# JJKK1313/DiTreeOnlinePlanner

Measured on AMD Instinct MI355X. Metric: candidate tree-expansions/sec (carmaze, H=32), higher is better.
Workload: dtype f16x3; 1 GPU; cfgs/carmaze.yaml + fm_policy flow sampler (K=1), batch=1024 candidates per GPU, H=32 (4 chunks x 8 steps), boxes.csv 20x20, 1024-node tree snapshot, seeded random weights; batch_per_gpu=1024, global_batch=1024, edge_length=32, action_horizon=8, pred_horizon=64, flow_steps=1, tree_nodes=1024, parallelism=candidates sharded x1

## Files before the change

### ditreeonlineplanner_amd/csrc/denoise.h

```cpp
#pragma once
#include <hip/hip_runtime.h>
#include <stdint.h>

enum { MODE_BIAS = 0, MODE_GN_MISH = 1, MODE_GN_MISH_FILM = 2, MODE_GN_MISH_RES = 3 };

enum { ST_BF16 = 0, ST_F32 = 1, ST_F16 = 2 };
static inline int fmt_make(int st, bool split) { return st | (split ? 4 : 0); }
static inline __host__ __device__ int fmt_st(int f) { return f & 3; }
static inline __host__ __device__ bool fmt_split(int f) { return (f & 4) != 0; }
static inline int fmt_es(int f) { return fmt_st(f) == ST_F32 ? 4 : 2; }

struct ConvGemmParams {
  const void* A;
  int lda;
  int in_Lp;
  int in_stride;
  int in_off;
  int taps, Cin;
  const void* W;
  void* Out;
  int ldc;
  int out_Lp, out_stride, out_off;
  int out_coff;
  int L;
  int M, N;
  const float* bias;
  int mode;
  const float* gamma;
  const float* beta;
  int group_ch;
  float eps;
  const float* film;
  int film_ld, film_off;
  const void* Res;
  int ldres, res_Lp, res_off;
  int out_f32;
  int dbg;
  int c2d, c2_H, c2_W, c2_OW, c2_OHW, c2_stride, c2_pad;
  signed char c2_kh[12], c2_kw[12];
  const void* zero;
  long long a_plane, w_plane, out_plane, res_plane;
  float w_scale;
  int splitk;
  long long slab_stride;
  float* sk_ws;
  int* sk_cnt;
  int* sat;
};

void denoise_set_dry_run(bool on);
bool denoise_dry_run();
void launch_conv_gemm(const ConvGemmParams& p, int fmt, hipStream_t s);
bool conv2d_small_eligible(int fmt);
int conv_gemm_kind(const ConvGemmParams& p, int fmt);
bool conv_gemm_supported(const ConvGemmParams& p, int fmt);
void launch_prep_sample(const float* x, void* A0, int B, int P, int D, int fmt, long long plane, hipStream_t s, int* sat = nullptr);
void launch_time_embed(float t, const float* W1, const float* b1, const float* W2, const float* b2, float* out,
                       hipStream_t s);
void launch_prep_cond(const float* temb, const float* map_emb, int E, int E_ld, const float* cond, int G, void* out, int B,
                      int Kpad, int fmt, long long plane, hipStream_t s, int* sat = nullptr);
struct FlowStep {
  int mode;
  float dt;
  float sb, sa, c0, c1, sigma;
  const float* z;
  long long z_row;
  const int* z_idx;
  int z_row0;
};
void launch_final_proj_flow(const void* Y, int C, int Lp, long long plane, const float* W, const float* bias, int D, float* x,
                            FlowStep fs, const double* act_norm , double* actions, int B, int P, int fmt,
                            hipStream_t s);
struct TapList {
  int n;
  signed char kh[49], kw[49];
};
void launch_gn1d(void* x, int ld, int Lp, int row_off, int coff, int L, int C, const float* gamma, const float* beta, float eps,
                 int mode, const float* film, int film_ld, int film_off, const void* res, int ldres, int res_Lp, int res_off,
                 int B, int fmt, long long x_plane, long long res_plane, hipStream_t s, int* sat = nullptr);
void launch_encoder_stem(const float* lm, int n, const float* W, const float* gamma, const float* beta, void* out, int B, float eps,
                         int fmt, long long plane, hipStream_t s, int* sat = nullptr);
void launch_im2col2d(const void* in, bool src_f32, void* out, int B, int H, int W, int C, const TapList& taps, int stride,
                     int pad, int OH, int OW, int Kpad, int fmt, hipStream_t s);
void launch_gn2d(const float* in, int nslab, long long slab_stride, const float* gamma, const float* beta, const void* res,
                 int relu, void* out, int B, int HW, int C, float eps, int fmt, long long res_plane, long long out_plane,
                 hipStream_t s, int* sat = nullptr);
void launch_maxpool2d(const void* in, void* out, int B, int H, int W, int C, int OH, int OW, int fmt, hipStream_t s);
void launch_avgpool2d(const void* in, void* out, int B, int HW, int C, int fmt, long long in_plane, long long out_plane,
                      hipStream_t s);
void launch_unpack_act(const void* in, int ld, int coff, int Lp, int roff, float* out, int B, int L, int C, int fmt,
                       long long plane, hipStream_t s);

enum { ENC_RESNET = 0, ENC_IDENTITY = 1, ENC_MLP = 2, ENC_MAX = 3, ENC_GRID = 4, ENC_CNN = 5 };
struct SmallEncoderParams {
  int kind;
  const float* lm;
  float* out;
  int B, n, E, k;
  const float* w[4];
  const float* b[4];
};
const char* small_encoder_name(int kind);
int small_encoder_width(int kind, int n, int k);
void launch_small_encoder(const SmallEncoderParams& p, hipStream_t s);
```

### ditreeonlineplanner_amd/csrc/denoise_host.hip

```cpp
#include <algorithm>
#include <cmath>
#include <cstring>
#include <functional>
#include <map>
#include <sstream>
#include <thread>

#include "denoise.h"
#include "ditree_internal.h"

namespace {

struct HostParam {
  std::vector<int64_t> dims;
  const float* data = nullptr;
  int64_t n = 0;
};

struct Act {
  void* p = nullptr;
  int L = 0, C = 0;
  int ld = 0, coff = 0;
  bool padded = true;
  long long plane = 0;
  int fmt = 0;
  int Lp() const { return padded ? L + 2 : L; }
};

struct Packed {
  void* p = nullptr;
  long long plane = 0;
  float scale = 1.0f;
};

inline uint16_t f2bf_host(float f) {
  uint32_t u;
  std::memcpy(&u, &f, 4);
  if ((u & 0x7fffffffu) > 0x7f800000u) return (uint16_t)((u >> 16) | 0x40);
  u += 0x7fffu + ((u >> 16) & 1u);
  return (uint16_t)(u >> 16);
}
inline float bf2f_host(uint16_t h) {
  uint32_t u = (uint32_t)h << 16;
  float f;
  std::memcpy(&f, &u, 4);
  return f;
}
inline uint16_t f2h_host(float f) { _Float16 h = (_Float16)f; uint16_t u; std::memcpy(&u, &h, 2); return u; }
inline float h2f_host(uint16_t u) { _Float16 h; std::memcpy(&h, &u, 2); return (float)h; }

}

struct DenoiserState {
  ditree_ctx* ctx = nullptr;
  std::vector<float> blob;
  std::map<std::string, HostParam> params;
  int D = 2, P = 64, E = 400, G = 7, cond_dim = 663, lm = 20;
  int enc_kind = ENC_RESNET;
  int enc_E = -1;
  int enc_k = 0;
  int dims[3] = {512, 1024, 2048};
  bool loaded = false;
  const float* ddpm_coef = nullptr;
  const float* ddpm_z = nullptr;
  long long ddpm_z_row = 0, ddpm_z_step = 0;
  int ddpm_row0 = 0;
  int prec = -1, Bmax = 0;
  int Buser = 0;
  int bgran = 16;
  int ufmt = 0, efmt = 0;
  std::vector<void*> allocs;
  std::map<std::string, Act> named;
  std::map<std::string, Packed> dev_w;
  std::map<std::string, float*> dev_f;
  std::vector<std::function<void(int, int, hipStream_t)>> unet_ops;
  std::vector<std::function<void(int, int, int, hipStream_t)>> enc_ops;
  static constexpr int ENC_SUBS = 4;
  int sub_cap = 0;
  size_t col_region = 0, gout_region = 0;
  hipStream_t aux[ENC_SUBS] = {nullptr, nullptr, nullptr, nullptr};
  hipEvent_t ev_fork = nullptr, ev_join[ENC_SUBS] = {nullptr, nullptr, nullptr, nullptr};
  std::function<void(int, int, hipStream_t)> film_op;
  float* x_cur = nullptr;
  float* temb = nullptr;
  float temb_t = -1.0f;
  float* map_emb = nullptr;
  int E_ld = 400;
  float* film = nullptr;
  void* condA = nullptr;
  long long cond_plane = 0;
  int condK = 0, film_cols = 0;
  Act final_h;
  const float* lm_ptr = nullptr;
  void* zero_row = nullptr;
  static constexpr int SAT_SLOTS = 256;
  int* sat_flags = nullptr;
  int *sat_cond = nullptr, *sat_sample = nullptr;
  std::vector<std::string> sat_names;
  int* sat_slot(const std::string& layer, int fmt) {
    if (fmt_st(fmt) != ST_F16 || sat_flags == nullptr) return nullptr;
    for (size_t i = 0; i < sat_names.size(); ++i)
      if (sat_names[i] == layer) return sat_flags + i;
    if ((int)sat_names.size() >= SAT_SLOTS) return sat_flags + SAT_SLOTS - 1;
    sat_names.push_back(layer);
    return sat_flags + sat_names.size() - 1;
  }
  int last_splitk[4] = {1, 1, 1, 1};
  long long last_slab[4] = {0, 0, 0, 0};
  bool prof_on = false;
  int prof_mode = 0;
  std::vector<hipEvent_t> prof_ev;
  size_t prof_used = 0;
  double prof_ms_done[3] = {0, 0, 0};
  int64_t prof_launches_done[3] = {0, 0, 0};
  double prof_flops_done[3] = {0, 0, 0};
  struct ProfRec { size_t a, b; int kind; double flops; int launches; };
  bool run_open = false;
  size_t run_end = 0;
  void close_run() {
    if (run_open) { hipEventRecord(prof_ev[run_end], prof_last_stream); run_open = false; }
  }
  hipStream_t prof_last_stream = nullptr;
  bool prof_chain = false;
  std::vector<ProfRec> prof_pairs;
  void note_other() { close_run(); prof_chain = false; }
  float* sk_ws = nullptr;
  int* sk_cnt = nullptr;
  static constexpr int SK_MAX_SLABS = 512;
  int pick_splitk(const ConvGemmParams& p, int fmt) {
    const char* e = getenv("DITREE_DENOISE_SPLITK");
    if (!e || atoi(e) == 0 || !fmt_split(fmt) || p.L == 4 || conv_gemm_kind(p, fmt) != 0) return 1;
    const int tiles = (p.M >> 8) * (p.N >> 8), nvc = p.Cin >> 5;
    int sk = 1;
    static const int cap = [] { const char* c = getenv("DITREE_DENOISE_SPLITK_WGS"); return c ? atoi(c) : 64; }();
    while (sk < 16 && tiles * (sk * 2) <= cap && tiles * (sk * 2) <= SK_MAX_SLABS && nvc % (sk * 2) == 0 && nvc / (sk * 2) >= 2) sk *= 2;
    return sk;
  }
  void run_gemm(const ConvGemmParams& p_in, int fmt, hipStream_t s) {
    ConvGemmParams p = p_in;
    static const int strips = [] { const char* e = getenv("DITREE_XCD_STRIPS"); return e ? atoi(e) : 1; }();
    p.dbg = strips;
    if (const int sk = pick_splitk(p, fmt); sk > 1) {
      if (sk_ws == nullptr) {
        sk_ws = (float*)dalloc((size_t)SK_MAX_SLABS * 65536 * sizeof(float), false);
        sk_cnt = (int*)dalloc(SK_MAX_SLABS * sizeof(int));
      }
      p.splitk = sk; p.sk_ws = sk_ws; p.sk_cnt = sk_cnt;
    }
    if (!conv_gemm_supported(p, fmt))
      throw std::runtime_error("denoiser layer of shape M " + std::to_string(p.M) + " x N " + std::to_string(p.N) + " x K " +
                               std::to_string(p.taps) + "*" + std::to_string(p.Cin) + " (L " + std::to_string(p.L) +
                               ") fits no tile of this precision");
    if (!prof_on) { launch_conv_gemm(p, fmt, s); return; }
    if (prof_used + 2 > prof_ev.size()) {
      const size_t old = prof_ev.size();
      prof_ev.resize(old + 4096);
      for (size_t i = old; i < prof_ev.size(); ++i) hipEventCreate(&prof_ev[i]);
    }
    const double fl = 2.0 * (double)p.M * (double)p.N * (double)p.taps * (double)p.Cin;
    if (prof_mode == 2) {
      const int dom = fmt_st(ufmt) == ST_F32 ? 1 : 0;
      if (conv_gemm_kind(p, fmt) != dom || fmt != ufmt) { close_run(); launch_conv_gemm(p, fmt, s); return; }
      if (run_open && prof_last_stream == s) {
        launch_conv_gemm(p, fmt, s);
        prof_pairs.back().flops += fl;
        prof_pairs.back().launches += 1;
        return;
      }
      close_run();
      const size_t st = prof_used++;
      run_end = prof_used++;
      hipEventRecord(prof_ev[st], s);
      launch_conv_gemm(p, fmt, s);
      prof_pairs.push_back(ProfRec{st, run_end, dom, fl, 1});
      run_open = true;
      prof_last_stream = s;
      return;
    }
    size_t start;
    if (prof_chain && prof_last_stream == s && prof_used > 0) {
      start = prof_used - 1;
    } else {
      start = prof_used++;
      hipEventRecord(prof_ev[start], s);
    }
    launch_conv_gemm(p, fmt, s);
    const size_t end = prof_used++;
    hipEventRecord(prof_ev[end], s);
    prof_pairs.push_back(ProfRec{start, end, conv_gemm_kind(p, fmt), fl, 1});
    prof_chain = true;
    prof_last_stream = s;
  }
  void prof_collect() {
    close_run();
    if (prof_used == 0) return;
    hipDeviceSynchronize();
    for (auto& pr : prof_pairs) {
      float ms = 0.f;
      if (hipEventElapsedTime(&ms, prof_ev[pr.a], prof_ev[pr.b]) == hipSuccess) prof_ms_done[pr.kind] += ms;
      prof_launches_done[pr.kind] += pr.launches;
      prof_flops_done[pr.kind] += pr.flops;
    }
    prof_pairs.clear();
    prof_used = 0;
    prof_chain = false;
  }
  int es() const { return fmt_es(ufmt); }
  int ees() const { return fmt_es(efmt); }
  int planes() const { return fmt_split(ufmt) ? 2 : 1; }

  const HostParam& P_(const std::string& name) const {
    auto it = params.find(name);
    if (it == params.end()) throw std::runtime_error("missing parameter " + name);
    return it->second;
  }
  bool has(const std::string& name) const { return params.count(name) != 0; }

  void* dalloc(size_t bytes, bool zero = true) {
    void* p = nullptr;
    if (hipMalloc(&p, bytes ? bytes : 16) != hipSuccess) throw std::runtime_error("hipMalloc failed");
    if (zero && hipMemset(p, 0, bytes ? bytes : 16) != hipSuccess) throw std::runtime_error("hipMemset failed");
    allocs.push_back(p);
    return p;
  }
  void free_workspace() {
    for (void* p : allocs) hipFree(p);
    allocs.clear();
    sk_ws = nullptr;
    sk_cnt = nullptr;
    named.clear();
    dev_w.clear();
    dev_f.clear();
    enc_ops.clear();
    unet_ops.clear();
    film_op = nullptr;
    sat_flags = sat_cond = sat_sample = nullptr;
    sat_names.clear();
    prec = -1;
    Bmax = 0;
    Buser = 0;
    temb_t = -1.0f;
  }

  float* upload_f32(const std::string& key, const float* src, int64_t n) {
    auto it = dev_f.find(key);
    if (it != dev_f.end()) return it->second;
    float* d = (float*)dalloc((size_t)n * 4, false);
    if (hipMemcpy(d, src, (size_t)n * 4, hipMemcpyHostToDevice) != hipSuccess) throw std::runtime_error("memcpy");
    dev_f[key] = d;
    return d;
  }
  float* vec(const std::string& name) {
    const HostParam& hp = P_(name);
    return upload_f32(name, hp.data, hp.n);
  }

  template <class F>
  Packed pack(const std::string& key, int fmt, int N, int T, int Cin_pad, F get) {
    auto it = dev_w.find(key);
    if (it != dev_w.end()) return it->second;
    const int Npad = (N + 255) / 256 * 256;
    const size_t K = (size_t)T * Cin_pad, total = (size_t)Npad * K;
    const int st = fmt_st(fmt), e = fmt_es(fmt), npl = fmt_split(fmt) ? 2 : 1;
    std::vector<uint8_t> host(total * e * npl, 0);
    const int nthreads = std::max(1u, std::min(16u, std::thread::hardware_concurrency()));
    float mul = 1.0f;
    if (st == ST_F16) {
      std::vector<float> mx(nthreads, 0.0f);
      std::vector<std::thread> th;
      for (int ti = 0; ti < nthreads; ++ti)
        th.emplace_back([&, ti]() {
          float m = 0.f;
          for (int n = ti; n < N; n += nthreads)
            for (int t = 0; t < T; ++t)
              for (int ci = 0; ci < Cin_pad; ++ci) m = std::max(m, std::fabs(get(n, t, ci)));
          mx[ti] = m;
        });
      for (auto& t : th) t.join();
      const float m = *std::max_element(mx.begin(), mx.end());
      if (m > 0.f && std::isfinite(m)) {
        int ex;
        std::frexp(m, &ex);
        mul = std::ldexp(1.0f, 14 - ex);
      }
    }
    std::vector<std::thread> th;
    for (int ti = 0; ti < nthreads; ++ti) {
      th.emplace_back([&, ti]() {
        for (int n = ti; n < N; n += nthreads) {
          for (int t = 0; t < T; ++t)
            for (int ci = 0; ci < Cin_pad; ++ci) {
              const float v = get(n, t, ci) * mul;
              const size_t idx = (size_t)n * K + (size_t)t * Cin_pad + ci;
              if (st == ST_F32) { ((float*)host.data())[idx] = v; continue; }
              uint16_t* hi = (uint16_t*)host.data();
              uint16_t* lo = hi + total;
              if (st == ST_BF16) {
                hi[idx] = f2bf_host(v);
                if (npl == 2) lo[idx] = f2bf_host(v - bf2f_host(hi[idx]));
              } else {
                hi[idx] = f2h_host(v);
                if (npl == 2) lo[idx] = f2h_host(v - h2f_host(hi[idx]));
              }
            }
        }
      });
    }
    for (auto& t : th) t.join();
    Packed pk;
    pk.p = dalloc(total * e * npl, false);
    pk.plane = npl == 2 ? (long long)(total * e) : 0;
    pk.scale = 1.0f / mul;
    if (hipMemcpy(pk.p, host.data(), total * e * npl, hipMemcpyHostToDevice) != hipSuccess) throw std::runtime_error("memcpy");
    dev_w[key] = pk;
    return pk;
  }
  static void set_w(ConvGemmParams& p, const Packed& pk) { p.W = pk.p; p.w_plane = pk.plane; p.w_scale = pk.scale; }

  Act make_act(const std::string& name, int L, int C, bool padded = true) {
    Act a;
    a.L = L; a.C = C; a.ld = C; a.coff = 0; a.padded = padded; a.fmt = ufmt;
    const size_t bytes = (size_t)Bmax * a.Lp() * C * es();
    a.plane = planes() == 2 ? (long long)bytes : 0;
    if (planes() == 2 && bytes >= 0x7f000000ull) throw std::runtime_error("activation plane of 2 GiB or more: lower the reserved batch");
    a.p = dalloc(bytes * planes());
    named[name] = a;
    return a;
  }
  static void set_in(ConvGemmParams& p, const Act& in) { p.a_plane = in.plane; }
  static void set_out(ConvGemmParams& p, const Act& out) { p.out_plane = out.plane; }
  static Act view(const Act& base, int coff, int C, const char* = nullptr) {
    Act v = base;
    v.coff = coff;
    v.C = C;
    return v;
  }
  const char* aptr(const Act& a) const { return (const char*)a.p + (size_t)a.coff * es(); }

  void add_conv3(std::vector<std::function<void(int, int, hipStream_t)>>& ops, const std::string& wname, const Act& in,
                 const Act& out, int mode, const std::string& gn, int film_off, const Act* res) {
    const HostParam& w = P_(wname + ".weight");
    const int Cout = (int)w.dims[0], Cin = (int)w.dims[1];
    const float* wd = w.data;
    const Packed wp = pack(wname, ufmt, Cout, 3, Cin, [=](int n, int t, int ci) { return wd[((size_t)n * Cin + ci) * 3 + t]; });
    ConvGemmParams p{};
    p.A = aptr(in); p.lda = in.ld; p.in_Lp = in.Lp(); p.in_stride = 1; p.in_off = 0; p.taps = 3; p.Cin = Cin;
    set_w(p, wp); set_in(p, in); set_out(p, out);
    p.sat = sat_slot(wname, ufmt);
    p.Out = (void*)aptr(out); p.ldc = out.ld; p.out_Lp = out.Lp(); p.out_stride = 1; p.out_off = 1; p.out_coff = 0;
    p.L = in.L; p.N = Cout; p.bias = vec(wname + ".bias"); p.mode = mode; p.eps = 1e-5f;
    if (mode >= MODE_GN_MISH) {
      p.gamma = vec(gn + ".weight"); p.beta = vec(gn + ".bias"); p.group_ch = Cout / 8;
    }
    if (mode == MODE_GN_MISH_FILM) { p.film = film; p.film_ld = film_cols; p.film_off = film_off; }
    if (mode == MODE_GN_MISH_RES) {
      p.Res = aptr(*res); p.ldres = res->ld; p.res_Lp = res->Lp(); p.res_off = res->padded ? 1 : 0; p.res_plane = res->plane;
    }
    emit_block(ops, p, out, in.L);
  }
  void emit_block(std::vector<std::function<void(int, int, hipStream_t)>>& ops, const ConvGemmParams& p, const Act& out, int L) {
    const int Cout = p.N, mode = p.mode, uf = ufmt;
    const int gch = Cout / 8;
    static const bool short_unfused = [] { const char* e = getenv("DITREE_GN_SHORT_UNFUSED"); return e && atoi(e) != 0; }();
    const bool short_fusable = (L == 8 || L == 4) && fmt_st(uf) != ST_F32 && !short_unfused;
    const bool fused = mode < MODE_GN_MISH ||
                       ((Cout & 255) == 0 && (gch == 64 || gch == 128 || gch == 256) && ((L & 15) == 0 || short_fusable));
    const bool fused_needs_tiles = fused && mode >= MODE_GN_MISH && (L & 15) != 0;
    ConvGemmParams qf = p, q = p;
    q.mode = MODE_BIAS;
    const float* film_p = p.film;
    const int film_ld_ = p.film_ld, film_off_ = p.film_off, ldres = p.ldres, res_Lp = p.res_Lp, res_off = p.res_off;
    const void* resp = p.Res;
    const float *ga = p.gamma, *be = p.beta;
    void* xo = (void*)out.p;
    const int ld = out.ld, oLp = out.Lp(), ocoff = out.coff;
    const long long xpl = out.plane, rpl = p.res_plane;
    int* gsat = p.sat;
    ops.push_back([=, this](int, int Bp, hipStream_t s) mutable {
      if (fused && (!fused_needs_tiles || ((Bp * L) & 255) == 0)) {
        qf.M = Bp * L;
        run_gemm(qf, uf, s);
        return;
      }
      q.M = Bp * L;
      run_gemm(q, uf, s);
      note_other();
      launch_gn1d(xo, ld, oLp, 1, ocoff, L, Cout, ga, be, 1e-5f, mode, film_p, film_ld_, film_off_, resp, ldres, res_Lp,
                  res_off, Bp, uf, xpl, rpl, s, gsat);
    });
  }
  void add_conv1(std::vector<std::function<void(int, int, hipStream_t)>>& ops, const std::string& wname, const Act& in,
                 const Act& out) {
    const HostParam& w = P_(wname + ".weight");
    const int Cout = (int)w.dims[0], Cin = (int)w.dims[1];
    const float* wd = w.data;
    const Packed wp = pack(wname, ufmt, Cout, 1, Cin, [=](int n, int, int ci) { return wd[(size_t)n * Cin + ci]; });
    ConvGemmParams p{};
    p.A = aptr(in); p.lda = in.ld; p.in_Lp = in.Lp(); p.in_stride = 1; p.in_off = 1; p.taps = 1; p.Cin = Cin;
    set_w(p, wp); set_in(p, in); set_out(p, out);
    p.sat = sat_slot(wname, ufmt);
    p.Out = (void*)aptr(out); p.ldc = out.ld; p.out_Lp = out.Lp(); p.out_stride = 1; p.out_off = 1;
    p.L = in.L; p.N = Cout; p.bias = vec(wname + ".bias"); p.mode = MODE_BIAS;
    const int L = in.L, uf = ufmt;
    ops.push_back([this, p, L, uf](int, int Bp, hipStream_t s) mutable {
      p.M = Bp * L;
      run_gemm(p, uf, s);
    });
  }
  void add_down(std::vector<std::function<void(int, int, hipStream_t)>>& ops, const std::string& wname, const Act& in,
                const Act& out) {
    const HostParam& w = P_(wname + ".weight");
    const int Cout = (int)w.dims[0], Cin = (int)w.dims[1];
    const float* wd = w.data;
    const Packed wp = pack(wname, ufmt, Cout, 3, Cin, [=](int n, int t, int ci) { return wd[((size_t)n * Cin + ci) * 3 + t]; });
    ConvGemmParams p{};
    p.A = aptr(in); p.lda = in.ld; p.in_Lp = in.Lp(); p.in_stride = 2; p.in_off = 0; p.taps = 3; p.Cin = Cin;
    set_w(p, wp); set_in(p, in); set_out(p, out);
    p.sat = sat_slot(wname, ufmt);
    p.Out = (void*)aptr(out); p.ldc = out.ld; p.out_Lp = out.Lp(); p.out_stride = 1; p.out_off = 1;
    p.L = out.L; p.N = Cout; p.bias = vec(wname + ".bias"); p.mode = MODE_BIAS;
    const int L = out.L, uf = ufmt;
    ops.push_back([this, p, L, uf](int, int Bp, hipStream_t s) mutable {
      p.M = Bp * L;
      run_gemm(p, uf, s);
    });
  }
  void add_up(std::vector<std::function<void(int, int, hipStream_t)>>& ops, const std::string& wname, const Act& in,
              const Act& out) {
    const HostParam& w = P_(wname + ".weight");
    const int Cin = (int)w.dims[0], Cout = (int)w.dims[1];
    const float* wd = w.data;
    for (int par = 0; par < 2; ++par) {
      const int k0 = par == 0 ? 3 : 2, k1 = par == 0 ? 1 : 0;
      const Packed wp = pack(wname + (par ? ".odd" : ".even"), ufmt, Cout, 2, Cin, [=](int n, int t, int ci) {
        return wd[((size_t)ci * Cout + n) * 4 + (t == 0 ? k0 : k1)];
      });
      ConvGemmParams p{};
      p.A = aptr(in); p.lda = in.ld; p.in_Lp = in.Lp(); p.in_stride = 1; p.in_off = par; p.taps = 2; p.Cin = Cin;
      set_w(p, wp); set_in(p, in); set_out(p, out);
      p.sat = sat_slot(wname, ufmt);
      p.Out = (void*)aptr(out); p.ldc = out.ld; p.out_Lp = out.Lp(); p.out_stride = 2; p.out_off = 1 + par;
      p.L = in.L; p.N = Cout; p.bias = vec(wname + ".bias"); p.mode = MODE_BIAS;
      const int L = in.L, uf = ufmt;
      ops.push_back([this, p, L, uf](int, int Bp, hipStream_t s) mutable {
        p.M = Bp * L;
        run_gemm(p, uf, s);
      });
    }
  }

  void add_crb(const std::string& pre, const Act& in, const Act& out, int& film_cursor, const std::string& tag) {
    const int Cout = (int)P_(pre + ".blocks.0.block.0.weight").dims[0];
    Act h = make_act(tag + ".h", in.L, Cout);
    const int film_off = film_cursor;
    film_cursor += 2 * Cout;
    add_conv3(unet_ops, pre + ".blocks.0.block.0", in, h, MODE_GN_MISH_FILM, pre + ".blocks.0.block.1", film_off, nullptr);
    Act res = in;
    if (has(pre + ".residual_conv.weight")) {
      res = make_act(tag + ".res", in.L, Cout);
      add_conv1(unet_ops, pre + ".residual_conv", in, res);
    }
    add_conv3(unet_ops, pre + ".blocks.1.block.0", h, out, MODE_GN_MISH_RES, pre + ".blocks.1.block.1", 0, &res);
  }

  void build(int prec_, int Bmax_);
};

void DenoiserState::build(int prec_, int Bmax_) {
  free_workspace();
  prec = prec_;
  switch (prec) {
    case DITREE_PREC_BF16: ufmt = fmt_make(ST_BF16, false); efmt = ST_BF16; break;
    case DITREE_PREC_F32: ufmt = fmt_make(ST_F32, false); efmt = ST_F32; break;
    case DITREE_PREC_F16X3: ufmt = fmt_make(ST_F16, true); efmt = ufmt; break;
    case DITREE_PREC_BF16X3: ufmt = fmt_make(ST_BF16, true); efmt = ufmt; break;
    case DITREE_PREC_F16: ufmt = fmt_make(ST_F16, false); efmt = ST_F16; break;
    default: throw std::runtime_error("unknown precision");
  }
  sat_flags = (int*)dalloc(SAT_SLOTS * sizeof(int));
  sat_cond = sat_slot("cond_encoder input: Mish(time | map embedding | observation)", ufmt);
  sat_sample = sat_slot("sample (the noisy action sequence)", ufmt);
  const int C0 = dims[0], C1 = dims[1], C2 = dims[2];
  const int L0 = P, L1 = P / 2, L2 = P / 4;
  if (P % 16 != 0 || P < 16 || P > 256 || (256 % P) != 0) throw std::runtime_error("pred_horizon must be 16, 32, 64, 128 or 256");
  bgran = fmt_st(ufmt) != ST_F32 ? std::max(16, 1024 / P) : 16;
  Buser = Bmax_;
  Bmax = (Bmax_ + bgran - 1) / bgran * bgran;
  {
    const long long per_sample = std::max({(long long)(L2 + 2) * 2 * C2, (long long)(L1 + 2) * 2 * C1, (long long)(L0 + 2) * C0,
                                           (long long)L0 * 64}) * fmt_es(ufmt);
    long long cap = std::min<long long>(8192, 0x7f000000LL / per_sample);
    cap = cap / 256 * 256;
    if (cap < 256) throw std::runtime_error("denoiser too large for one 256-sample work unit");
    if (Bmax > cap) Bmax = (int)cap;
  }
  if (fmt_split(ufmt) && ((C0 | C1 | C2) & 255) != 0)
    throw std::runtime_error("the split precisions need down_dims that are multiples of 256 (halo / gemm16 tiles)");
  x_cur = (float*)dalloc((size_t)Bmax * P * D * 4);
  temb = (float*)dalloc(256 * 4);
  condK = (cond_dim + 63) / 64 * 64;
  const int Brows = (Bmax + 255) / 256 * 256;
  E_ld = (enc_kind == ENC_RESNET && fmt_split(efmt)) ? (E + 255) / 256 * 256 : E;
  map_emb = (float*)dalloc((size_t)Brows * E_ld * 4);
  cond_plane = planes() == 2 ? (long long)Brows * condK * es() : 0;
  condA = dalloc((size_t)Brows * condK * es() * planes());

  std::vector<std::string> crbs = {"unet.down_modules.0.0", "unet.down_modules.0.1", "unet.down_modules.1.0",
                                   "unet.down_modules.1.1", "unet.down_modules.2.0", "unet.down_modules.2.1",
                                   "unet.mid_modules.0",    "unet.mid_modules.1",    "unet.up_modules.0.0",
                                   "unet.up_modules.0.1",   "unet.up_modules.1.0",   "unet.up_modules.1.1"};
  film_cols = 0;
  std::vector<int> film_offs;
  for (auto& c : crbs) {
    film_offs.push_back(film_cols);
    film_cols += (int)P_(c + ".cond_encoder.1.weight").dims[0];
  }
  film = (float*)dalloc((size_t)Brows * film_cols * 4);
  {
    std::vector<const float*> wsrc, bsrc;
    std::vector<int> rows;
    for (auto& c : crbs) {
      wsrc.push_back(P_(c + ".cond_encoder.1.weight").data);
      bsrc.push_back(P_(c + ".cond_encoder.1.bias").data);
      rows.push_back((int)P_(c + ".cond_encoder.1.weight").dims[0]);
    }
    std::vector<int> start(rows.size());
    for (size_t i = 0, a = 0; i < rows.size(); ++i) { start[i] = (int)a; a += rows[i]; }
    const int cd = cond_dim;
    const Packed wp = pack("film.all", ufmt, film_cols, 1, condK, [=](int n, int, int ci) {
      size_t i = std::upper_bound(start.begin(), start.end(), n) - start.begin() - 1;
      return ci < cd ? wsrc[i][(size_t)(n - start[i]) * cd + ci] : 0.0f;
    });
    std::vector<float> ball(film_cols);
    for (size_t i = 0; i < rows.size(); ++i) std::memcpy(ball.data() + start[i], bsrc[i], (size_t)rows[i] * 4);
    float* bd = upload_f32("film.bias", ball.data(), film_cols);
    ConvGemmParams p{};
    p.A = condA; p.lda = condK; p.in_Lp = 0; p.in_stride = 1; p.in_off = 0; p.taps = 1; p.Cin = condK;
    set_w(p, wp); p.a_plane = cond_plane;
    p.Out = film; p.ldc = film_cols; p.out_Lp = 0; p.out_stride = 1; p.out_off = 0;
    p.N = film_cols; p.bias = bd; p.mode = MODE_BIAS; p.out_f32 = 1;
    const int uf = ufmt;
    film_op = [this, p, uf](int, int Bp, hipStream_t s) mutable {
      const int Mr = fmt_st(uf) == ST_F32 ? Bp : (Bp + 255) / 256 * 256;
      p.M = Mr; p.L = Mr; p.in_Lp = Mr; p.out_Lp = Mr;
      run_gemm(p, uf, s);
    };
  }

  int fc = 0;
  Act a0;
  a0.L = L0; a0.C = 64; a0.ld = 64; a0.coff = 0; a0.padded = false; a0.fmt = ufmt;
  a0.plane = planes() == 2 ? (long long)Bmax * L0 * 64 * es() : 0;
  a0.p = dalloc((size_t)Bmax * L0 * 64 * es() * planes());
  named["a0"] = a0;
  {
    const std::string pre = "unet.down_modules.0.0";
    const HostParam& w = P_(pre + ".blocks.0.block.0.weight");
    const float* wd = w.data;
    const int Dd = D;
    const Packed wp = pack(pre + ".blocks.0.block.0", ufmt, C0, 1, 64, [=](int n, int, int ci) {
      if (ci >= 3 * Dd) return 0.0f;
      const int t = ci / Dd, d = ci - t * Dd;
      return wd[((size_t)n * Dd + d) * 3 + t];
    });
    Act h = make_act("d0b1.h", L0, C0);
    ConvGemmParams p{};
    p.A = a0.p; p.lda = 64; p.in_Lp = L0; p.in_stride = 1; p.in_off = 0; p.taps = 1; p.Cin = 64;
    set_w(p, wp); set_in(p, a0); set_out(p, h);
    p.sat = sat_slot(pre + ".blocks.0.block.0", ufmt);
    p.Out = h.p; p.ldc = h.ld; p.out_Lp = h.Lp(); p.out_stride = 1; p.out_off = 1;
    p.L = L0; p.N = C0; p.bias = vec(pre + ".blocks.0.block.0.bias"); p.mode = MODE_GN_MISH_FILM; p.eps = 1e-5f;
    p.gamma = vec(pre + ".blocks.0.block.1.weight"); p.beta = vec(pre + ".blocks.0.block.1.bias"); p.group_ch = C0 / 8;
    p.film = film; p.film_ld = film_cols; p.film_off = film_offs[0];
    const int L = L0;
    emit_block(unet_ops, p, h, L0);
    const HostParam& wr = P_(pre + ".residual_conv.weight");
    const float* wrd = wr.data;
    const Packed wrp = pack(pre + ".residual_conv", ufmt, C0, 1, 64, [=](int n, int, int ci) {
      return (ci >= Dd && ci < 2 * Dd) ? wrd[(size_t)n * Dd + (ci - Dd)] : 0.0f;
    });
    Act res = make_act("d0b1.res", L0, C0);
    ConvGemmParams q{};
    q.A = a0.p; q.lda = 64; q.in_Lp = L0; q.in_stride = 1; q.in_off = 0; q.taps = 1; q.Cin = 64;
    set_w(q, wrp); set_in(q, a0); set_out(q, res);
    q.sat = sat_slot(pre + ".residual_conv", ufmt);
    q.Out = res.p; q.ldc = res.ld; q.out_Lp = res.Lp(); q.out_stride = 1; q.out_off = 1;
    q.L = L0; q.N = C0; q.bias = vec(pre + ".residual_conv.bias"); q.mode = MODE_BIAS;
    const int uf = ufmt;
    unet_ops.push_back([this, q, L, uf](int, int Bp, hipStream_t s) mutable { q.M = Bp * L; run_gemm(q, uf, s); });
    Act o = make_act("d0b1.out", L0, C0);
    add_conv3(unet_ops, pre + ".blocks.1.block.0", h, o, MODE_GN_MISH_RES, pre + ".blocks.1.block.1", 0, &res);
    fc = film_offs[1];
  }
  Act cat1 = make_act("cat1", L1, 2 * C1);
  Act cat0 = make_act("cat0", L2, 2 * C2);
  Act d0o = named["d0b1.out"];
  Act skip0 = make_act("skip0", L0, C0);
  add_crb("unet.down_modules.0.1", d0o, skip0, fc, "d0b2");
  Act d1in = make_act("d1.in", L1, C0);
  add_down(unet_ops, "unet.down_modules.0.2.conv", skip0, d1in);
  Act d1o = make_act("d1b1.out", L1, C1);
  add_crb("unet.down_modules.1.0", d1in, d1o, fc, "d1b1");
  Act skip1 = view(cat1, C1, C1);
  named["skip1"] = skip1;
  add_crb("unet.down_modules.1.1", d1o, skip1, fc, "d1b2");
  Act d2in = make_act("d2.in", L2, C1);
  add_down(unet_ops, "unet.down_modules.1.2.conv", skip1, d2in);
  Act d2o = make_act("d2b1.out", L2, C2);
  add_crb("unet.down_modules.2.0", d2in, d2o, fc, "d2b1");
  Act skip2 = view(cat0, C2, C2);
  named["skip2"] = skip2;
  add_crb("unet.down_modules.2.1", d2o, skip2, fc, "d2b2");
  Act m1 = make_act("mid1.out", L2, C2);
  add_crb("unet.mid_modules.0", skip2, m1, fc, "mid1");
  Act m2 = view(cat0, 0, C2);
  named["mid2.out"] = m2;
  add_crb("unet.mid_modules.1", m1, m2, fc, "mid2");
  Act u0a = make_act("u0b1.out", L2, C1);
  add_crb("unet.up_modules.0.0", cat0, u0a, fc, "u0b1");
  Act u0b = make_act("u0b2.out", L2, C1);
  add_crb("unet.up_modules.0.1", u0a, u0b, fc, "u0b2");
  Act up0 = view(cat1, 0, C1);
  named["up0.out"] = up0;
  add_up(unet_ops, "unet.up_modules.0.2.conv", u0b, up0);
  Act u1a = make_act("u1b1.out", L1, C0);
  add_crb("unet.up_modules.1.0", cat1, u1a, fc, "u1b1");
  Act u1b = make_act("u1b2.out", L1, C0);
  add_crb("unet.up_modules.1.1", u1a, u1b, fc, "u1b2");
  Act fin = make_act("final.in", L0, C0);
  add_up(unet_ops, "unet.up_modules.1.2.conv", u1b, fin);
  final_h = make_act("final.h", L0, C0);
  add_conv3(unet_ops, "unet.final_conv.0.block.0", fin, final_h, MODE_GN_MISH, "unet.final_conv.0.block.1", 0, nullptr);
  vec("unet.final_conv.1.weight");
  vec("unet.final_conv.1.bias");
  vec("unet.diffusion_step_encoder.1.weight");
  vec("unet.diffusion_step_encoder.1.bias");
  vec("unet.diffusion_step_encoder.3.weight");
  vec("unet.diffusion_step_encoder.3.bias");

  sub_cap = ((Bmax + ENC_SUBS - 1) / ENC_SUBS + 15) / 16 * 16;
  if (enc_kind != ENC_RESNET) {
    SmallEncoderParams q{};
    q.kind = enc_kind; q.n = lm; q.E = E; q.k = enc_k;
    auto transposed = [&](const std::string& name, int out_f, int in_f) {
      const HostParam& w = P_(name);
      if (w.dims.size() != 2 || w.dims[0] != out_f || w.dims[1] != in_f)
        throw std::runtime_error(name + " must be (" + std::to_string(out_f) + ", " + std::to_string(in_f) + ")");
      std::vector<float> t((size_t)out_f * in_f);
      for (int o = 0; o < out_f; ++o)
        for (int i = 0; i < in_f; ++i) t[(size_t)i * out_f + o] = w.data[(size_t)o * in_f + i];
      return upload_f32(name + "#t", t.data(), (int64_t)t.size());
    };
    auto conv_w = [&](const std::string& name, int co, int ci) {
      const HostParam& w = P_(name + ".weight");
      const HostParam& b = P_(name + ".bias");
      if (w.dims.size() != 4 || w.dims[0] != co || w.dims[1] != ci || w.dims[2] != 3 || w.dims[3] != 3 || b.n != co)
        throw std::runtime_error(name + " must be a Conv2d(" + std::to_string(ci) + ", " + std::to_string(co) + ", 3)");
    };
    if (enc_kind == ENC_MLP) {
      const int in_f = lm * lm;
      q.w[0] = transposed("encoder.fc1.weight", 128, in_f);
      q.w[1] = transposed("encoder.fc2.weight", 256, 128);
      q.w[2] = transposed("encoder.fc3.weight", E, 256);
      const int outs[3] = {128, 256, E};
      for (int l = 0; l < 3; ++l) {
        const std::string bn = "encoder.fc" + std::to_string(l + 1) + ".bias";
        if (P_(bn).n != outs[l]) throw std::runtime_error(bn + " must have " + std::to_string(outs[l]) + " elements");
        q.b[l] = vec(bn);
      }
    } else if (enc_kind == ENC_GRID || enc_kind == ENC_CNN) {
      const bool g = enc_kind == ENC_GRID;
      const int nl = g ? 3 : 4;
      const int ci[4] = {1, g ? 3 : 2, g ? 6 : 4, 4}, co[4] = {g ? 3 : 2, g ? 6 : 4, 4, 4};
      for (int l = 0; l < nl; ++l) {
        const std::string nm = "encoder.conv" + std::to_string(l + 1);
        conv_w(nm, co[l], ci[l]);
        q.w[l] = vec(nm + ".weight");
        q.b[l] = vec(nm + ".bias");
      }
    }
    const float** lm_slot = &lm_ptr;
    float* op = map_emb;
    const int LM = lm * lm, Ew = E;
    enc_ops.push_back([=, this](int b0, int Bn, int, hipStream_t s) {
      note_other();
      SmallEncoderParams r = q;
      r.lm = *lm_slot + (size_t)b0 * LM; r.out = op + (size_t)b0 * Ew; r.B = Bn;
      launch_small_encoder(r, s);
    });
  } else {
    const std::string R = "encoder.resnet18.";
    const int pr = efmt;
    const size_t E_ = ees();
    zero_row = dalloc(256);
    const size_t col_per_sample = 25 * 576;
    const size_t gout_per_sample = 9216;
    col_region = (size_t)sub_cap * col_per_sample;
    gout_region = (size_t)sub_cap * gout_per_sample;
    char* col = (char*)dalloc(col_region * ENC_SUBS * E_);
    float* gout = (float*)dalloc(gout_region * ENC_SUBS * 4);
    const size_t colreg = col_region, goutreg = gout_region;
    auto ebuf = [&](const std::string& name, int HW, int C) {
      Act a;
      a.L = HW; a.C = C; a.ld = C; a.coff = 0; a.padded = false; a.fmt = efmt;
      const size_t rows = HW == 1 ? (size_t)Brows : (size_t)Bmax;
      const size_t bytes = rows * HW * C * ees();
      a.plane = fmt_split(efmt) ? (long long)bytes : 0;
      a.p = dalloc(bytes * (fmt_split(efmt) ? 2 : 1));
      named[name] = a;
      return a;
    };
    auto live_taps = [](int k, int stride, int pad, int H, int OH) {
      TapList tl{};
      for (int kh = 0; kh < k; ++kh)
        for (int kw = 0; kw < k; ++kw) {
          bool lh = false, lw = false;
          for (int o = 0; o < OH; ++o) {
            const int ih = o * stride + kh - pad, iw = o * stride + kw - pad;
            lh |= (ih >= 0 && ih < H);
            lw |= (iw >= 0 && iw < H);
          }
          if (lh && lw) { tl.kh[tl.n] = (signed char)kh; tl.kw[tl.n] = (signed char)kw; ++tl.n; }
        }
      return tl;
    };
    auto conv2d = [&](const std::string& wname, const void* in, long long in_plane, int H, int Cin, int Cout, int k, int stride,
                      int pad, int OH, bool fold_in) {
      const HostParam& w = P_(wname + ".weight");
      const float* wd = w.data;
      const int Cw = (int)w.dims[1];
      const TapList tl = live_taps(k, stride, pad, H, OH);
      const int K = tl.n * Cin, Kpad = (K + 63) / 64 * 64;
      if ((size_t)OH * OH * Kpad > col_per_sample || (size_t)OH * OH * Cout > gout_per_sample)
        throw std::runtime_error("encoder scratch region too small for " + wname);
      const Packed wp = pack(wname, efmt, Cout, 1, Kpad, [=](int n, int, int kk) {
        if (kk >= K) return 0.0f;
        const int c = kk % Cin, t = kk / Cin, kw = tl.kw[t], kh = tl.kh[t];
        if (!fold_in) return wd[(((size_t)n * Cw + c) * k + kh) * k + kw];
        float s = 0.f;
        for (int cc = 0; cc < Cw; ++cc) s += wd[(((size_t)n * Cw + cc) * k + kh) * k + kw];
        return s;
      });
      const float** lm_slot = &lm_ptr;
      const bool implicit = (in != nullptr) && (Cin % 64 == 0) && tl.n <= 12;
      if (!implicit && fmt_split(efmt)) throw std::runtime_error("split encoder: " + wname + " needs the im2col path");
      const void* zr = zero_row;
      enc_ops.push_back([=, this](int b0, int Bn, int reg, hipStream_t s) {
        char* colr = col + (size_t)reg * colreg * E_;
        float* goutr = gout + (size_t)reg * goutreg;
        ConvGemmParams p{};
        const int M = Bn * OH * OH;
        if (implicit) {
          p.A = (const char*)in + (size_t)b0 * H * H * Cin * E_; p.lda = Cin; p.taps = tl.n; p.Cin = Cin; p.a_plane = in_plane;
          p.c2d = 1; p.c2_H = H; p.c2_W = H; p.c2_OW = OH; p.c2_OHW = OH * OH; p.c2_stride = stride; p.c2_pad = pad;
          for (int t = 0; t < tl.n; ++t) { p.c2_kh[t] = tl.kh[t]; p.c2_kw[t] = tl.kw[t]; }
          p.zero = zr;
          const int nk_total = tl.n * (Cin / 64);
          const int tiles = ((1024 * OH * OH + 255) / 256) * ((Cout + 255) / 256);
          static int sk_target = -1, sk_cap = 8;
          if (sk_target < 0) {
            const char* e = getenv("DITREE_SPLITK_TARGET");
            sk_target = (e && atoi(e) > 0) ? atoi(e) : 256;
            const char* c = getenv("DITREE_SPLITK_CAP");
            if (c && atoi(c) > 0) sk_cap = atoi(c);
          }
          int sk = std::max(1, std::min(std::min(sk_cap, nk_total / 2), std::max(1, sk_target / tiles)));
          while (sk > 1 && (size_t)sk * OH * OH * Cout > gout_per_sample) --sk;
          if (sk > 1) {
            const int per = (nk_total + sk - 1) / sk;
            sk = (nk_total + per - 1) / per;
          }
          static int use_split = -1;
          if (use_split < 0) { const char* e = getenv("DITREE_SPLITK"); use_split = (e && !atoi(e)) ? 0 : 1; }
          if (conv2d_small_eligible(pr)) {
            static int small_target = -1;
            if (small_target < 0) { const char* e = getenv("DITREE_C2D_TARGET"); small_target = (e && atoi(e) > 0) ? atoi(e) : 768; }
            const int tiles64 = ((1024 * OH * OH + 63) / 64) * (Cout / 64);
            sk = std::max(1, std::min(std::min(8, nk_total / 2), small_target / tiles64));
            while (sk > 1 && (size_t)sk * OH * OH * Cout > gout_per_sample) --sk;
            if (sk > 1) {
              const int per = (nk_total + sk - 1) / sk;
              sk = (nk_total + per - 1) / per;
            }
          }
          if (!use_split) sk = 1;
// ... 6 lines not shown
          last_slab[reg] = 0;
        }
        if (!implicit) {
          note_other();
          if (in == nullptr)
            launch_im2col2d(*lm_slot + (size_t)b0 * H * H, true, colr, Bn, H, H, 1, tl, stride, pad, OH, OH, Kpad, pr, s);
          else
            launch_im2col2d((const char*)in + (size_t)b0 * H * H * Cin * E_, false, colr, Bn, H, H, Cin, tl, stride, pad,
                            OH, OH, Kpad, pr, s);
          p.A = colr; p.lda = Kpad; p.taps = 1; p.Cin = Kpad;
        }
        p.in_Lp = M; p.in_stride = 1; p.in_off = 0;
        set_w(p, wp);
        p.Out = goutr; p.ldc = Cout; p.out_Lp = M; p.out_stride = 1; p.out_off = 0;
        p.L = M; p.M = M; p.N = Cout; p.mode = MODE_BIAS; p.out_f32 = 1;
        run_gemm(p, pr, s);
      });
    };
    auto gn = [&](const std::string& gname, const Act& out, const Act* res, bool relu) {
      float* ga = vec(gname + ".weight");
      float* be = vec(gname + ".bias");
      const char* rp = res ? (const char*)res->p : nullptr;
      char* op = (char*)out.p;
      const int HW = out.L, C = out.C;
      const long long rpl = res ? res->plane : 0, opl = out.plane;
      {
        const int pp = (C >= 64 && C <= 1024 && (C & (C - 1)) == 0) ? 256 / (C >> 2) : 0;
        if (pp == 0 || (HW + pp - 1) / pp > 7)
          throw std::runtime_error("encoder GroupNorm: unsupported map (" + std::to_string(HW) + " pixels x " + std::to_string(C) + " channels)");
      }
      int* gsat = sat_slot(gname, efmt);
      enc_ops.push_back([=, this](int b0, int Bn, int reg, hipStream_t s) {
        note_other();
        const size_t off = (size_t)b0 * HW * C * E_;
        launch_gn2d(gout + (size_t)reg * goutreg, last_splitk[reg], last_slab[reg], ga, be, rp ? rp + off : nullptr,
                    relu ? 1 : 0, op + off, Bn, HW, C, 1e-5f, pr, rpl, opl, s, gsat);
      });
    };
    const int H0 = lm;
    auto osz = [](int h, int k, int s, int p) { return (h + 2 * p - k) / s + 1; };
    const int H1 = osz(H0, 7, 2, 3);
    const int H2 = osz(H1, 3, 2, 1);
    Act c1 = ebuf("enc.c1", H1 * H1, 64);
    Act pool = ebuf("enc.pool", H2 * H2, 64);
    if (H0 == 20 || H0 == 16) {
      const HostParam& w = P_(R + "conv1.weight");
      const int Cw = (int)w.dims[1];
      std::vector<float> wf(64 * 49);
      for (int n = 0; n < 64; ++n)
        for (int t = 0; t < 49; ++t) {
          float sacc = 0.f;
          for (int cc = 0; cc < Cw; ++cc) sacc += w.data[((size_t)n * Cw + cc) * 49 + t];
          wf[t * 64 + n] = sacc;
        }
      float* wdev = upload_f32(R + "conv1.weight#folded", wf.data(), 64 * 49);
      float* ga = vec(R + "bn1.weight");
      float* be = vec(R + "bn1.bias");
      char* op = (char*)pool.p;
      const float** lm_slot = &lm_ptr;
      const long long ppl = pool.plane;
      int* ssat = sat_slot(R + "conv1", efmt);
      enc_ops.push_back([=, this](int b0, int Bn, int, hipStream_t s) {
        note_other();
        launch_encoder_stem(*lm_slot + (size_t)b0 * H0 * H0, H0, wdev, ga, be, op + (size_t)b0 * H2 * H2 * 64 * E_, Bn, 1e-5f, pr, ppl, s, ssat);
      });
    } else {
    conv2d(R + "conv1", nullptr, 0, H0, 1, 64, 7, 2, 3, H1, true);
    gn(R + "bn1", c1, nullptr, true);
    {
      const char* ip = (const char*)c1.p; char* op = (char*)pool.p;
      const int a = H1, b2 = H2;
      enc_ops.push_back([=, this](int b0, int Bn, int, hipStream_t s) {
        note_other();
        launch_maxpool2d(ip + (size_t)b0 * a * a * 64 * E_, op + (size_t)b0 * b2 * b2 * 64 * E_, Bn, a, a, 64, b2, b2, pr, s);
      });
    }
    }
    Act cur = pool;
    int Hc = H2, Cc = 64;
    const int chans[4] = {64, 128, 256, 512};
    for (int li = 0; li < 4; ++li) {
      for (int bi = 0; bi < 2; ++bi) {
        const std::string pre = R + "layer" + std::to_string(li + 1) + "." + std::to_string(bi);
        const int Cout = chans[li];
        const int stride = (bi == 0 && li > 0) ? 2 : 1;
        const int Ho = osz(Hc, 3, stride, 1);
        const std::string tag = "enc.l" + std::to_string(li + 1) + "." + std::to_string(bi);
        Act t1 = ebuf(tag + ".t", Ho * Ho, Cout);
        conv2d(pre + ".conv1", cur.p, cur.plane, Hc, Cc, Cout, 3, stride, 1, Ho, false);
        gn(pre + ".bn1", t1, nullptr, true);
        Act idt = cur;
        if (has(pre + ".downsample.0.weight")) {
          Act ds = ebuf(tag + ".ds", Ho * Ho, Cout);
          conv2d(pre + ".downsample.0", cur.p, cur.plane, Hc, Cc, Cout, 1, stride, 0, Ho, false);
          gn(pre + ".downsample.1", ds, nullptr, false);
          idt = ds;
        }
        Act o = ebuf(tag + ".out", Ho * Ho, Cout);
        conv2d(pre + ".conv2", t1.p, t1.plane, Ho, Cout, Cout, 3, 1, 1, Ho, false);
        gn(pre + ".bn2", o, &idt, true);
        cur = o;
        Hc = Ho;
        Cc = Cout;
      }
    }
    Act pooled = ebuf("enc.avg", 1, Cc);
    {
      const char* ip = (const char*)cur.p; char* op = (char*)pooled.p;
      const int HW = Hc * Hc, C = Cc;
      const long long ipl = cur.plane, opl = pooled.plane;
      enc_ops.push_back([=, this](int b0, int Bn, int, hipStream_t s) {
        note_other();
        launch_avgpool2d(ip + (size_t)b0 * HW * C * E_, op + (size_t)b0 * C * E_, Bn, HW, C, pr, ipl, opl, s);
      });
    }
    {
      const HostParam& w = P_(R + "fc.weight");
      const float* wd = w.data;
      const int Kf = (int)w.dims[1], Nf = (int)w.dims[0];
      const Packed wp = pack(R + "fc", efmt, Nf, 1, Kf, [=](int n, int, int ci) { return wd[(size_t)n * Kf + ci]; });
      const bool esplit = fmt_split(efmt);
      const int eld = E_ld;
      float* bd;
      if (esplit) {
        std::vector<float> bpad(eld, 0.0f);
        std::memcpy(bpad.data(), P_(R + "fc.bias").data, (size_t)Nf * 4);
        bd = upload_f32(R + "fc.bias#padded", bpad.data(), eld);
      } else {
        bd = vec(R + "fc.bias");
      }
      const char* ip = (const char*)pooled.p;
      float* op = map_emb;
      const long long ppl = pooled.plane;
      enc_ops.push_back([=, this](int b0, int Bn, int, hipStream_t s) {
        ConvGemmParams p{};
        const int Mr = esplit ? (Bn + 255) / 256 * 256 : Bn;
        p.A = ip + (size_t)b0 * Kf * E_; p.lda = Kf; p.in_Lp = Mr; p.in_stride = 1; p.in_off = 0; p.taps = 1; p.Cin = Kf;
        set_w(p, wp); p.a_plane = ppl;
        p.Out = op + (size_t)b0 * eld; p.ldc = eld; p.out_Lp = Mr; p.out_stride = 1; p.out_off = 0;
        p.L = Mr; p.M = Mr; p.N = esplit ? eld : Nf; p.bias = bd; p.mode = MODE_BIAS; p.out_f32 = 1;
        run_gemm(p, pr, s);
      });
    }
  }
  if (hipDeviceSynchronize() != hipSuccess) throw std::runtime_error("sync after build failed");
  {
    float* lm_dev = (float*)dalloc((size_t)bgran * lm * lm * 4);
    lm_ptr = lm_dev;
    denoise_set_dry_run(true);
    try {
      for (auto& op : enc_ops) op(0, bgran, 0, nullptr);
      film_op(bgran, bgran, nullptr);
      for (auto& op : unet_ops) op(bgran, bgran, nullptr);
    } catch (...) {
      denoise_set_dry_run(false);
      lm_ptr = nullptr;
      throw;
    }
    denoise_set_dry_run(false);
    lm_ptr = nullptr;
  }
}

static int parse_manifest(DenoiserState* st, const char* manifest, int64_t n_floats) {
  std::istringstream in(manifest);
  std::string line;
  while (std::getline(in, line)) {
    if (line.empty()) continue;
    if (line.rfind("#config", 0) == 0) {
      std::istringstream cs(line.substr(7));
      std::string key;
      int val;
      while (cs >> key >> val) {
        if (key == "pred_horizon") st->P = val;
        else if (key == "local_map_size") st->lm = val;
      }
      continue;
    }
    if (line.rfind("#encoder", 0) == 0) {
      std::istringstream cs(line.substr(8));
      std::string kind;
      if (!(cs >> kind)) return -1;
      st->enc_kind = -1;
      for (int k = ENC_RESNET; k <= ENC_CNN; ++k)
        if (kind == small_encoder_name(k)) st->enc_kind = k;
      if (st->enc_kind < 0) return -3;
      int e;
      if (cs >> e) st->enc_E = e;
      continue;
    }
    if (line.rfind("#checksum", 0) == 0) {
      std::istringstream cs(line.substr(9));
      std::string a, b;
      if (!(cs >> a >> b)) return -1;
      const uint32_t* w = (const uint32_t*)st->blob.data();
      uint64_t s1 = 0, s2 = 0;
      for (int64_t i = 0; i < n_floats; ++i) { s1 += w[i]; s2 += s1; }
      if (s1 != std::stoull(a, nullptr, 16) || s2 != std::stoull(b, nullptr, 16)) return -2;
      continue;
    }
    if (line[0] == '#') continue;
    std::istringstream ls(line);
    std::string name;
    int64_t off, n;
    int nd;
    if (!(ls >> name >> off >> n >> nd)) return -1;
    HostParam hp;
    int64_t prod = 1;
    for (int i = 0; i < nd; ++i) {
      int64_t d;
      if (!(ls >> d)) return -1;
      hp.dims.push_back(d);
      prod *= d;
    }
    if (prod != n || off < 0 || off + n > n_floats) return -1;
    hp.data = st->blob.data() + off;
    hp.n = n;
    st->params[name] = hp;
  }
  return 0;
}

static int denoise_core(ditree_ctx* ctx, const float* noise, int64_t noise_stride, const int32_t* noise_idx,
                        const float* local_map, const float* cond, int B, int K, const float* t0, const float* dt,
                        const double* act_norm, double* actions, float* x_out, hipStream_t s, float t_scale, int raw,
                        int reuse_encoder);

static int denoise_core_one(ditree_ctx* ctx, const float* noise, int64_t noise_stride, const int32_t* noise_idx,
                            const float* local_map, const float* cond, int B, int K, const float* t0, const float* dt,
                            const double* act_norm, double* actions, float* x_out, hipStream_t s, float t_scale, int raw,
                            int reuse_encoder);

int denoise_run_ddpm(ditree_ctx* ctx, const float* noise, int64_t noise_stride, const int32_t* noise_idx, const float* local_map,
                     const float* cond, int B, int K, const float* timesteps, const float* coef, const float* z, int64_t z_row,
                     int64_t z_step, const double* act_norm, double* actions, float* x_out, hipStream_t s) {
  DenoiserState* st = ctx->dn;
  if (!st || !st->loaded) return set_err(ctx, DITREE_E_STATE, "denoise: weights not loaded");
  if (!coef || !timesteps || K < 1) return set_err(ctx, DITREE_E_ARG, "denoise_ddpm: schedule missing");
  std::vector<float> ones((size_t)K, 1.0f);
  st->ddpm_coef = coef; st->ddpm_z = z; st->ddpm_z_row = z_row; st->ddpm_z_step = z_step; st->ddpm_row0 = 0;
  const int rc = denoise_core(ctx, noise, noise_stride, noise_idx, local_map, cond, B, K, timesteps, ones.data(), act_norm, actions,
                              x_out, s, 1.0f, 0, 0);
  st->ddpm_coef = nullptr; st->ddpm_z = nullptr;
  return rc;
}

int denoise_wave_quantum(ditree_ctx* ctx) {
  DenoiserState* st = ctx->dn;
  if (!st || !st->loaded) return 512;
  const long long q = 256ll * 65536ll / ((long long)st->P * st->dims[0]);
  return (int)std::max(64ll, std::min(q, 65536ll));
}

int denoise_run(ditree_ctx* ctx, const float* noise, int64_t noise_stride, const int32_t* noise_idx, const float* local_map,
                const float* cond, int B, int K, const float* t0, const float* dt, const double* act_norm, double* actions,
                float* x_out, hipStream_t s) {
  return denoise_core(ctx, noise, noise_stride, noise_idx, local_map, cond, B, K, t0, dt, act_norm, actions, x_out, s,
                      20.0f , 0, 0);
}

static int denoise_core(ditree_ctx* ctx, const float* noise, int64_t noise_stride, const int32_t* noise_idx,
                        const float* local_map, const float* cond, int B, int K, const float* t0, const float* dt,
                        const double* act_norm, double* actions, float* x_out, hipStream_t s, float t_scale, int raw,
                        int reuse_encoder) {
  DenoiserState* st = ctx->dn;
  if (!st || !st->loaded) return set_err(ctx, DITREE_E_STATE, "denoise: weights not loaded");
  if (st->prec < 0) return set_err(ctx, DITREE_E_STATE, "denoise: call ditree_denoise_reserve first");
  if (B <= 0 || B > st->Buser) return set_err(ctx, DITREE_E_ARG, "denoise: batch exceeds the reserved workspace");
  if (B <= st->Bmax)
    return denoise_core_one(ctx, noise, noise_stride, noise_idx, local_map, cond, B, K, t0, dt, act_norm, actions, x_out, s,
                            t_scale, raw, reuse_encoder);
  if (!noise || !local_map || !cond) return set_err(ctx, DITREE_E_ARG, "denoise: bad argument");
  const size_t PD = (size_t)st->P * st->D, LM = (size_t)st->lm * st->lm;
  const int row0 = st->ddpm_row0;
  for (int b0 = 0; b0 < B; b0 += st->Bmax) {
    const int bn = std::min(st->Bmax, B - b0);
    st->ddpm_row0 = row0 + (noise_idx ? 0 : b0);
    const int rc = denoise_core_one(ctx, noise_idx ? noise : noise + (size_t)b0 * noise_stride, noise_stride,
                                    noise_idx ? noise_idx + b0 : nullptr, local_map + (size_t)b0 * LM, cond + (size_t)b0 * st->G, bn,
                                    K, t0, dt, act_norm, actions ? actions + (size_t)b0 * PD : nullptr,
                                    x_out ? x_out + (size_t)b0 * PD : nullptr, s, t_scale, raw, 0);
    if (rc) { st->ddpm_row0 = row0; return rc; }
  }
  st->ddpm_row0 = row0;
  return DITREE_OK;
}

static int denoise_core_one(ditree_ctx* ctx, const float* noise, int64_t noise_stride, const int32_t* noise_idx,
                            const float* local_map, const float* cond, int B, int K, const float* t0, const float* dt,
                            const double* act_norm, double* actions, float* x_out, hipStream_t s, float t_scale, int raw,
                            int reuse_encoder) {
  DenoiserState* st = ctx->dn;
  if (B <= 0 || B > st->Bmax) return set_err(ctx, DITREE_E_ARG, "denoise: batch exceeds the workspace");
  if (!noise || !local_map || !cond || !t0 || !dt || !act_norm || K <= 0 || (!actions && !x_out))
    return set_err(ctx, DITREE_E_ARG, "denoise: bad argument");
  const int Bp = (B + st->bgran - 1) / st->bgran * st->bgran;
  const int uf = st->ufmt;
  {
    const size_t row = (size_t)st->P * st->D * 4;
    if (noise_stride < (int64_t)st->P * st->D) return set_err(ctx, DITREE_E_ARG, "denoise: noise stride");
    if (noise_idx)
      launch_gather_rows_f32(noise, noise_stride, noise_idx, st->x_cur, st->P * st->D, B, s);
    else
      HIP_TRY(ctx, hipMemcpy2DAsync(st->x_cur, row, noise, (size_t)noise_stride * 4, row, (size_t)B,
                                    hipMemcpyDeviceToDevice, s));
  }
  st->lm_ptr = local_map;
  try {
  if (!reuse_encoder) {
    static int subs_env = -1;
    if (subs_env < 0) { const char* e = getenv("DITREE_ENC_SUBS"); subs_env = e ? std::max(1, std::min(atoi(e), (int)DenoiserState::ENC_SUBS)) : 1; }
    const int nsub = (B >= 64 && !fmt_split(st->efmt)) ? subs_env : 1;
    const int per = nsub == 1 ? B : std::min(st->sub_cap, (((B + nsub - 1) / nsub) + 15) / 16 * 16);
    if (nsub > 1 && !st->aux[1]) {
      for (int i = 1; i < DenoiserState::ENC_SUBS; ++i) {
        HIP_TRY(ctx, hipStreamCreateWithFlags(&st->aux[i], hipStreamNonBlocking));
        HIP_TRY(ctx, hipEventCreateWithFlags(&st->ev_join[i], hipEventDisableTiming));
      }
      HIP_TRY(ctx, hipEventCreateWithFlags(&st->ev_fork, hipEventDisableTiming));
    }
    if (nsub > 1) HIP_TRY(ctx, hipEventRecord(st->ev_fork, s));
    for (int i = 0; i < nsub; ++i) {
      const int b0 = i * per, bn = std::min(per, B - b0);
      if (bn <= 0) break;
      hipStream_t si = (i == 0) ? s : st->aux[i];
      if (i > 0) HIP_TRY(ctx, hipStreamWaitEvent(si, st->ev_fork, 0));
      for (auto& op : st->enc_ops) op(b0, bn, i, si);
      if (i > 0) {
        HIP_TRY(ctx, hipEventRecord(st->ev_join[i], si));
        HIP_TRY(ctx, hipStreamWaitEvent(s, st->ev_join[i], 0));
      }
    }
  }
  for (int k = 0; k < K; ++k) {
    const float t = t0[k] * t_scale;
    if (t != st->temb_t) {
      launch_time_embed(t, st->dev_f["unet.diffusion_step_encoder.1.weight"], st->dev_f["unet.diffusion_step_encoder.1.bias"],
                        st->dev_f["unet.diffusion_step_encoder.3.weight"], st->dev_f["unet.diffusion_step_encoder.3.bias"],
                        st->temb, s);
      st->temb_t = K == 1 ? t : -1.0f;
    }
    st->note_other();
    launch_prep_cond(st->temb, st->map_emb, st->E, st->E_ld, cond, st->G, st->condA, B, st->condK, uf, st->cond_plane, s,
                     st->sat_cond);
    st->film_op(B, Bp, s);
    st->note_other();
    launch_prep_sample(st->x_cur, st->named["a0"].p, Bp, st->P, st->D, uf, st->named["a0"].plane, s,
                       st->sat_sample);
    for (auto& op : st->unet_ops) op(B, Bp, s);
    const bool last = (k == K - 1);
    st->note_other();
    FlowStep fs{};
    fs.mode = raw ? 1 : 0;
    fs.dt = dt[k];
    if (st->ddpm_coef) {
      const float* c = st->ddpm_coef + 5 * k;
      fs.mode = 2; fs.sb = c[0]; fs.sa = c[1]; fs.c0 = c[2]; fs.c1 = c[3]; fs.sigma = c[4];
      fs.z = st->ddpm_z ? st->ddpm_z + (long long)k * st->ddpm_z_step : nullptr;
      fs.z_row = st->ddpm_z_row; fs.z_idx = noise_idx; fs.z_row0 = st->ddpm_row0;
      if (fs.sigma != 0.0f && !fs.z) return set_err(ctx, DITREE_E_ARG, "denoise: a DDPM step with sigma > 0 needs step noise");
    }
    launch_final_proj_flow(st->final_h.p, st->final_h.C, st->final_h.Lp(), st->final_h.plane, st->dev_f["unet.final_conv.1.weight"],
                           st->dev_f["unet.final_conv.1.bias"], st->D, st->x_cur, fs, act_norm,
                           (last && actions) ? actions : nullptr, B, st->P, uf, s);
  }
  } catch (const std::exception& e) {
    return set_err(ctx, DITREE_E_ARG, std::string("denoise: ") + e.what());
  }
  if (x_out) HIP_TRY(ctx, hipMemcpyAsync(x_out, st->x_cur, (size_t)B * st->P * st->D * 4, hipMemcpyDeviceToDevice, s));
  HIP_TRY(ctx, hipGetLastError());
  return DITREE_OK;
}

void denoise_destroy(ditree_ctx* ctx) {
  if (ctx->dn) {
    for (auto e : ctx->dn->prof_ev) hipEventDestroy(e);
    ctx->dn->prof_ev.clear();
    for (int i = 1; i < DenoiserState::ENC_SUBS; ++i) {
      if (ctx->dn->aux[i]) hipStreamDestroy(ctx->dn->aux[i]);
      if (ctx->dn->ev_join[i]) hipEventDestroy(ctx->dn->ev_join[i]);
    }
    if (ctx->dn->ev_fork) hipEventDestroy(ctx->dn->ev_fork);
    ctx->dn->free_workspace();
    delete ctx->dn;
    ctx->dn = nullptr;
  }
}

extern "C" {

int32_t ditree_load_weights(ditree_ctx* ctx, const float* blob, int64_t n_floats, const char* manifest, void* stream) {
  if (!ctx) return DITREE_E_ARG;
  if (!blob || !manifest || n_floats <= 0) return set_err(ctx, DITREE_E_ARG, "load_weights: bad argument");
  HIP_TRY(ctx, hipSetDevice(ctx->device));
  denoise_destroy(ctx);
  DenoiserState* st = new (std::nothrow) DenoiserState();
  if (!st) return set_err(ctx, DITREE_E_NOMEM, "load_weights: out of memory");
  st->ctx = ctx;
  try {
    st->blob.assign(blob, blob + n_floats);
    const int prc = parse_manifest(st, manifest, n_floats);
    if (prc == -2) throw std::runtime_error("weight blob does not match the manifest checksum");
    if (prc == -3) throw std::runtime_error("unknown encoder in the manifest (identity, mlp, max, grid, cnn or resnet)");
    if (prc != 0) throw std::runtime_error("malformed manifest");
    const HostParam& w0 = st->P_("unet.down_modules.0.0.blocks.0.block.0.weight");
    st->D = (int)w0.dims[1];
    for (int i = 0; i < 3; ++i)
      st->dims[i] = (int)st->P_("unet.down_modules." + std::to_string(i) + ".0.blocks.0.block.0.weight").dims[0];
    if (st->has("unet.down_modules.3.0.blocks.0.block.0.weight")) throw std::runtime_error("only 3 U-Net levels supported");
    st->cond_dim = (int)st->P_("unet.down_modules.0.0.cond_encoder.1.weight").dims[1];
    if (st->lm != 20 && st->lm != 16) throw std::runtime_error("local_map_size must be 20 (car) or 16 (ant)");
    if (st->enc_kind == ENC_RESNET) {
      st->E = (int)st->P_("encoder.resnet18.fc.weight").dims[0];
      if (st->enc_E >= 0 && st->enc_E != st->E) throw std::runtime_error("the manifest's encoder width differs from encoder.resnet18.fc");
    } else {
      const std::string kn = small_encoder_name(st->enc_kind);
      if (st->enc_E < 1) throw std::runtime_error("the manifest's #encoder line must carry the embedding width");
      st->enc_k = 0;
      if (st->enc_kind == ENC_MAX) {
        int k = 1;
        while ((k + 1) * (k + 1) <= st->enc_E) ++k;
        if (k * k != st->enc_E) throw std::runtime_error("encoder 'max': the embedding width must be a perfect square, got " + std::to_string(st->enc_E));
        st->enc_k = k;
      }
      st->E = small_encoder_width(st->enc_kind, st->lm, st->enc_k);
      if (st->E != st->enc_E)
        throw std::runtime_error("encoder '" + kn + "' produces " + std::to_string(st->E) + " columns at local_map_size " +
                                 std::to_string(st->lm) + ", the manifest declares " + std::to_string(st->enc_E));
    }
    st->G = st->cond_dim - 256 - st->E;
    if (st->G < 0 && st->enc_kind != ENC_RESNET)
      throw std::runtime_error("the U-Net's cond_dim " + std::to_string(st->cond_dim) + " is narrower than 256 + the encoder's " +
                               std::to_string(st->E) + " columns");
    if (st->G < 0 || (st->D != 2 && st->D != 8)) throw std::runtime_error("unsupported dimensions (action_dim 2 or 8)");
    if (st->P_("unet.diffusion_step_encoder.1.weight").dims[1] != 256) throw std::runtime_error("diffusion_step_embed_dim must be 256");
    for (int i = 0; i < 3; ++i)
      if (st->dims[i] % 64 != 0 || st->dims[i] > 4096) throw std::runtime_error("down_dims must be multiples of 64, <= 4096");
  } catch (const std::exception& e) {
    delete st;
    return set_err(ctx, DITREE_E_ARG, std::string("load_weights: ") + e.what());
  }
  st->loaded = true;
  ctx->dn = st;
  (void)stream;
  return DITREE_OK;
}

int32_t ditree_denoise_reserve(ditree_ctx* ctx, int32_t max_batch, int32_t precision) {
  if (!ctx) return DITREE_E_ARG;
  DenoiserState* st = ctx->dn;
  if (!st || !st->loaded) return set_err(ctx, DITREE_E_STATE, "denoise_reserve: weights not loaded");
  if (max_batch <= 0 || precision < DITREE_PREC_BF16 || precision > DITREE_PREC_F16)
    return set_err(ctx, DITREE_E_ARG, "denoise_reserve: bad argument");
  HIP_TRY(ctx, hipSetDevice(ctx->device));
  if (st->prec == precision && st->Buser >= max_batch) return DITREE_OK;
  try {
    HIP_TRY(ctx, hipDeviceSynchronize());
    st->build(precision, max_batch);
  } catch (const std::exception& e) {
    st->free_workspace();
    return set_err(ctx, DITREE_E_NOMEM, std::string("denoise_reserve: ") + e.what());
  }
  return DITREE_OK;
}

int32_t ditree_denoise(ditree_ctx* ctx, const float* noise, const float* local_map, const float* cond, int32_t B,
                       int32_t K, const float* t0, const float* dt, const double* act_norm, double* actions,
                       float* x_out, void* stream) {
  if (!ctx) return DITREE_E_ARG;
  if (!ctx->dn) return set_err(ctx, DITREE_E_STATE, "denoise: weights not loaded");
  return denoise_run(ctx, noise, (int64_t)ctx->dn->P * ctx->dn->D, nullptr, local_map, cond, B, K, t0, dt, act_norm, actions, x_out,
                     (hipStream_t)stream);
}

int32_t ditree_denoise_ddpm(ditree_ctx* ctx, const float* noise, const float* step_noise, const float* local_map, const float* cond,
                            int32_t B, int32_t K, const float* timesteps, const float* coef, const double* act_norm,
                            double* actions, float* x_out, void* stream) {
  if (!ctx) return DITREE_E_ARG;
  if (!ctx->dn) return set_err(ctx, DITREE_E_STATE, "denoise_ddpm: weights not loaded");
  if (B == 0) return DITREE_OK;
  const int64_t PD = (int64_t)ctx->dn->P * ctx->dn->D;
  return denoise_run_ddpm(ctx, noise, PD, nullptr, local_map, cond, B, K, timesteps, coef, step_noise, (int64_t)K * PD, PD, act_norm,
                          actions, x_out, (hipStream_t)stream);
}

int32_t ditree_denoise_eval(ditree_ctx* ctx, const float* sample, const float* local_map, const float* cond, int32_t B,
                            float timestep, int32_t reuse_encoder, float* out, void* stream) {
  if (!ctx) return DITREE_E_ARG;
  if (!ctx->dn) return set_err(ctx, DITREE_E_STATE, "denoise_eval: weights not loaded");
  if (!out) return set_err(ctx, DITREE_E_ARG, "denoise_eval: bad argument");
  const float one = 1.0f;
  double unit[16];
  for (int d = 0; d < 8; ++d) { unit[d] = 0.0; unit[8 + d] = 1.0; }
  for (int d = 0; d < ctx->dn->D && d < 8; ++d) { unit[d] = 0.0; unit[ctx->dn->D + d] = 1.0; }
  return denoise_core(ctx, sample, (int64_t)ctx->dn->P * ctx->dn->D, nullptr, local_map, cond, B, 1, &timestep, &one, unit,
                      nullptr, out, (hipStream_t)stream, 1.0f, 1, reuse_encoder);
}

int32_t ditree_denoise_dims(ditree_ctx* ctx, int32_t* dims5) {
  if (!ctx) return DITREE_E_ARG;
  DenoiserState* st = ctx->dn;
  if (!st || !st->loaded || !dims5) return set_err(ctx, DITREE_E_STATE, "denoise_dims: weights not loaded");
  dims5[0] = st->P; dims5[1] = st->D; dims5[2] = st->lm; dims5[3] = st->G; dims5[4] = st->E;
  return DITREE_OK;
}

int32_t ditree_denoise_status(ditree_ctx* ctx, int32_t* n_saturated, char* names, int64_t names_cap, int32_t clear,
                              void* stream) {
  if (!ctx) return DITREE_E_ARG;
  DenoiserState* st = ctx->dn;
  if (!n_saturated || (names_cap > 0 && !names)) return set_err(ctx, DITREE_E_ARG, "denoise_status: bad argument");
  *n_saturated = 0;
  if (names_cap > 0) names[0] = '\0';
  if (!st || st->prec < 0 || st->sat_flags == nullptr || st->sat_names.empty()) return DITREE_OK;
  hipStream_t s = (hipStream_t)stream;
  std::vector<int> host(st->sat_names.size());
  HIP_TRY(ctx, hipMemcpyAsync(host.data(), st->sat_flags, host.size() * sizeof(int), hipMemcpyDeviceToHost, s));
  HIP_TRY(ctx, hipStreamSynchronize(s));
  std::string text;
  for (size_t i = 0; i < host.size(); ++i)
    if (host[i] != 0) {
      ++*n_saturated;
      if (!text.empty()) text += "\n";
      text += st->sat_names[i];
    }
  if (names_cap > 0) {
    const size_t n = std::min((size_t)names_cap - 1, text.size());
    std::memcpy(names, text.data(), n);
    names[n] = '\0';
  }
  if (clear && *n_saturated) HIP_TRY(ctx, hipMemsetAsync(st->sat_flags, 0, host.size() * sizeof(int), s));
  return DITREE_OK;
}

int32_t ditree_profile(ditree_ctx* ctx, int32_t enable) {
  if (!ctx) return DITREE_E_ARG;
  DenoiserState* st = ctx->dn;
  if (!st) return set_err(ctx, DITREE_E_STATE, "profile: weights not loaded");
  st->prof_collect();
  st->prof_on = enable != 0;
  st->prof_mode = enable;
  if (enable) for (int k = 0; k < 3; ++k) { st->prof_ms_done[k] = 0.0; st->prof_launches_done[k] = 0; st->prof_flops_done[k] = 0.0; }
  return DITREE_OK;
}

int32_t ditree_profile_read(ditree_ctx* ctx, double* ms3, int64_t* launches3, double* flops3) {
  if (!ctx) return DITREE_E_ARG;
  DenoiserState* st = ctx->dn;
  if (!st || !ms3 || !launches3 || !flops3) return set_err(ctx, DITREE_E_STATE, "profile_read: bad state");
  st->prof_collect();
  for (int k = 0; k < 3; ++k) {
    ms3[k] = st->prof_ms_done[k];
    launches3[k] = st->prof_launches_done[k];
    flops3[k] = st->prof_flops_done[k];
  }
  return DITREE_OK;
}

int32_t ditree_denoise_debug_read(ditree_ctx* ctx, const char* name, int32_t B, float* out, int64_t capacity,
                                  int32_t* dims3, void* stream) {
  if (!ctx) return DITREE_E_ARG;
  DenoiserState* st = ctx->dn;
  if (!st || st->prec < 0 || !name || !out || !dims3) return set_err(ctx, DITREE_E_STATE, "debug_read: no workspace");
  hipStream_t s = (hipStream_t)stream;
  std::string nm(name);
  if (nm == "film" || nm == "map_emb") {
    const int cols = nm == "film" ? st->film_cols : st->E;
    const int ld = nm == "film" ? st->film_cols : st->E_ld;
    const float* src = nm == "film" ? st->film : st->map_emb;
    if ((int64_t)B * cols > capacity) return set_err(ctx, DITREE_E_ARG, "debug_read: capacity");
    HIP_TRY(ctx, hipMemcpy2DAsync(out, (size_t)cols * 4, src, (size_t)ld * 4, (size_t)cols * 4, (size_t)B, hipMemcpyDeviceToDevice, s));
    dims3[0] = B; dims3[1] = 1; dims3[2] = cols;
    return DITREE_OK;
  }
  auto it = st->named.find(nm);
  if (it == st->named.end()) return set_err(ctx, DITREE_E_ARG, "debug_read: unknown buffer " + nm);
  const Act& a = it->second;
  if ((int64_t)B * a.L * a.C > capacity) return set_err(ctx, DITREE_E_ARG, "debug_read: capacity");
  launch_unpack_act(a.p, a.ld, a.coff, a.Lp(), a.padded ? 1 : 0, out, B, a.L, a.C, a.fmt, a.plane, s);
  dims3[0] = B; dims3[1] = a.L; dims3[2] = a.C;
  HIP_TRY(ctx, hipGetLastError());
  return DITREE_OK;
}

}
```

### ditreeonlineplanner_amd/csrc/denoise_kernels.hip

```cpp
#include <cstdlib>
#include <type_traits>

#include <stdexcept>

#include "denoise.h"

static thread_local bool g_dn_dry_run = false;
void denoise_set_dry_run(bool on) { g_dn_dry_run = on; }
bool denoise_dry_run() { return g_dn_dry_run; }
#define DN_LAUNCH(...) do { if (!g_dn_dry_run) hipLaunchKernelGGL(__VA_ARGS__); } while (0)

typedef __attribute__((ext_vector_type(8))) __bf16 bf16x8_t;
typedef __attribute__((ext_vector_type(8))) _Float16 half8_t;
typedef __attribute__((ext_vector_type(8))) short short8_t;
typedef __attribute__((ext_vector_type(4))) short short4_t;
typedef __attribute__((ext_vector_type(16))) float f32x16_t;
typedef __attribute__((ext_vector_type(4))) float f32x4_t;
typedef __attribute__((ext_vector_type(2))) float f32x2_t;
typedef __attribute__((ext_vector_type(2))) _Float16 half2_t;
typedef __attribute__((ext_vector_type(2))) short short2_t;

#define GLOBAL_AS __attribute__((address_space(1)))
#define LDS_AS __attribute__((address_space(3)))

// ... 381 lines not shown
    const int c = (r & 128) + 4 * (r & 31) + ((r >> 5) & 3);
    boff[q] = (((long long)(tn * 256 + c)) * K + slot * EPS) * ES;
  }
  const char* pa[4];
  const char* pb[4];
#pragma unroll
  for (int q = 0; q < 4; ++q) {
    pa[q] = Abase + aoff[q];
    pb[q] = Wbase + boff[q] + (long long)k_first * 128;
  }
  int kin = C2D ? (k_first % kpt) : 0;
  const long long a_tap_jump = ((long long)p.lda - (long long)p.Cin + EK) * ES;
  const char* c2_base[4];
  int c2_ih0[4], c2_iw0[4], c2_slot[4];
  int c2_tap = C2D ? (k_first / kpt) : 0;
  if constexpr (C2D) {
#pragma unroll
    for (int q = 0; q < 4; ++q) {
      const int r = (w * 4 + q) * 8 + (lane >> 3);
      int m = tm * 256 + r;
      m = m < p.M ? m : p.M - 1;
      const int b = m / p.c2_OHW, rem = m - b * p.c2_OHW;
      const int oh = rem / p.c2_OW, ow = rem - oh * p.c2_OW;
      c2_base[q] = Abase + (long long)b * p.c2_H * p.c2_W * p.Cin * ES;
      c2_ih0[q] = oh * p.c2_stride - p.c2_pad;
      c2_iw0[q] = ow * p.c2_stride - p.c2_pad;
      c2_slot[q] = ((lane & 7) ^ ((r >> 1) & 7)) * 16;
    }
  }
  auto c2_point = [&]() {
    const int kh = p.c2_kh[c2_tap], kw = p.c2_kw[c2_tap];
#pragma unroll
    for (int q = 0; q < 4; ++q) {
      const int ih = c2_ih0[q] + kh, iw = c2_iw0[q] + kw;
      const bool ok = ih >= 0 && ih < p.c2_H && iw >= 0 && iw < p.c2_W;
      const char* src = c2_base[q] + ((long long)(ih * p.c2_W + iw) * p.Cin + kin * EK) * ES;
      pa[q] = (ok ? src : (const char*)p.zero) + c2_slot[q];
    }
  };
  if constexpr (C2D) c2_point();
  auto advance = [&]() {
    ++kin;
    if constexpr (C2D) {
      if (kin == kpt) { kin = 0; ++c2_tap; }
      if (c2_tap < p.taps) c2_point();
#pragma unroll
      for (int q = 0; q < 4; ++q) pb[q] += 128;
    } else {
      long long ainc = 128;
      if (kin == kpt) { kin = 0; ainc = a_tap_jump; }
#pragma unroll
      for (int q = 0; q < 4; ++q) {
        pa[q] += ainc;
        pb[q] += 128;
      }
    }
  };
  auto stage_piece = [&](int q, char* sbase) {
    if (q < 4)
      __builtin_amdgcn_global_load_lds((const GLOBAL_AS void*)pa[q], (LDS_AS void*)(sbase + (w * 4 + q) * 1024), 16, 0, 0);
    else
      __builtin_amdgcn_global_load_lds((const GLOBAL_AS void*)pb[q - 4],
                                       (LDS_AS void*)(sbase + 32768 + (w * 4 + q - 4) * 1024), 16, 0, 0);
  };

  f32x16_t acc[2][4];
#pragma unroll
  for (int mb = 0; mb < 2; ++mb)
#pragma unroll
    for (int j = 0; j < 4; ++j)
#pragma unroll
      for (int i = 0; i < 16; ++i) acc[mb][j][i] = 0.0f;

  const int swl = (r5 >> 1) & 7;
  const int a_row_off = (wm * 64 + r5) * 128;
  const int b_row_off = 32768 + (wn * 128 + r5) * 128;

  auto kstep = [&](const char* sb, auto stage_tag, char* snext) {
    constexpr bool STAGE = decltype(stage_tag)::value;
    if constexpr (PREC != 1) {
      short8_t af[2][2], bfr[2][4];
      auto rd = [&](int ks, int slot) {
        const int ps = (((ks << 1) | h) ^ swl) << 4;
#pragma unroll
        for (int mb = 0; mb < 2; ++mb)
          af[slot][mb] = *(const short8_t*)(sb + a_row_off + mb * 4096 + ps);
#pragma unroll
        for (int j = 0; j < 4; ++j)
          bfr[slot][j] = *(const short8_t*)(sb + b_row_off + j * 4096 + ps);
      };
      if constexpr (STAGE) {
#pragma unroll
        for (int q = 0; q < 8; ++q) stage_piece(q, snext);
      }
      rd(0, 0);
#pragma unroll
      for (int ks = 0; ks < 4; ++ks) {
        if (ks < 3) rd(ks + 1, (ks + 1) & 1);
#pragma unroll
        for (int mb = 0; mb < 2; ++mb)
#pragma unroll
          for (int j = 0; j < 4; ++j)
            acc[mb][j] = mfma32<ET>(af[ks & 1][mb], bfr[ks & 1][j], acc[mb][j]);
      }
      if constexpr (STAGE) __builtin_amdgcn_sched_group_barrier(0x020, 8, 0);
      __builtin_amdgcn_sched_group_barrier(0x100, 6, 0);
#pragma unroll
      for (int ks = 0; ks < 4; ++ks) {
        if (ks < 3) __builtin_amdgcn_sched_group_barrier(0x100, 6, 0);
        __builtin_amdgcn_sched_group_barrier(0x008, 8, 0);
      }
    } else {
#pragma unroll
      for (int sl = 0; sl < 8; ++sl) {
        const int ps = (sl ^ swl) << 4;
        f32x4_t af[2], bfr[4];
#pragma unroll
        for (int mb = 0; mb < 2; ++mb) af[mb] = *(const f32x4_t*)(sb + a_row_off + mb * 4096 + ps);
#pragma unroll
        for (int j = 0; j < 4; ++j) bfr[j] = *(const f32x4_t*)(sb + b_row_off + j * 4096 + ps);
#pragma unroll
        for (int s2 = 0; s2 < 2; ++s2) {
#pragma unroll
          for (int mb = 0; mb < 2; ++mb) {
            const float a = h ? af[mb][2 * s2 + 1] : af[mb][2 * s2];
#pragma unroll
            for (int j = 0; j < 4; ++j) {
              const float bv = h ? bfr[j][2 * s2 + 1] : bfr[j][2 * s2];
              acc[mb][j] = __builtin_amdgcn_mfma_f32_32x32x2f32(a, bv, acc[mb][j], 0, 0, 0);
            }
          }
        }
        if constexpr (STAGE) stage_piece(sl, snext);
      }
    }
  };

#pragma unroll
  for (int q = 0; q < 8; ++q) stage_piece(q, smem);
  advance();
  for (int kt = 0; kt < nk - 1; ++kt) {
    asm volatile("s_waitcnt vmcnt(0)" ::: "memory");
    __syncthreads();
    kstep(smem + (kt & 1) * 65536, std::true_type{}, smem + ((kt + 1) & 1) * 65536);
    advance();
  }
  asm volatile("s_waitcnt vmcnt(0)" ::: "memory");
  __syncthreads();
  kstep(smem + ((nk - 1) & 1) * 65536, std::false_type{}, nullptr);
  __syncthreads();
  gemm_epilogue<PREC>(p, acc, smem, tm, tn, tid, lane, r5, h, wm, wn, out_extra);
}

template <int ET, bool SPLIT, bool SHORT = false>
__device__ __forceinline__ void gemm_epilogue16(const ConvGemmParams& p, f32x4_t (&acc)[4][8], char* smem, int tm, int tn,
                                                int tid, int lane, int r4, int h4, int wm, int wn) {
  const int c_l = wn * 128 + 8 * r4;
  const int n0 = tn * 256 + c_l;
  {
    f32x4_t b0 = {0.f, 0.f, 0.f, 0.f}, b1 = b0;
    if (p.bias != nullptr) { b0 = *(const f32x4_t*)(p.bias + n0); b1 = *(const f32x4_t*)(p.bias + n0 + 4); }
    if constexpr (ET == 1) {
      const float ws = p.w_scale;
#pragma unroll
      for (int mb = 0; mb < 4; ++mb)
#pragma unroll
        for (int j = 0; j < 4; ++j) { acc[mb][j] = acc[mb][j] * ws + b0[j]; acc[mb][4 + j] = acc[mb][4 + j] * ws + b1[j]; }
    } else if (p.bias != nullptr) {
#pragma unroll
      for (int mb = 0; mb < 4; ++mb)
#pragma unroll
        for (int j = 0; j < 4; ++j) { acc[mb][j] += b0[j]; acc[mb][4 + j] += b1[j]; }
    }
  }
  constexpr bool short_l = SHORT;
  const int lane_b = short_l ? (4 * h4) / p.L : 0, lane_l = -lane_b * p.L;
  int blk_b[4], blk_l[4];
#pragma unroll
  for (int mb = 0; mb < 4; ++mb) {
    const int m0 = tm * 256 + wm * 64 + mb * 16;
    const int b = m0 / p.L;
    blk_b[mb] = b;
    blk_l[mb] = m0 - b * p.L;
  }
  auto store_row = [&](char* o, const float (&v)[8]) {
    short8_t hi, lo;
    if constexpr (ET == 1) {
      sat_check_row(p.sat, v);
#pragma unroll
      for (int jj = 0; jj < 4; ++jj) {
        const f32x2_t c = {__builtin_amdgcn_fmed3f(v[2 * jj], -65504.0f, 65504.0f),
                           __builtin_amdgcn_fmed3f(v[2 * jj + 1], -65504.0f, 65504.0f)};
        const half2_t h = __builtin_convertvector(c, half2_t);
        const short2_t hs = __builtin_bit_cast(short2_t, h);
        hi[2 * jj] = hs[0]; hi[2 * jj + 1] = hs[1];
        if constexpr (SPLIT) {
          const half2_t l = __builtin_convertvector(c - __builtin_convertvector(h, f32x2_t), half2_t);
          const short2_t ls = __builtin_bit_cast(short2_t, l);
          lo[2 * jj] = ls[0]; lo[2 * jj + 1] = ls[1];
        }
      }
    } else {
#pragma unroll
      for (int j = 0; j < 8; ++j) {
        hi[j] = (short)f2bf(v[j]);
        if constexpr (SPLIT) lo[j] = (short)f2bf(v[j] - bf2f((unsigned short)hi[j]));
      }
    }
    *(short8_t*)o = hi;
    if constexpr (SPLIT) *(short8_t*)(o + p.out_plane) = lo;
  };
  auto out_ptr = [&](int mb, int esize) {
    const long long orow = (long long)(blk_b[mb] + lane_b) * p.out_Lp + (long long)(blk_l[mb] + 4 * h4 + lane_l) * p.out_stride + p.out_off;
    return (char*)p.Out + (orow * p.ldc + p.out_coff + n0) * esize;
  };
  if (p.mode < MODE_GN_MISH) {
    const int esize = p.out_f32 ? 4 : 2;
    const long long ostep = (long long)p.out_stride * p.ldc * esize;
#pragma unroll
    for (int mb = 0; mb < 4; ++mb) {
      char* ob = out_ptr(mb, esize);
#pragma unroll
      for (int i = 0; i < 4; ++i, ob += ostep) {
        float v[8];
#pragma unroll
        for (int j = 0; j < 8; ++j) v[j] = acc[mb][j][i];
        if (p.out_f32) {
          *(f32x4_t*)ob = f32x4_t{v[0], v[1], v[2], v[3]};
          *(f32x4_t*)(ob + 16) = f32x4_t{v[4], v[5], v[6], v[7]};
        } else {
          store_row(ob, v);
        }
      }
    }
    return;
  }
  const bool has_film = p.mode == MODE_GN_MISH_FILM, has_res = p.mode == MODE_GN_MISH_RES;
  const int spt = 256 / p.L;
  const int ns = spt > 16 ? spt * 4 : 64;
  float* s_sum = (float*)smem;
  float* s_sq = s_sum + ns;
  float* s_gb = s_sq + ns;
  float* s_film = s_gb + 512;
  const bool film_direct = has_film && short_l;
  const int b_last = p.M / p.L - 1;
  for (int i = tid; i < 2 * ns; i += 512) s_sum[i] = 0.0f;
  s_gb[tid] = tid < 256 ? p.gamma[tn * 256 + tid] : p.beta[tn * 256 + tid - 256];
  if (has_film && !film_direct) {
    for (int idx = tid; idx < spt * 128; idx += 512) {
      const int sm = idx >> 7, c4 = idx & 127;
      const int b = min(tm * spt + sm, b_last);
      const float* src = p.film + (long long)b * p.film_ld + p.film_off + tn * 256 + (c4 & 63) * 4 + (c4 >> 6) * p.N;
      *(f32x4_t*)(s_film + sm * 512 + c4 * 4) = *(const f32x4_t*)src;
    }
  }
  f32x4_t rh[2], rl[2];
  const long long rstep = (long long)p.ldres * 2;
  auto fetch_film = [&](int mb) {
    const float* fr = p.film + (long long)min(blk_b[mb] + lane_b, b_last) * p.film_ld + p.film_off + n0;
    rh[0] = *(const f32x4_t*)fr; rh[1] = *(const f32x4_t*)(fr + 4);
    rl[0] = *(const f32x4_t*)(fr + p.N); rl[1] = *(const f32x4_t*)(fr + p.N + 4);
  };
  if (film_direct) fetch_film(0);
  auto fetch_res = [&](int r) {
    const long long rrow = (long long)(blk_b[r >> 2] + lane_b) * p.res_Lp + blk_l[r >> 2] + 4 * h4 + lane_l + p.res_off;
    const char* rp = (const char*)p.Res + (rrow * p.ldres + n0) * 2 + (r & 3) * rstep;
    rh[r & 1] = *(const f32x4_t*)rp;
    if constexpr (SPLIT) rl[r & 1] = *(const f32x4_t*)(rp + p.res_plane);
  };
  if (has_res) { fetch_res(0); fetch_res(1); }
  __syncthreads();
  const int gi = c_l / p.group_ch;
  const bool wide = p.group_ch >= 128;
  const float inv_cnt = 1.0f / (float)(p.group_ch * p.L);
  int slot[4];
#pragma unroll
  for (int mb = 0; mb < 4; ++mb) slot[mb] = (blk_b[mb] + lane_b - tm * spt) * 4 + gi;
  const int hsame = short_l ? (p.L == 8 ? 2 : 1) : 4;
  const bool adder = (r4 == 0 || (!wide && r4 == 8)) && (h4 & (hsame - 1)) == 0;
  auto block_sums = [&](float (&s)[4], float* cell) {
#pragma unroll
    for (int mb = 0; mb < 4; ++mb) s[mb] = dpp_add<0xB1>(s[mb]);
#pragma unroll
    for (int mb = 0; mb < 4; ++mb) s[mb] = dpp_add<0x4E>(s[mb]);
#pragma unroll
    for (int mb = 0; mb < 4; ++mb) s[mb] = dpp_add<0x141>(s[mb]);
    if (wide) {
#pragma unroll
      for (int mb = 0; mb < 4; ++mb) s[mb] = dpp_add<0x140>(s[mb]);
    }
    if (hsame >= 2) {
#pragma unroll
      for (int mb = 0; mb < 4; ++mb) s[mb] += __shfl_xor(s[mb], 16);
    }
    if (hsame == 4) {
#pragma unroll
      for (int mb = 0; mb < 4; ++mb) s[mb] += __shfl_xor(s[mb], 32);
    }
    if (adder) {
#pragma unroll
      for (int mb = 0; mb < 4; ++mb) atomicAdd(&cell[slot[mb]], s[mb]);
    }
  };
  float mean_[4], rstd_[4];
  auto pair = [&](int mb, int j, int ip) { return f32x2_t{acc[mb][j][2 * ip], acc[mb][j][2 * ip + 1]}; };
  if constexpr (!SPLIT) {
    float s[4], q[4];
#pragma unroll
    for (int mb = 0; mb < 4; ++mb) {
      f32x2_t s2 = {0.f, 0.f}, q2 = {0.f, 0.f};
#pragma unroll
      for (int j = 0; j < 8; ++j)
#pragma unroll
        for (int ip = 0; ip < 2; ++ip) {
          const f32x2_t v = pair(mb, j, ip);
          s2 += v;
          q2 = __builtin_elementwise_fma(v, v, q2);
        }
      s[mb] = s2[0] + s2[1];
      q[mb] = q2[0] + q2[1];
    }
    block_sums(s, s_sum);
    block_sums(q, s_sq);
    __syncthreads();
#pragma unroll
    for (int mb = 0; mb < 4; ++mb) {
      mean_[mb] = s_sum[slot[mb]] * inv_cnt;
      const float var = fmaxf(s_sq[slot[mb]] * inv_cnt - mean_[mb] * mean_[mb], 0.0f);
      rstd_[mb] = rsqrtf(var + p.eps);
    }
  } else {
    float s[4];
#pragma unroll
    for (int mb = 0; mb < 4; ++mb) {
      f32x2_t s2 = {0.f, 0.f};
#pragma unroll
      for (int j = 0; j < 8; ++j)
#pragma unroll
        for (int ip = 0; ip < 2; ++ip) s2 += pair(mb, j, ip);
      s[mb] = s2[0] + s2[1];
    }
    block_sums(s, s_sum);
    __syncthreads();
#pragma unroll
    for (int mb = 0; mb < 4; ++mb) {
      mean_[mb] = s_sum[slot[mb]] * inv_cnt;
      f32x2_t q2 = {0.f, 0.f};
#pragma unroll
      for (int j = 0; j < 8; ++j) {
#pragma unroll
        for (int ip = 0; ip < 2; ++ip) {
          const f32x2_t d = pair(mb, j, ip) - mean_[mb];
          q2 = __builtin_elementwise_fma(d, d, q2);
        }
        if (j & 1) __builtin_amdgcn_sched_barrier(0);
      }
      s[mb] = q2[0] + q2[1];
    }
    block_sums(s, s_sq);
    __syncthreads();
#pragma unroll
    for (int mb = 0; mb < 4; ++mb) rstd_[mb] = rsqrtf(s_sq[slot[mb]] * inv_cnt + p.eps);
  }
  const long long ostep = (long long)p.out_stride * p.ldc * 2;
#pragma unroll
  for (int mb = 0; mb < 4; ++mb) {
    float mean = mean_[mb];
    const float rstd = rstd_[mb];
    if constexpr (SPLIT) asm volatile("" : "+v"(mean));
    float ga[8], be[8], fs[8], fb[8];
    {
      const f32x4_t gam0 = *(const f32x4_t*)(s_gb + c_l), gam1 = *(const f32x4_t*)(s_gb + c_l + 4);
      const f32x4_t bet0 = *(const f32x4_t*)(s_gb + 256 + c_l), bet1 = *(const f32x4_t*)(s_gb + 256 + c_l + 4);
#pragma unroll
      for (int j = 0; j < 4; ++j) {
        ga[j] = gam0[j] * rstd; ga[4 + j] = gam1[j] * rstd;
        if constexpr (SPLIT) { be[j] = bet0[j]; be[4 + j] = bet1[j]; }
        else { be[j] = bet0[j] - mean * ga[j]; be[4 + j] = bet1[j] - mean * ga[4 + j]; }
      }
    }
    if (film_direct) {
#pragma unroll
      for (int j = 0; j < 4; ++j) { fs[j] = rh[0][j]; fs[4 + j] = rh[1][j]; fb[j] = rl[0][j]; fb[4 + j] = rl[1][j]; }
      if (mb + 1 < 4) fetch_film(mb + 1);
    } else if (has_film) {
      const float* fr = s_film + (blk_b[mb] - tm * spt) * 512 + c_l;
      const f32x4_t f0 = *(const f32x4_t*)fr, f1 = *(const f32x4_t*)(fr + 4);
      const f32x4_t f2 = *(const f32x4_t*)(fr + 256), f3 = *(const f32x4_t*)(fr + 260);
#pragma unroll
      for (int j = 0; j < 4; ++j) { fs[j] = f0[j]; fs[4 + j] = f1[j]; fb[j] = f2[j]; fb[4 + j] = f3[j]; }
    }
    char* ob = out_ptr(mb, 2);
#pragma unroll
    for (int ip = 0; ip < 2; ++ip, ob += 2 * ostep) {
      const int r = mb * 4 + 2 * ip;
      f32x2_t v[8];
      if (has_res) {
        const short8_t h0 = __builtin_bit_cast(short8_t, rh[0]), h1 = __builtin_bit_cast(short8_t, rh[1]);
#pragma unroll
        for (int j = 0; j < 8; ++j) v[j] = f32x2_t{e2f<ET>((unsigned short)h0[j]), e2f<ET>((unsigned short)h1[j])};
        if constexpr (SPLIT) {
          const short8_t l0 = __builtin_bit_cast(short8_t, rl[0]), l1 = __builtin_bit_cast(short8_t, rl[1]);
#pragma unroll
          for (int j = 0; j < 8; ++j) v[j] += f32x2_t{e2f<ET>((unsigned short)l0[j]), e2f<ET>((unsigned short)l1[j])};
        }
        if (r + 2 < 16) { fetch_res(r + 2); fetch_res(r + 3); }
      } else {
#pragma unroll
        for (int j = 0; j < 8; ++j) v[j] = f32x2_t{0.f, 0.f};
      }
#pragma unroll
      for (int j = 0; j < 8; ++j) {
        f32x2_t x = pair(mb, j, ip);
        if constexpr (SPLIT) x = (x - mean) * ga[j] + be[j];
        else x = x * ga[j] + be[j];
        x = mish2<SPLIT ? 2 : 0>(x);
        v[j] += x;
      }
      if (has_film) {
#pragma unroll
        for (int j = 0; j < 8; ++j) v[j] = v[j] * fs[j] + fb[j];
      }
      float row[8];
#pragma unroll
      for (int j = 0; j < 8; ++j) row[j] = v[j][0];
      store_row(ob, row);
#pragma unroll
      for (int j = 0; j < 8; ++j) row[j] = v[j][1];
      store_row(ob + ostep, row);
      __builtin_amdgcn_sched_barrier(0);
    }
  }
}

#ifdef HALO16_STAMP
__device__ unsigned long long g_halo_stamp[8];
extern "C" int ditree_debug_halo_stamp(unsigned long long* out) {
  return (int)hipMemcpyFromSymbol(out, HIP_SYMBOL(g_halo_stamp), sizeof(g_halo_stamp));
}
__device__ unsigned int g_x3_phase[8][32];
extern "C" int ditree_debug_x3_phase(unsigned int* out) {
  return (int)hipMemcpyFromSymbol(out, HIP_SYMBOL(g_x3_phase), sizeof(g_x3_phase));
}
#define X3_STAMP_MAX 65536
__device__ unsigned long long g_x3_stamp[X3_STAMP_MAX][6];
__device__ unsigned int g_x3_count;
extern "C" int ditree_debug_x3_stamp(unsigned long long* out, unsigned int* count, int reset) {
  int rc = (int)hipMemcpyFromSymbol(count, HIP_SYMBOL(g_x3_count), 4);
  if (rc == 0 && out != nullptr) rc = (int)hipMemcpyFromSymbol(out, HIP_SYMBOL(g_x3_stamp), sizeof(unsigned long long) * 6 * X3_STAMP_MAX);
  if (rc == 0 && reset) { unsigned int z = 0; rc = (int)hipMemcpyToSymbol(HIP_SYMBOL(g_x3_count), &z, 4); }
  return rc;
}
#endif
template <int ET, bool SPLIT>
__global__ void __launch_bounds__(512, 2) conv3_halo16_kernel(ConvGemmParams p) {
  extern __shared__ __attribute__((aligned(16))) char smem[];
  constexpr int A_BUF = 40960, W_BUF = 32768, W_BASE = 2 * A_BUF;
  const int tid = threadIdx.x, lane = tid & 63;
  const int w = __builtin_amdgcn_readfirstlane(tid >> 6);
  const int r4 = lane & 15, h4 = lane >> 4;
  const int wm = w >> 1, wn = w & 1;
  const int ntn = (p.N + 255) >> 8;
  const int ntm = (p.M + 255) >> 8;
  const int tile = xcd_remap_strips(blockIdx.x, ntm, ntn, p.dbg);
  const int tm = tile / ntn, tn = tile - tm * ntn;
  const int L = p.L, Lp = p.in_Lp, S = 256 / L;
  const int a_rows = S * Lp;
  const int nc = p.Cin >> 6;
  const int nv = SPLIT ? 3 * nc : nc;
  const int a_plane = (int)p.a_plane, w_plane = (int)p.w_plane;
  const long long K = 3LL * p.Cin;
  constexpr bool SNAKE = true;

  unsigned pa0, pa4, pbe, pbo;
  const char* const a_base = (const char*)p.A + ((long long)tm * S * Lp + p.in_off) * p.lda * 2;
  const char* const w_base = (const char*)p.W + ((long long)tn * 256) * K * 2;
  const __amdgpu_buffer_rsrc_t a_rsrc = __builtin_amdgcn_make_buffer_rsrc((void*)a_base, 0, 0x7fffffff, 0x00020000);
  const __amdgpu_buffer_rsrc_t w_rsrc = __builtin_amdgcn_make_buffer_rsrc((void*)w_base, 0, 0x7fffffff, 0x00020000);
  {
    const int r = w * 8 + (lane >> 3);
    const int slot = (lane & 7) ^ (r & 7);
    pa0 = (unsigned)((r * p.lda + slot * 8) * 2);
    const int r4r = r + 256;
    const int rs = r4r < a_rows ? r4r : a_rows - 1;
    pa4 = (unsigned)((rs * p.lda + slot * 8) * 2);
  }
  const int a_piece = 64 * p.lda * 2;
  long long wq[4];
  {
    const int lr = lane >> 3;
    const int slot0 = (lane & 7) ^ lr;
    const int slot1 = slot0;
    pbe = (unsigned)(((long long)(8 * lr) * K + slot0 * 8) * 2);
    pbo = (unsigned)(((long long)(8 * lr) * K + slot1 * 8) * 2);
#pragma unroll
    for (int q = 0; q < 4; ++q) {
      const int r0 = (w * 4 + q) * 8;
      const int cu = (r0 & 128) + 8 * (r0 & 8) + ((r0 >> 4) & 7);
      wq[q] = (long long)cu * K * 2;
    }
  }
  const int w_tap = p.Cin * 2;
  auto issue_a = [&](int v, int i) {
    int c = v, po = 0;
    if constexpr (SPLIT) { c = v / 3; po = (v - 3 * c == 2) ? a_plane : 0; }
    __builtin_amdgcn_raw_ptr_buffer_load_lds(a_rsrc, (LDS_AS void*)(smem + (v & 1) * A_BUF + (w + 8 * i) * 1024), 16,
                                             i < 4 ? pa0 : pa4, c * 128 + (i < 4 ? i * a_piece : 0) + po, 0, 0);
  };
  auto issue_w = [&](int v, int t, int q) {
    int c = v, po = 0;
    if constexpr (SPLIT) { c = v / 3; po = (v - 3 * c == 1) ? w_plane : 0; }
    __builtin_amdgcn_raw_ptr_buffer_load_lds(w_rsrc, (LDS_AS void*)(smem + W_BASE + ((v + t) & 1) * W_BUF + (w * 4 + q) * 1024),
                                             16, (q & 1) ? pbo : pbe, (int)wq[q] + c * 128 + t * w_tap + po, 0, 0);
  };

  int lrow0;
  {
    const int ml = wm * 64 + r4;
    const int sb = ml / L;
    lrow0 = sb * Lp + (ml - sb * L);
  }
  int lstep[4];
#pragma unroll
  for (int mb = 0; mb < 4; ++mb) lstep[mb] = 16 * mb + 2 * (((wm * 64 + 16 * mb) / L) - ((wm * 64) / L));
  const int swl = r4 & 7;
  const int b_row_off = (wn * 128 + r4) * 128;

  f32x4_t acc[4][8];
#pragma unroll
  for (int mb = 0; mb < 4; ++mb)
#pragma unroll
    for (int j = 0; j < 8; ++j) acc[mb][j] = f32x4_t{0.f, 0.f, 0.f, 0.f};

  short8_t af[2][4], bq[2][4];
  auto rdA = [&](int set, int c, int t, int ks) {
    const char* ab = smem + (c & 1) * A_BUF;
#pragma unroll
    for (int mb = 0; mb < 4; ++mb) {
      const int row = lrow0 + lstep[mb] + t;
      const int ps = (((ks << 2) | h4) ^ (row & 7)) << 4;
      af[set][mb] = *(const short8_t*)(ab + row * 128 + ps);
    }
  };
  auto rdB = [&](int set, int c, int t, int ks, int half) {
    const char* wb = smem + W_BASE + ((c + t) & 1) * W_BUF + b_row_off + half * 8192;
    const int psb = (((ks << 2) | h4) ^ swl) << 4;
#pragma unroll
    for (int jj = 0; jj < 4; ++jj) bq[set][jj] = *(const short8_t*)(wb + jj * 2048 + psb);
  };
  auto mm = [&](int aset, int bset, int half, int mb, int jj) {
    acc[mb][half * 4 + jj] = mfma16<ET>(af[aset][mb], bq[bset][jj], acc[mb][half * 4 + jj]);
  };
  auto mm16 = [&](int aset, int bset, int half) {
#pragma unroll
    for (int mb = 0; mb < 4; ++mb)
#pragma unroll
      for (int jj = 0; jj < 4; ++jj) mm(aset, bset, half, mb, SNAKE ? ((mb & 1) ? 3 - jj : jj) : jj);
  };

  auto step = [&](auto tT, auto tNext, auto tIW, auto tIA, auto tVM, int c) {
    constexpr int T = decltype(tT)::value;
    constexpr bool HAS_NEXT = decltype(tNext)::value, ISSUE_W = decltype(tIW)::value, ISSUE_A = decltype(tIA)::value;
    constexpr int VM = decltype(tVM)::value;
    constexpr int NV = ISSUE_W ? 4 : 0;
    asm volatile("" : "+v"(lrow0));
    __builtin_amdgcn_s_setprio(2);
    rdB(1, c, T, 0, 1);
    mm16(0, 0, 0);
    __builtin_amdgcn_sched_group_barrier(0x100, 4, 0);
    __builtin_amdgcn_sched_group_barrier(0x008, 16, 0);
    __builtin_amdgcn_sched_barrier(0);
    __builtin_amdgcn_s_setprio(1);
    rdA(1, c, T, 1);
    rdB(0, c, T, 1, 0);
    mm16(0, 1, 1);
    __builtin_amdgcn_sched_group_barrier(0x100, 8, 0);
    __builtin_amdgcn_sched_group_barrier(0x008, 16, 0);
    __builtin_amdgcn_sched_barrier(0);
    __builtin_amdgcn_s_setprio(0);
    rdB(1, c, T, 1, 1);
    mm16(1, 0, 0);
    if constexpr (ISSUE_A && T != 2) {
      if constexpr (T == 0) { issue_a(c + 1, 0); issue_a(c + 1, 1); issue_a(c + 1, 2); }
      else { issue_a(c + 1, 3); issue_a(c + 1, 4); }
      __builtin_amdgcn_sched_group_barrier(0x100, 4, 0);
      __builtin_amdgcn_sched_group_barrier(0x008, 4, 0);
      __builtin_amdgcn_sched_group_barrier(0x020, 1, 0);
      __builtin_amdgcn_sched_group_barrier(0x008, 4, 0);
      __builtin_amdgcn_sched_group_barrier(0x020, 1, 0);
      __builtin_amdgcn_sched_group_barrier(0x008, 4, 0);
      if constexpr (T == 0) __builtin_amdgcn_sched_group_barrier(0x020, 1, 0);
      __builtin_amdgcn_sched_group_barrier(0x008, 4, 0);
    } else {
      __builtin_amdgcn_sched_group_barrier(0x100, 4, 0);
      __builtin_amdgcn_sched_group_barrier(0x008, 16, 0);
    }
    __builtin_amdgcn_sched_barrier(0);
    if constexpr (HAS_NEXT) {
      if constexpr (VM == 0) asm volatile("s_waitcnt vmcnt(0) lgkmcnt(0)" ::: "memory");
      else if constexpr (VM == 3) asm volatile("s_waitcnt vmcnt(3) lgkmcnt(0)" ::: "memory");
      else asm volatile("s_waitcnt vmcnt(2) lgkmcnt(0)" ::: "memory");
      __builtin_amdgcn_s_barrier();
      __builtin_amdgcn_s_setprio(3);
      constexpr int T1 = (T + 1) % 3;
      rdA(0, c + (T + 1) / 3, T1, 0);
      rdB(0, c + (T + 1) / 3, T1, 0, 0);
    }
    constexpr int T2 = (T + 2) % 3;
    const int c2 = c + (T + 2) / 3;
#pragma unroll
    for (int mb = 0; mb < 4; ++mb)
#pragma unroll
      for (int jj = 0; jj < 4; ++jj) {
        mm(1, 1, 1, mb, SNAKE ? ((mb & 1) ? 3 - jj : jj) : jj);
        const int i = mb * 4 + jj;
        const int d = (i & 1) ? -1 : (i >> 1);
        if constexpr (ISSUE_W) { if (d >= 0 && d < 4) issue_w(c2, T2, d); }
      }
    if constexpr (HAS_NEXT) __builtin_amdgcn_sched_group_barrier(0x100, 8, 1);
#pragma unroll
    for (int i = 0; i < 16; ++i) {
      __builtin_amdgcn_sched_group_barrier(0x008, 1, 1);
      if (!(i & 1) && (i >> 1) < NV) __builtin_amdgcn_sched_group_barrier(0x020, 1, 1);
    }
    __builtin_amdgcn_sched_barrier(0);
  };
  using I0 = std::integral_constant<int, 0>;
  using I1 = std::integral_constant<int, 1>;
  using I2 = std::integral_constant<int, 2>;
  using I3 = std::integral_constant<int, 3>;
  using Tt = std::true_type;
  using Ff = std::false_type;

#pragma unroll
  for (int i = 0; i < 5; ++i) issue_a(0, i);
#pragma unroll
  for (int q = 0; q < 4; ++q) issue_w(0, 0, q);
  asm volatile("s_waitcnt vmcnt(0)" ::: "memory");
  __builtin_amdgcn_s_barrier();
#pragma unroll
  for (int q = 0; q < 4; ++q) issue_w(0, 1, q);
  rdA(0, 0, 0, 0);
  rdB(0, 0, 0, 0, 0);

#ifdef HALO16_STAMP
  const unsigned long long st0 = __builtin_amdgcn_s_memtime(), rt0 = __builtin_amdgcn_s_memrealtime();
#endif
  for (int c = 0; c < nv - 2; ++c) {
    step(I0{}, Tt{}, Tt{}, Tt{}, I3{}, c);
    step(I1{}, Tt{}, Tt{}, Tt{}, I2{}, c);
    step(I2{}, Tt{}, Tt{}, Tt{}, I0{}, c);
  }
#ifdef HALO16_STAMP
  if (blockIdx.x == 100 && tid == 0 && nv >= 32) {
    g_halo_stamp[0] = __builtin_amdgcn_s_memtime() - st0;
    g_halo_stamp[1] = __builtin_amdgcn_s_memrealtime() - rt0;
    g_halo_stamp[2] = (unsigned long long)(nv - 2) * 3;
  }
#endif
  {
    const int c = nv - 2;
    step(I0{}, Tt{}, Tt{}, Tt{}, I0{}, c);
    step(I1{}, Tt{}, Tt{}, Tt{}, I0{}, c);
    step(I2{}, Tt{}, Tt{}, Ff{}, I0{}, c);
  }
  {
    const int c = nv - 1;
    step(I0{}, Tt{}, Tt{}, Ff{}, I0{}, c);
    step(I1{}, Tt{}, Ff{}, Ff{}, I0{}, c);
    step(I2{}, Ff{}, Ff{}, Ff{}, I0{}, c);
  }
  __builtin_amdgcn_s_setprio(0);
  __syncthreads();
  gemm_epilogue16<ET, SPLIT>(p, acc, smem, tm, tn, tid, lane, r4, h4, wm, wn);
}

template <int ET, bool SHORT = false, bool SPLITK = false, int NP = 5>
__global__ void __launch_bounds__(512, 2) conv3_halo16x3_kernel(ConvGemmParams p) {
  extern __shared__ __attribute__((aligned(16))) char smem[];
  static_assert(NP == 5 || NP == 6, "five or six activation pieces");
  constexpr int A_BUF = NP * 8192, W_BUF = 32768, W_BASE = 2 * A_BUF;
  const int tid = threadIdx.x, lane = tid & 63;
  const int w = __builtin_amdgcn_readfirstlane(tid >> 6);
  const int r4 = lane & 15, h4 = lane >> 4;
  const int wm = w >> 1, wn = w & 1;
  const int ntn = (p.N + 255) >> 8;
  const int ntm = (p.M + 255) >> 8;
  const int tile = xcd_remap_strips(blockIdx.x, ntm, ntn, p.dbg);
  const int tm = tile / ntn, tn = tile - tm * ntn;
  const int L = p.L, Lp = p.in_Lp, S = 256 / L;
  const int a_rows = S * Lp;
  const int nv_all = p.Cin >> 5;
  const int v_lo = SPLITK ? (int)blockIdx.y * (nv_all / p.splitk) : 0;
  const int nv = SPLITK ? v_lo + nv_all / p.splitk : nv_all;
  const long long K = 3LL * p.Cin;
  const unsigned a_plane = (unsigned)p.a_plane, w_plane = (unsigned)p.w_plane;

  unsigned pa0, pa4, pa5 = 0, pbe, pbo;
  const char* const a_base = (const char*)p.A + ((long long)tm * S * Lp + p.in_off) * p.lda * 2;
  const char* const w_base = (const char*)p.W + ((long long)tn * 256) * K * 2;
  const __amdgpu_buffer_rsrc_t a_rsrc = __builtin_amdgcn_make_buffer_rsrc((void*)a_base, 0, 0x7fffffff, 0x00020000);
  const __amdgpu_buffer_rsrc_t w_rsrc = __builtin_amdgcn_make_buffer_rsrc((void*)w_base, 0, 0x7fffffff, 0x00020000);
  {
    const int r = w * 8 + (lane >> 3);
    const int slot = (lane & 7) ^ (r & 7);
    const unsigned po = (slot & 4) ? a_plane : 0u;
    pa0 = (unsigned)((r * p.lda + (slot & 3) * 8) * 2) + po;
    const int r4r = r + 256;
    const int rs = r4r < a_rows ? r4r : a_rows - 1;
    pa4 = (unsigned)((rs * p.lda + (slot & 3) * 8) * 2) + po;
    if constexpr (NP == 6) {
      const int r5r = r + 320;
      const int rs5 = r5r < a_rows ? r5r : a_rows - 1;
      pa5 = (unsigned)((rs5 * p.lda + (slot & 3) * 8) * 2) + po;
    }
  }
  const int a_piece = 64 * p.lda * 2;
  long long wq[4];
  {
    const int lr = lane >> 3;
    const int slot0 = (lane & 7) ^ lr;
    const int slot1 = slot0;
    pbe = (unsigned)(((long long)(8 * lr) * K + (slot0 & 3) * 8) * 2) + ((slot0 & 4) ? w_plane : 0u);
    pbo = (unsigned)(((long long)(8 * lr) * K + (slot1 & 3) * 8) * 2) + ((slot1 & 4) ? w_plane : 0u);
#pragma unroll
    for (int q = 0; q < 4; ++q) {
      const int r0 = (w * 4 + q) * 8;
      const int cu = (r0 & 128) + 8 * (r0 & 8) + ((r0 >> 4) & 7);
      wq[q] = (long long)cu * K * 2;
    }
  }
  const int w_tap = p.Cin * 2;
  auto issue_a = [&](int v, int i) {
    __builtin_amdgcn_raw_ptr_buffer_load_lds(a_rsrc, (LDS_AS void*)(smem + (v & 1) * A_BUF + (w + 8 * i) * 1024), 16,
                                             i < 4 ? pa0 : (i == 4 ? pa4 : pa5), v * 64 + (i < 4 ? i * a_piece : 0), 0, 0);
  };
  auto issue_w = [&](int v, int t, int q) {
    __builtin_amdgcn_raw_ptr_buffer_load_lds(w_rsrc, (LDS_AS void*)(smem + W_BASE + ((v + t) & 1) * W_BUF + (w * 4 + q) * 1024),
                                             16, (q & 1) ? pbo : pbe, (int)wq[q] + v * 64 + t * w_tap, 0, 0);
  };

  int lrow0;
  {
    const int ml = wm * 64 + r4;
    const int sb = ml / L;
    lrow0 = sb * Lp + (ml - sb * L);
  }
  int lstep[4];
#pragma unroll
  for (int mb = 0; mb < 4; ++mb) lstep[mb] = 16 * mb + 2 * (((wm * 64 + 16 * mb) / L) - ((wm * 64) / L));
  const int swl = r4 & 7;
  const int b_row_off = (wn * 128 + r4) * 128;

  f32x4_t acc[4][8];
#pragma unroll
  for (int mb = 0; mb < 4; ++mb)
#pragma unroll
    for (int j = 0; j < 8; ++j) acc[mb][j] = f32x4_t{0.f, 0.f, 0.f, 0.f};

  short8_t af[2][4], bq[2][4];
  auto rdA = [&](int set, int v, int t, int pl) {
    const char* ab = smem + (v & 1) * A_BUF;
#pragma unroll
    for (int mb = 0; mb < 4; ++mb) {
      const int row = lrow0 + lstep[mb] + t;
      const int ps = (((pl << 2) | h4) ^ (row & 7)) << 4;
      af[set][mb] = *(const short8_t*)(ab + row * 128 + ps);
    }
  };
  auto rdB = [&](int set, int v, int t, int pl, int half) {
    const char* wb = smem + W_BASE + ((v + t) & 1) * W_BUF + b_row_off + half * 8192;
    const int psb = (((pl << 2) | h4) ^ swl) << 4;
#pragma unroll
    for (int jj = 0; jj < 4; ++jj) bq[set][jj] = *(const short8_t*)(wb + jj * 2048 + psb);
  };
  auto mm = [&](int aset, int bset, int half, int mb, int jj) {
    acc[mb][half * 4 + jj] = mfma16<ET>(af[aset][mb], bq[bset][jj], acc[mb][half * 4 + jj]);
  };
  auto mm16 = [&](int aset, int bset, int half) {
#pragma unroll
    for (int mb = 0; mb < 4; ++mb)
#pragma unroll
      for (int jj = 0; jj < 4; ++jj) mm(aset, bset, half, mb, (mb & 1) ? 3 - jj : jj);
  };

#ifdef X3_PHASE_STAMP
  unsigned pst[24];
#define PSTAMP(k) do { pst[T * 8 + (k)] = (unsigned)__builtin_amdgcn_s_memtime(); __builtin_amdgcn_sched_barrier(0); } while (0)
#else
#define PSTAMP(k) do { } while (0)
#endif
  auto step = [&](auto tT, auto tNext, auto tIW, auto tIA, auto tVM, int v) {
    constexpr int T = decltype(tT)::value;
    constexpr bool HAS_NEXT = decltype(tNext)::value, ISSUE_W = decltype(tIW)::value, ISSUE_A = decltype(tIA)::value;
    constexpr int VM = decltype(tVM)::value;
    asm volatile("" : "+v"(lrow0));
    PSTAMP(0);
    __builtin_amdgcn_s_setprio(2);
    rdB(1, v, T, 1, 1);
    mm16(0, 0, 0);
    __builtin_amdgcn_sched_group_barrier(0x100, 4, 0);
    __builtin_amdgcn_sched_group_barrier(0x008, 16, 0);
    __builtin_amdgcn_sched_barrier(0);
    PSTAMP(1);
    rdB(0, v, T, 0, 0);
    rdA(1, v, T, 1);
    mm16(0, 1, 1);
    __builtin_amdgcn_sched_group_barrier(0x100, 8, 0);
    __builtin_amdgcn_sched_group_barrier(0x008, 16, 0);
    __builtin_amdgcn_sched_barrier(0);
    PSTAMP(2);
    __builtin_amdgcn_s_setprio(1);
    rdB(1, v, T, 0, 1);
    mm16(0, 0, 0);
    __builtin_amdgcn_sched_group_barrier(0x100, 4, 0);
    __builtin_amdgcn_sched_group_barrier(0x008, 16, 0);
    __builtin_amdgcn_sched_barrier(0);
    PSTAMP(3);
    mm16(1, 0, 0);
    if constexpr (ISSUE_A && T != 2) {
      if constexpr (T == 0) { issue_a(v + 1, 0); issue_a(v + 1, 1); issue_a(v + 1, 2); }
      else { issue_a(v + 1, 3); issue_a(v + 1, 4); if constexpr (NP == 6) issue_a(v + 1, 5); }
      __builtin_amdgcn_sched_group_barrier(0x008, 4, 2);
      __builtin_amdgcn_sched_group_barrier(0x020, 1, 2);
      __builtin_amdgcn_sched_group_barrier(0x008, 4, 2);
      __builtin_amdgcn_sched_group_barrier(0x020, 1, 2);
      __builtin_amdgcn_sched_group_barrier(0x008, 4, 2);
      if constexpr (T == 0 || NP == 6) __builtin_amdgcn_sched_group_barrier(0x020, 1, 2);
      __builtin_amdgcn_sched_group_barrier(0x008, 4, 2);
    }
    __builtin_amdgcn_sched_barrier(0);
    PSTAMP(4);
    __builtin_amdgcn_s_setprio(0);
    mm16(0, 1, 1);
    __builtin_amdgcn_sched_barrier(0);
    PSTAMP(5);
    if constexpr (HAS_NEXT) {
      if constexpr (VM == 0) asm volatile("s_waitcnt vmcnt(0) lgkmcnt(0)" ::: "memory");
      else if constexpr (VM == 3) asm volatile("s_waitcnt vmcnt(3) lgkmcnt(0)" ::: "memory");
      else asm volatile("s_waitcnt vmcnt(2) lgkmcnt(0)" ::: "memory");
      __builtin_amdgcn_s_barrier();
      __builtin_amdgcn_s_setprio(3);
      PSTAMP(6);
      constexpr int T1 = (T + 1) % 3;
      rdA(0, v + (T + 1) / 3, T1, 0);
      rdB(0, v + (T + 1) / 3, T1, 1, 0);
    }
    constexpr int T2 = (T + 2) % 3;
    const int v2 = v + (T + 2) / 3;
#pragma unroll
    for (int mb = 0; mb < 4; ++mb)
#pragma unroll
      for (int jj = 0; jj < 4; ++jj) {
        mm(1, 1, 1, mb, (mb & 1) ? 3 - jj : jj);
        const int i = mb * 4 + jj;
        const int d = (i & 1) ? -1 : (i >> 1);
        if constexpr (ISSUE_W) { if (d >= 0 && d < 4) issue_w(v2, T2, d); }
      }
    if constexpr (HAS_NEXT) __builtin_amdgcn_sched_group_barrier(0x100, 8, 1);
    constexpr int NV = ISSUE_W ? 4 : 0;
#pragma unroll
    for (int i = 0; i < 16; ++i) {
      __builtin_amdgcn_sched_group_barrier(0x008, 1, 1);
      if (!(i & 1) && (i >> 1) < NV) __builtin_amdgcn_sched_group_barrier(0x020, 1, 1);
    }
    __builtin_amdgcn_sched_barrier(0);
    PSTAMP(7);
  };
#undef PSTAMP
  using I0 = std::integral_constant<int, 0>;
  using I1 = std::integral_constant<int, 1>;
  using I2 = std::integral_constant<int, 2>;
  using I3 = std::integral_constant<int, 3>;
  using Tt = std::true_type;
  using Ff = std::false_type;

#ifdef HALO16_STAMP
  const unsigned long long xs0 = __builtin_amdgcn_s_memrealtime();
#endif
#pragma unroll
  for (int i = 0; i < NP; ++i) issue_a(v_lo, i);
#pragma unroll
  for (int q = 0; q < 4; ++q) issue_w(v_lo, 0, q);
  asm volatile("s_waitcnt vmcnt(0)" ::: "memory");
  __builtin_amdgcn_s_barrier();
#pragma unroll
  for (int q = 0; q < 4; ++q) issue_w(v_lo, 1, q);
  rdA(0, v_lo, 0, 0);
  rdB(0, v_lo, 0, 1, 0);
#ifdef HALO16_STAMP
  const unsigned long long xs1 = __builtin_amdgcn_s_memrealtime();
#endif

  using IT1 = std::integral_constant<int, NP == 6 ? 3 : 2>;
  for (int v = v_lo; v < nv - 2; ++v) {
    step(I0{}, Tt{}, Tt{}, Tt{}, I3{}, v);
    step(I1{}, Tt{}, Tt{}, Tt{}, IT1{}, v);
    step(I2{}, Tt{}, Tt{}, Tt{}, I0{}, v);
  }
#ifdef X3_PHASE_STAMP
  if (blockIdx.x == 100 && lane == 0 && nv == 64) {
#pragma unroll
    for (int k = 0; k < 24; ++k) g_x3_phase[w][k] = pst[k];
    g_x3_phase[w][24] = (unsigned)nv;
  }
#endif
  {
    const int v = nv - 2;
    step(I0{}, Tt{}, Tt{}, Tt{}, I0{}, v);
    step(I1{}, Tt{}, Tt{}, Tt{}, I0{}, v);
    step(I2{}, Tt{}, Tt{}, Ff{}, I0{}, v);
  }
  {
    const int v = nv - 1;
    step(I0{}, Tt{}, Tt{}, Ff{}, I0{}, v);
    step(I1{}, Tt{}, Ff{}, Ff{}, I0{}, v);
    step(I2{}, Ff{}, Ff{}, Ff{}, I0{}, v);
  }
  __builtin_amdgcn_s_setprio(0);
  __syncthreads();
#ifdef HALO16_STAMP
  const unsigned long long xs2 = __builtin_amdgcn_s_memrealtime();
#endif
  if constexpr (SPLITK) {
    const int ntiles = ntm * ntn;
    float* mine = p.sk_ws + ((size_t)blockIdx.y * ntiles + tile) * 65536;
#pragma unroll
    for (int mb = 0; mb < 4; ++mb)
#pragma unroll
      for (int j = 0; j < 8; ++j) *(f32x4_t*)(mine + ((mb * 8 + j) * 512 + tid) * 4) = acc[mb][j];
    __threadfence();
    __syncthreads();
    int* s_last = (int*)smem;
    if (tid == 0) *s_last = atomicAdd(p.sk_cnt + tile, 1) == p.splitk - 1;
    __syncthreads();
    const bool last = *s_last != 0;
    __syncthreads();
    if (!last) return;
    __threadfence();
#pragma unroll
    for (int mb = 0; mb < 4; ++mb)
#pragma unroll
      for (int j = 0; j < 8; ++j) acc[mb][j] = f32x4_t{0.f, 0.f, 0.f, 0.f};
    for (int sp = 0; sp < p.splitk; ++sp) {
      const float* sl = p.sk_ws + ((size_t)sp * ntiles + tile) * 65536;
#pragma unroll
      for (int mb = 0; mb < 4; ++mb)
#pragma unroll
        for (int j = 0; j < 8; ++j) acc[mb][j] += *(const f32x4_t*)(sl + ((mb * 8 + j) * 512 + tid) * 4);
    }
    if (tid == 0) p.sk_cnt[tile] = 0;
  }
  gemm_epilogue16<ET, true, SHORT>(p, acc, smem, tm, tn, tid, lane, r4, h4, wm, wn);
#ifdef HALO16_STAMP
  __syncthreads();
  if (tid == 0) {
    const unsigned long long xs3 = __builtin_amdgcn_s_memrealtime();
    const unsigned int k = atomicAdd(&g_x3_count, 1u);
    if (k < X3_STAMP_MAX) {
      g_x3_stamp[k][0] = xs0; g_x3_stamp[k][1] = xs1; g_x3_stamp[k][2] = xs2; g_x3_stamp[k][3] = xs3;
      g_x3_stamp[k][4] = ((unsigned long long)nv << 32) | blockIdx.x;
      g_x3_stamp[k][5] = ((unsigned long long)__builtin_amdgcn_s_getreg((31 << 11) | 20) << 32) |
                         (unsigned int)__builtin_amdgcn_s_getreg((31 << 11) | 4);
    }
  }
#endif
}

template <int ET, bool SPLIT>
__global__ void __launch_bounds__(256) conv2d_small_kernel(ConvGemmParams p) {
  extern __shared__ __attribute__((aligned(16))) char smem[];
  constexpr int STAGE = 16384;
  constexpr int CK = SPLIT ? 32 : 64;
  const int tid = threadIdx.x, lane = tid & 63;
  const int w = __builtin_amdgcn_readfirstlane(tid >> 6);
  const int r5 = lane & 31, h = lane >> 5;
  const int wm = w >> 1, wn = w & 1;
  const int ntn = p.N >> 6;
  const int tm = blockIdx.x / ntn, tn = blockIdx.x - tm * ntn;
  const int kpt = p.Cin / CK;
  const long long K = (long long)p.taps * p.Cin;
  int k0 = 0, nk = p.taps * kpt;
  long long out_extra = 0;
  if (p.splitk > 1) {
    const int per = (nk + p.splitk - 1) / p.splitk;
    k0 = blockIdx.y * per;
    nk = min(nk - k0, per);
    out_extra = (long long)blockIdx.y * p.slab_stride;
  }

  const char* a_base[2];
  int ih0[2], iw0[2];
  const char* w_src[2];
  int slot_b[2];
  long long plane_a[2];
#pragma unroll
  for (int q = 0; q < 2; ++q) {
    const int r = (2 * w + q) * 8 + (lane >> 3);
    const int slot = (lane & 7) ^ ((r >> 1) & 7);
    slot_b[q] = SPLIT ? (slot & 3) * 16 : slot * 16;
    plane_a[q] = (SPLIT && (slot & 4)) ? p.a_plane : 0;
    const long long plane_w = (SPLIT && (slot & 4)) ? p.w_plane : 0;
    int m = tm * 64 + r;
    m = m < p.M ? m : p.M - 1;
    const int b = m / p.c2_OHW, rem = m - b * p.c2_OHW;
    const int oh = rem / p.c2_OW, ow = rem - oh * p.c2_OW;
    a_base[q] = (const char*)p.A + (long long)b * p.c2_H * p.c2_W * p.Cin * 2;
    ih0[q] = oh * p.c2_stride - p.c2_pad;
    iw0[q] = ow * p.c2_stride - p.c2_pad;
    w_src[q] = (const char*)p.W + ((long long)(tn * 64 + r) * K) * 2 + slot_b[q] + plane_w;
  }
  auto issue = [&](int kl) {
    const int k = k0 + kl;
    const int tap = k / kpt, kin = k - tap * kpt;
    const int kh = p.c2_kh[tap], kw = p.c2_kw[tap];
    char* st = smem + (kl % 3) * STAGE;
#pragma unroll
    for (int q = 0; q < 2; ++q) {
      const int ih = ih0[q] + kh, iw = iw0[q] + kw;
      const bool ok = ih >= 0 && ih < p.c2_H && iw >= 0 && iw < p.c2_W;
      const char* src = ok ? a_base[q] + ((long long)(ih * p.c2_W + iw) * p.Cin + kin * CK) * 2 + plane_a[q] : (const char*)p.zero;
      __builtin_amdgcn_global_load_lds((const GLOBAL_AS void*)(src + slot_b[q]), (LDS_AS void*)(st + (2 * w + q) * 1024), 16, 0, 0);
    }
#pragma unroll
    for (int q = 0; q < 2; ++q)
      __builtin_amdgcn_global_load_lds((const GLOBAL_AS void*)(w_src[q] + (long long)k * (CK * 2)),
                                       (LDS_AS void*)(st + 8192 + (2 * w + q) * 1024), 16, 0, 0);
  };

  f32x16_t acc;
#pragma unroll
  for (int i = 0; i < 16; ++i) acc[i] = 0.0f;
  const int a_row = wm * 32 + r5, b_row = wn * 32 + r5;
  const int a_off = a_row * 128, b_off = 8192 + b_row * 128;
  const int sa = (a_row >> 1) & 7, sb = (b_row >> 1) & 7;

  issue(0);
  if (nk > 1) issue(1);
  for (int k = 0; k < nk; ++k) {
    if (k + 1 < nk) asm volatile("s_waitcnt vmcnt(4)" ::: "memory");
    else asm volatile("s_waitcnt vmcnt(0)" ::: "memory");
    __builtin_amdgcn_s_barrier();
    if (k + 2 < nk) issue(k + 2);
    const char* st = smem + (k % 3) * STAGE;
    if constexpr (SPLIT) {
      short8_t af[4], bf[4];
#pragma unroll
      for (int ks = 0; ks < 4; ++ks) {
        af[ks] = *(const short8_t*)(st + a_off + ((((ks << 1) | h) ^ sa) << 4));
        bf[ks] = *(const short8_t*)(st + b_off + ((((ks << 1) | h) ^ sb) << 4));
      }
#pragma unroll
      for (int kk = 0; kk < 2; ++kk) acc = mfma32<ET>(af[kk], bf[kk + 2], acc);
#pragma unroll
      for (int kk = 0; kk < 2; ++kk) acc = mfma32<ET>(af[kk], bf[kk], acc);
#pragma unroll
      for (int kk = 0; kk < 2; ++kk) acc = mfma32<ET>(af[kk + 2], bf[kk], acc);
    } else {
#pragma unroll
      for (int ks = 0; ks < 4; ++ks) {
        const short8_t af = *(const short8_t*)(st + a_off + ((((ks << 1) | h) ^ sa) << 4));
        const short8_t bf = *(const short8_t*)(st + b_off + ((((ks << 1) | h) ^ sb) << 4));
        acc = mfma32<ET>(af, bf, acc);
      }
    }
    asm volatile("s_waitcnt lgkmcnt(0)" ::: "memory");
  }

  const int n = tn * 64 + wn * 32 + r5;
  float bias = (p.bias != nullptr && k0 == 0) ? p.bias[n] : 0.0f;
#pragma unroll
  for (int i = 0; i < 16; ++i) {
    const int m = tm * 64 + wm * 32 + (i & 3) + 8 * (i >> 2) + 4 * h;
    if (m < p.M) ((float*)p.Out)[out_extra + (long long)m * p.ldc + p.out_coff + n] = (ET == 1 ? acc[i] * p.w_scale : acc[i]) + bias;
  }
}

template <int ET, bool SPLIT, bool SHORT = false>
__global__ void __launch_bounds__(512, 2) gemm16_kernel(ConvGemmParams p) {
  extern __shared__ __attribute__((aligned(16))) char smem[];
  constexpr int BUF = 32768, W_BASE = 2 * BUF;
  const int tid = threadIdx.x, lane = tid & 63;
  const int w = __builtin_amdgcn_readfirstlane(tid >> 6);
  const int r4 = lane & 15, h4 = lane >> 4;
  const int wm = w >> 1, wn = w & 1;
  const int ntn = p.N >> 8, ntm = p.M >> 8;
  const int tile = xcd_remap_strips(blockIdx.x, ntm, ntn, p.dbg);
  const int tm = tile / ntn, tn = tile - tm * ntn;
  constexpr int KB = SPLIT ? 64 : 128;
  const int nc = SPLIT ? (p.Cin >> 5) : (p.Cin >> 6), nk = p.taps * nc;
  const unsigned a_plane = (unsigned)p.a_plane, w_plane = (unsigned)p.w_plane;
  const long long K = (long long)p.taps * p.Cin;

  long long a_tile0;
  {
    const int m0 = tm * 256;
    const int b0 = m0 / p.L, l0 = m0 - b0 * p.L;
    a_tile0 = (((long long)b0 * p.in_Lp + (long long)l0 * p.in_stride + p.in_off) * p.lda) * 2;
  }
  const __amdgpu_buffer_rsrc_t a_rsrc =
      __builtin_amdgcn_make_buffer_rsrc((void*)((const char*)p.A + a_tile0), 0, 0x7fffffff, 0x00020000);
  const __amdgpu_buffer_rsrc_t w_rsrc =
      __builtin_amdgcn_make_buffer_rsrc((void*)((const char*)p.W + ((long long)tn * 256) * K * 2), 0, 0x7fffffff, 0x00020000);
  unsigned pae, pao, pbe, pbo;
  int aq[4], wq[4];
  {
// ... 93 lines not shown
        __builtin_amdgcn_sched_group_barrier(0x008, 8, 0);
      } else
      {
      __builtin_amdgcn_sched_group_barrier(0x100, 4, 0);
      __builtin_amdgcn_sched_group_barrier(0x008, 16, 0);
      }
      __builtin_amdgcn_sched_barrier(0);
      rdB(0, k, 0, 0);
      rdA(1, k, 1);
      mm16(0, 1, 1);
      if constexpr (HAS_NEXT) {
        issue_wq(k + 1, 2); issue_wq(k + 1, 3);
        __builtin_amdgcn_sched_group_barrier(0x100, 8, 0);
        __builtin_amdgcn_sched_group_barrier(0x008, 4, 0);
        __builtin_amdgcn_sched_group_barrier(0x020, 1, 0);
        __builtin_amdgcn_sched_group_barrier(0x008, 4, 0);
        __builtin_amdgcn_sched_group_barrier(0x020, 1, 0);
        __builtin_amdgcn_sched_group_barrier(0x008, 8, 0);
      } else
      {
      __builtin_amdgcn_sched_group_barrier(0x100, 8, 0);
      __builtin_amdgcn_sched_group_barrier(0x008, 16, 0);
      }
      __builtin_amdgcn_sched_barrier(0);
      rdB(1, k, 0, 1);
      mm16(0, 0, 0);
      __builtin_amdgcn_sched_group_barrier(0x100, 4, 0);
      __builtin_amdgcn_sched_group_barrier(0x008, 16, 0);
      __builtin_amdgcn_sched_barrier(0);
      mm16(1, 0, 0);
      __builtin_amdgcn_sched_barrier(0);
      mm16(0, 1, 1);
      __builtin_amdgcn_sched_barrier(0);
    } else {
      rdB(1, k, 0, 1);
      mm16(0, 0, 0);
      __builtin_amdgcn_sched_group_barrier(0x100, 4, 0);
      __builtin_amdgcn_sched_group_barrier(0x008, 16, 0);
      __builtin_amdgcn_sched_barrier(0);
      rdA(1, k, 1);
      rdB(0, k, 1, 0);
      mm16(0, 1, 1);
      __builtin_amdgcn_sched_group_barrier(0x100, 8, 0);
      __builtin_amdgcn_sched_group_barrier(0x008, 16, 0);
      __builtin_amdgcn_sched_barrier(0);
      rdB(1, k, 1, 1);
      mm16(1, 0, 0);
      __builtin_amdgcn_sched_group_barrier(0x100, 4, 0);
      __builtin_amdgcn_sched_group_barrier(0x008, 16, 0);
      __builtin_amdgcn_sched_barrier(0);
    }
    int ao2 = 0, wo2 = 0;
    if constexpr (ISSUE) src_off(k + 2, ao2, wo2);
    if constexpr (HAS_NEXT) {
      asm volatile("s_waitcnt vmcnt(0) lgkmcnt(0)" ::: "memory");
      __builtin_amdgcn_s_barrier();
      rdA(0, k + 1, 0);
      rdB(0, k + 1, SPLIT ? 1 : 0, 0);
    }
#pragma unroll
    for (int mb = 0; mb < 4; ++mb)
#pragma unroll
      for (int jj = 0; jj < 4; ++jj) {
        mm(1, 1, 1, mb, (mb & 1) ? 3 - jj : jj);
        if constexpr (ISSUE) {
          const int m = mb * 4 + jj, i = (m & 1) ? -1 : (m >> 1);
          if (i >= 0 && i < 4)
            __builtin_amdgcn_raw_ptr_buffer_load_lds(a_rsrc, (LDS_AS void*)(smem + (k & 1) * BUF + (w * 4 + i) * 1024), 16,
                                                     (i & 1) ? pao : pae, aq[i] + ao2, 0, 0);
          else if (!SPLIT && i >= 4 && i < 8)
            __builtin_amdgcn_raw_ptr_buffer_load_lds(w_rsrc, (LDS_AS void*)(smem + W_BASE + (k & 1) * BUF + (w * 4 + i - 4) * 1024),
                                                     16, ((i - 4) & 1) ? pbo : pbe, wq[i - 4] + wo2, 0, 0);
        }
      }
    if constexpr (HAS_NEXT) __builtin_amdgcn_sched_group_barrier(0x100, 8, 1);
#pragma unroll
    for (int i = 0; i < 16; ++i) {
      __builtin_amdgcn_sched_group_barrier(0x008, 1, 1);
      if (ISSUE && !(i & 1) && (!SPLIT || i < 8)) __builtin_amdgcn_sched_group_barrier(0x020, 1, 1);
    }
    __builtin_amdgcn_sched_barrier(0);
  };
  using Tt = std::true_type;
  using Ff = std::false_type;

  issue(0);
  asm volatile("s_waitcnt vmcnt(0)" ::: "memory");
  __builtin_amdgcn_s_barrier();
  if (nk > 1) {
    if constexpr (SPLIT) {
      int ao, wo;
      src_off(1, ao, wo);
#pragma unroll
      for (int q = 0; q < 4; ++q)
        __builtin_amdgcn_raw_ptr_buffer_load_lds(a_rsrc, (LDS_AS void*)(smem + BUF + (w * 4 + q) * 1024), 16, (q & 1) ? pao : pae,
                                                 aq[q] + ao, 0, 0);
    } else {
      issue(1);
    }
  }
  rdA(0, 0, 0);
  rdB(0, 0, SPLIT ? 1 : 0, 0);
  for (int k = 0; k < nk - 2; ++k) step(Tt{}, Tt{}, k);
  if (nk >= 2) step(Tt{}, Ff{}, nk - 2);
  step(Ff{}, Ff{}, nk - 1);
  __syncthreads();
  gemm_epilogue16<ET, SPLIT, SHORT>(p, acc, smem, tm, tn, tid, lane, r4, h4, wm, wn);
}
static bool gemm16_eligible(const ConvGemmParams& p, int fmt) {
  const bool short_ok = p.L == 8 || p.L == 4;
  return fmt_st(fmt) != ST_F32 && !p.c2d && (!p.out_f32 || p.mode == MODE_BIAS) && p.taps >= 1 && p.taps <= 3 && (p.M & 255) == 0 &&
         (p.N & 255) == 0 && (p.Cin & 63) == 0 && ((p.L & 15) == 0 || short_ok) && p.M > 0 &&
         (p.mode == MODE_BIAS || (256 % p.L) == 0);
}
static bool halo_eligible(const ConvGemmParams& p, int fmt) {
  static const bool l8_off = [] { const char* e = getenv("DITREE_HALO_L8"); return e && atoi(e) == 0; }();
  static const bool l4_off = [] { const char* e = getenv("DITREE_HALO_L4"); return e && atoi(e) == 0; }();
  const bool l_ok = p.L >= 16 || (p.L == 8 && fmt_split(fmt) && !l8_off) || (p.L == 4 && fmt_split(fmt) && !l4_off && p.splitk <= 1);
  return fmt_st(fmt) != ST_F32 && !p.c2d && p.taps == 3 && p.in_stride == 1 && p.in_Lp == p.L + 2 && (256 % p.L) == 0 &&
         l_ok && (p.M & 255) == 0 && (p.N & 255) == 0 && (p.Cin & 63) == 0 && p.Cin >= 192;
}
bool conv2d_small_eligible(int fmt) { return fmt_st(fmt) != ST_F32; }
int conv_gemm_kind(const ConvGemmParams& p, int fmt) { return halo_eligible(p, fmt) ? 0 : (p.c2d ? 2 : 1); }
bool conv_gemm_supported(const ConvGemmParams& p, int fmt) {
  return !fmt_split(fmt) || halo_eligible(p, fmt) || gemm16_eligible(p, fmt) ||
         (p.c2d && (p.N & 63) == 0 && (p.Cin & 63) == 0 && p.out_f32 && p.mode == MODE_BIAS);
}

static void ensure_lds_attrs() {
  static bool done[64] = {};
  int dev = 0;
  hipGetDevice(&dev);
  if (dev < 0 || dev >= 64 || done[dev]) return;
  done[dev] = true;
  const hipFuncAttribute at = hipFuncAttributeMaxDynamicSharedMemorySize;
  hipFuncSetAttribute((const void*)conv_gemm_kernel<0, false>, at, 131072);
  hipFuncSetAttribute((const void*)conv_gemm_kernel<1, false>, at, 131072);
  hipFuncSetAttribute((const void*)conv_gemm_kernel<2, false>, at, 131072);
  hipFuncSetAttribute((const void*)conv_gemm_kernel<0, true>, at, 131072);
  hipFuncSetAttribute((const void*)conv_gemm_kernel<1, true>, at, 131072);
  hipFuncSetAttribute((const void*)conv_gemm_kernel<2, true>, at, 131072);
  hipFuncSetAttribute((const void*)conv3_halo16_kernel<0, false>, at, 147456);
  hipFuncSetAttribute((const void*)conv3_halo16_kernel<1, false>, at, 147456);
  hipFuncSetAttribute((const void*)conv3_halo16x3_kernel<0>, at, 147456);
  hipFuncSetAttribute((const void*)conv3_halo16x3_kernel<1>, at, 147456);
  hipFuncSetAttribute((const void*)conv3_halo16x3_kernel<0, true>, at, 147456);
  hipFuncSetAttribute((const void*)conv3_halo16x3_kernel<1, true>, at, 147456);
  hipFuncSetAttribute((const void*)conv3_halo16x3_kernel<0, false, true>, at, 147456);
  hipFuncSetAttribute((const void*)conv3_halo16x3_kernel<1, false, true>, at, 147456);
  hipFuncSetAttribute((const void*)conv3_halo16x3_kernel<0, true, true>, at, 147456);
  hipFuncSetAttribute((const void*)conv3_halo16x3_kernel<1, true, true>, at, 147456);
  hipFuncSetAttribute((const void*)conv3_halo16x3_kernel<0, true, false, 6>, at, 163840);
  hipFuncSetAttribute((const void*)conv3_halo16x3_kernel<1, true, false, 6>, at, 163840);
  hipFuncSetAttribute((const void*)gemm16_kernel<0, false>, at, 131072);
  hipFuncSetAttribute((const void*)gemm16_kernel<1, false>, at, 131072);
  hipFuncSetAttribute((const void*)gemm16_kernel<0, true>, at, 131072);
  hipFuncSetAttribute((const void*)gemm16_kernel<1, true>, at, 131072);
  hipFuncSetAttribute((const void*)gemm16_kernel<0, false, true>, at, 131072);
  hipFuncSetAttribute((const void*)gemm16_kernel<1, false, true>, at, 131072);
  hipFuncSetAttribute((const void*)gemm16_kernel<0, true, true>, at, 131072);
  hipFuncSetAttribute((const void*)gemm16_kernel<1, true, true>, at, 131072);
}

void launch_conv_gemm(const ConvGemmParams& p, int fmt, hipStream_t s) {
  ensure_lds_attrs();
  const int st = fmt_st(fmt);
  const bool split = fmt_split(fmt), f16 = st == ST_F16;
  const int ntn = (p.N + 255) >> 8, ntm = (p.M + 255) >> 8;
  const dim3 grid(ntm * ntn), block(512);
  if (halo_eligible(p, fmt)) {
    if (split && p.splitk > 1) {
      if (p.sk_ws == nullptr || p.sk_cnt == nullptr || ((p.Cin >> 5) % p.splitk) != 0 || (p.Cin >> 5) / p.splitk < 2)
        throw std::runtime_error("conv_gemm: split-K of the halo kernel needs its workspace and splitk | Cin / 32, >= 2 chunks each");
      const dim3 gsk(ntm * ntn, p.splitk);
      if (p.L == 8) {
        if (f16) DN_LAUNCH((conv3_halo16x3_kernel<1, true, true>), gsk, block, 147456, s, p);
        else DN_LAUNCH((conv3_halo16x3_kernel<0, true, true>), gsk, block, 147456, s, p);
      } else if (f16) DN_LAUNCH((conv3_halo16x3_kernel<1, false, true>), gsk, block, 147456, s, p);
      else DN_LAUNCH((conv3_halo16x3_kernel<0, false, true>), gsk, block, 147456, s, p);
      return;
    }
    if (split && p.L == 4) {
      if (f16) DN_LAUNCH((conv3_halo16x3_kernel<1, true, false, 6>), grid, block, 163840, s, p);
      else DN_LAUNCH((conv3_halo16x3_kernel<0, true, false, 6>), grid, block, 163840, s, p);
      return;
    }
    if (split) {
      if (p.L == 8) {
        if (f16) DN_LAUNCH((conv3_halo16x3_kernel<1, true>), grid, block, 147456, s, p);
        else DN_LAUNCH((conv3_halo16x3_kernel<0, true>), grid, block, 147456, s, p);
      } else if (f16) DN_LAUNCH(conv3_halo16x3_kernel<1>, grid, block, 147456, s, p);
      else DN_LAUNCH(conv3_halo16x3_kernel<0>, grid, block, 147456, s, p);
    } else {
      if (f16) DN_LAUNCH((conv3_halo16_kernel<1, false>), grid, block, 147456, s, p);
      else DN_LAUNCH((conv3_halo16_kernel<0, false>), grid, block, 147456, s, p);
    }
    return;
  }
  if (gemm16_eligible(p, fmt) && (p.L & 15) != 0) {
    if (split) {
      if (f16) DN_LAUNCH((gemm16_kernel<1, true, true>), grid, block, 131072, s, p);
      else DN_LAUNCH((gemm16_kernel<0, true, true>), grid, block, 131072, s, p);
    } else {
      if (f16) DN_LAUNCH((gemm16_kernel<1, false, true>), grid, block, 131072, s, p);
      else DN_LAUNCH((gemm16_kernel<0, false, true>), grid, block, 131072, s, p);
    }
    return;
  }
  if (gemm16_eligible(p, fmt)) {
    if (split) {
      if (f16) DN_LAUNCH((gemm16_kernel<1, true>), grid, block, 131072, s, p);
      else DN_LAUNCH((gemm16_kernel<0, true>), grid, block, 131072, s, p);
    } else {
      if (f16) DN_LAUNCH((gemm16_kernel<1, false>), grid, block, 131072, s, p);
      else DN_LAUNCH((gemm16_kernel<0, false>), grid, block, 131072, s, p);
    }
    return;
  }
  if (p.mode >= MODE_GN_MISH && (p.L & 15) != 0)
    throw std::runtime_error("conv_gemm: a fused GroupNorm epilogue at L = 8 / 4 exists on the gemm16 tile only (whole 256-row tiles)");
  if (p.c2d && conv2d_small_eligible(fmt) && (p.N & 63) == 0 && (p.Cin & 63) == 0 && p.out_f32 && p.mode == MODE_BIAS) {
    const dim3 g2(((p.M + 63) >> 6) * (p.N >> 6), p.splitk > 1 ? p.splitk : 1);
    if (split) {
      if (f16) DN_LAUNCH((conv2d_small_kernel<1, true>), g2, dim3(256), 3 * 16384, s, p);
      else DN_LAUNCH((conv2d_small_kernel<0, true>), g2, dim3(256), 3 * 16384, s, p);
    } else {
      if (f16) DN_LAUNCH((conv2d_small_kernel<1, false>), g2, dim3(256), 3 * 16384, s, p);
      else DN_LAUNCH((conv2d_small_kernel<0, false>), g2, dim3(256), 3 * 16384, s, p);
    }
    return;
  }
  if (split) throw std::runtime_error("conv_gemm: a split GEMM of this shape fits no tile (conv_gemm_supported is the contract)");
  if (p.c2d) {
    const dim3 grid2(ntm * ntn, p.splitk > 1 ? p.splitk : 1);
    if (st == ST_F32) DN_LAUNCH((conv_gemm_kernel<1, true>), grid2, block, 131072, s, p);
    else if (f16) DN_LAUNCH((conv_gemm_kernel<2, true>), grid2, block, 131072, s, p);
    else DN_LAUNCH((conv_gemm_kernel<0, true>), grid2, block, 131072, s, p);
    return;
  }
  if (st == ST_F32) DN_LAUNCH((conv_gemm_kernel<1, false>), grid, block, 131072, s, p);
  else if (f16) DN_LAUNCH((conv_gemm_kernel<2, false>), grid, block, 131072, s, p);
  else DN_LAUNCH((conv_gemm_kernel<0, false>), grid, block, 131072, s, p);
}

template <int FMT>
__device__ __forceinline__ void store_elem(void* base, long long idx, float v, long long plane = 0) {
  constexpr int ST = FMT & 3;
  if constexpr (ST == ST_F32) {
    ((float*)base)[idx] = v;
  } else {
    constexpr int ET = ST == ST_F16 ? 1 : 0;
    const unsigned short hi = f2e<ET>(v);
    ((unsigned short*)base)[idx] = hi;
    if constexpr ((FMT & 4) != 0) ((unsigned short*)((char*)base + plane))[idx] = f2e<ET>(v - e2f<ET>(hi));
  }
}
template <int FMT>
__device__ __forceinline__ void store_elem(void* base, long long idx, float v, long long plane, float& satm) {
  if constexpr ((FMT & 3) == ST_F16) sat_see(satm, v);
  store_elem<FMT>(base, idx, v, plane);
}
template <int FMT>
__device__ __forceinline__ float load_elem(const void* base, long long idx, long long plane = 0) {
  constexpr int ST = FMT & 3;
  if constexpr (ST == ST_F32) {
    return ((const float*)base)[idx];
  } else {
    constexpr int ET = ST == ST_F16 ? 1 : 0;
    float v = e2f<ET>(((const unsigned short*)base)[idx]);
    if constexpr ((FMT & 4) != 0) v += e2f<ET>(((const unsigned short*)((const char*)base + plane))[idx]);
    return v;
  }
}
#define MISH_OF(FMT) mish_f<((FMT) == ST_BF16 || (FMT) == ST_F16) ? 0 : 1>
#define DISPATCH_FMT(fmt, CALL)                                   \
  switch (fmt) {                                                  \
    case 0: CALL(0); break;                                       \
    case 1: CALL(1); break;                                       \
    case 2: CALL(2); break;                                       \
    case 4: CALL(4); break;                                       \
    case 6: CALL(6); break;                                       \
    default: throw std::runtime_error("denoiser kernels: unknown activation format"); \
  }
#define DISPATCH_ST(fmt, CALL)                                    \
  switch (fmt) {                                                  \
    case 0: CALL(0); break;                                       \
    case 1: CALL(1); break;                                       \
    case 2: CALL(2); break;                                       \
    default: throw std::runtime_error("denoiser kernels: unknown activation format"); \
  }

template <int PREC>
__global__ void __launch_bounds__(256) gn1d_kernel(void* __restrict__ x, int ld, int Lp, int row_off, int coff, int L, int C,
                                                   const float* __restrict__ gamma, const float* __restrict__ beta, float eps,
                                                   int mode, const float* __restrict__ film, int film_ld, int film_off,
                                                   const void* __restrict__ res, int ldres, int res_Lp, int res_off,
                                                   long long x_plane, long long res_plane, int* __restrict__ sat) {
  __shared__ float red[8];
  float satm = 0.0f;
  const int b = blockIdx.x >> 3, g = blockIdx.x & 7;
  const int gc = C >> 3, vpr = gc >> 3, nvec = L * vpr;
  const int tid = threadIdx.x, lane = tid & 63, wv = tid >> 6;
  auto at = [&](int v, int& l, int& c) { l = v / vpr; c = g * gc + (v - l * vpr) * 8; };
  auto load8 = [&](int l, int c, float (&o)[8]) {
    const long long idx = ((long long)b * Lp + l + row_off) * ld + coff + c;
#pragma unroll
    for (int j = 0; j < 8; ++j) o[j] = load_elem<PREC>(x, idx + j, x_plane);
  };
  auto wg_sum = [&](float v) {
#pragma unroll
    for (int m = 32; m >= 1; m >>= 1) v += __shfl_xor(v, m);
    __syncthreads();
    if (lane == 0) red[wv] = v;
    __syncthreads();
    return (red[0] + red[1]) + (red[2] + red[3]);
  };
  float s = 0.f;
  for (int v = tid; v < nvec; v += 256) {
    int l, c; at(v, l, c);
    float o[8]; load8(l, c, o);
#pragma unroll
    for (int j = 0; j < 8; ++j) s += o[j];
// ... 164 lines not shown
    s_map[i] = (r >= 0 && r < N && cc >= 0 && cc < N) ? lm[(size_t)b * (N * N) + r * N + cc] : 0.0f;
  }
  float w[49];
#pragma unroll
  for (int k = 0; k < 49; ++k) w[k] = W[k * 64 + c];
  __syncthreads();
  float v[J];
  float sum = 0.f;
#pragma unroll
  for (int j = 0; j < J; ++j) {
    const int p = q + 4 * j, oh = p / OH, ow = p - oh * OH;
    const float* m0 = s_map + (oh * 2) * PD + ow * 2;
    float a = 0.f;
#pragma unroll
    for (int kh = 0; kh < 7; ++kh)
#pragma unroll
      for (int kw = 0; kw < 7; ++kw) a = fmaf(w[kh * 7 + kw], m0[kh * PD + kw], a);
    v[j] = a;
    sum += a;
  }
  sum += __shfl_xor(sum, 1); sum += __shfl_xor(sum, 2); sum += __shfl_xor(sum, 4); sum += __shfl_xor(sum, 8);
  if ((c & 15) == 0) s_red[0][q][g] = sum;
  __syncthreads();
  constexpr float inv_n = 1.0f / (float)(NP * 16);
  const float mean = ((s_red[0][0][g] + s_red[0][1][g]) + (s_red[0][2][g] + s_red[0][3][g])) * inv_n;
  float sq = 0.f;
#pragma unroll
  for (int j = 0; j < J; ++j) { const float d = v[j] - mean; sq = fmaf(d, d, sq); }
  sq += __shfl_xor(sq, 1); sq += __shfl_xor(sq, 2); sq += __shfl_xor(sq, 4); sq += __shfl_xor(sq, 8);
  if ((c & 15) == 0) s_red[1][q][g] = sq;
  __syncthreads();
  const float var = ((s_red[1][0][g] + s_red[1][1][g]) + (s_red[1][2][g] + s_red[1][3][g])) * inv_n;
  const float rstd = rsqrtf(var + eps);
  const float ga = gamma[c] * rstd, be = beta[c] - mean * ga;
#pragma unroll
  for (int j = 0; j < J; ++j) {
    float y = fmaf(v[j], ga, be);
    y = y > 0.f ? y : 0.f;
    if constexpr (PREC == ST_BF16) y = bf2f(f2bf(y));
    if constexpr (PREC == ST_F16) y = h2f(f2h(y));
    s_act[(q + 4 * j) * 64 + c] = y;
  }
  __syncthreads();
  for (int o = tid; o < PH * PH * 64; o += 256) {
    const int oc = o & 63, op = o >> 6, oh = op / PH, ow = op - oh * PH;
    float best = -__builtin_huge_valf();
#pragma unroll
    for (int kh = 0; kh < 3; ++kh)
#pragma unroll
      for (int kw = 0; kw < 3; ++kw) {
        const int ih = oh * 2 + kh - 1, iw = ow * 2 + kw - 1;
        if (ih >= 0 && ih < OH && iw >= 0 && iw < OH) best = fmaxf(best, s_act[(ih * OH + iw) * 64 + oc]);
      }
    store_elem<PREC>(out, (long long)b * (PH * PH * 64) + o, best, plane, satm);
  }
  if constexpr ((PREC & 3) == ST_F16) sat_flush(sat, satm);
}
void launch_encoder_stem(const float* lm, int n, const float* W, const float* gamma, const float* beta, void* out, int B, float eps,
                         int fmt, long long plane, hipStream_t s, int* sat) {
  if (n != 20 && n != 16) throw std::runtime_error("encoder stem: local map must be 20 x 20 or 16 x 16");
#define CALL(F)                                                                                                                    \
  do {                                                                                                                             \
    if (n == 20) DN_LAUNCH((encoder_stem_kernel<F, 20>), dim3(B), dim3(256), 0, s, lm, W, gamma, beta, out, eps, plane, sat);  \
    else DN_LAUNCH((encoder_stem_kernel<F, 16>), dim3(B), dim3(256), 0, s, lm, W, gamma, beta, out, eps, plane, sat);          \
  } while (0)
  DISPATCH_FMT(fmt, CALL)
#undef CALL
}

template <int PREC>
__global__ void prep_sample_kernel(const float* __restrict__ x, void* __restrict__ A0, int B, int P, int D, long long plane,
                                   int* __restrict__ sat) {
  const long long row = blockIdx.x * (long long)(blockDim.x >> 6) + (threadIdx.x >> 6);
  const int lane = threadIdx.x & 63;
  if (row >= (long long)B * P) return;
  const int b = (int)(row / P), l = (int)(row - (long long)b * P);
  float v = 0.f;
  if (lane < 3 * D) {
    const int t = lane / D, d = lane - t * D;
    const int ls = l + t - 1;
    if (ls >= 0 && ls < P) v = x[((long long)b * P + ls) * D + d];
  }
  float satm = 0.0f;
  store_elem<PREC>(A0, row * 64 + lane, v, plane, satm);
  if constexpr ((PREC & 3) == ST_F16) sat_flush(sat, satm);
}
void launch_prep_sample(const float* x, void* A0, int B, int P, int D, int fmt, long long plane, hipStream_t s, int* sat) {
  long long rows = (long long)B * P;
  dim3 grid((unsigned)((rows + 3) / 4)), block(256);
#define CALL(F) DN_LAUNCH(prep_sample_kernel<F>, grid, block, 0, s, x, A0, B, P, D, plane, sat)
  DISPATCH_FMT(fmt, CALL)
#undef CALL
}

__global__ void __launch_bounds__(1024) time_embed_kernel(float t, const float* __restrict__ W1, const float* __restrict__ b1,
                                                          const float* __restrict__ W2, const float* __restrict__ b2,
                                                          float* __restrict__ out ) {
  __shared__ float emb[256];
  __shared__ float hid[1024];
  const int tid = threadIdx.x;
  if (tid < 256) {
    const int half = 128;
    const float wlog = logf(10000.0f) / (float)(half - 1);
    const int k = tid & 127;
    const float f = expf((float)k * -wlog);
    const float a = t * f;
    emb[tid] = (tid < 128) ? sinf(a) : cosf(a);
  }
  __syncthreads();
  {
    float s = b1[tid];
    const float* wr = W1 + (long long)tid * 256;
    for (int k = 0; k < 256; ++k) s += wr[k] * emb[k];
    hid[tid] = mish_f<1>(s);
  }
  __syncthreads();
  if (tid < 256) {
    float s = b2[tid];
    const float* wr = W2 + (long long)tid * 1024;
    for (int k = 0; k < 1024; ++k) s += wr[k] * hid[k];
    out[tid] = s;
  }
}
void launch_time_embed(float t, const float* W1, const float* b1, const float* W2, const float* b2, float* out,
                       hipStream_t s) {
  DN_LAUNCH(time_embed_kernel, dim3(1), dim3(1024), 0, s, t, W1, b1, W2, b2, out);
}

template <int PREC>
__global__ void prep_cond_kernel(const float* __restrict__ temb, const float* __restrict__ map_emb, int E, int E_ld,
                                 const float* __restrict__ cond, int G, void* __restrict__ out, int B, int Kpad, long long plane,
                                 int* __restrict__ sat) {
  const int b = blockIdx.x;
  float satm = 0.0f;
  for (int k = threadIdx.x; k < Kpad; k += blockDim.x) {
    float v = 0.f;
    bool live = true;
    if (k < 256) v = temb[k];
    else if (k < 256 + E) v = map_emb[(long long)b * E_ld + (k - 256)];
    else if (k < 256 + E + G) v = cond[(long long)b * G + (k - 256 - E)];
    else live = false;
    store_elem<PREC>(out, (long long)b * Kpad + k, live ? MISH_OF(PREC)(v) : 0.f, plane, satm);
  }
  if constexpr ((PREC & 3) == ST_F16) sat_flush(sat, satm);
}
void launch_prep_cond(const float* temb, const float* map_emb, int E, int E_ld, const float* cond, int G, void* out, int B,
                      int Kpad, int fmt, long long plane, hipStream_t s, int* sat) {
#define CALL(F) DN_LAUNCH(prep_cond_kernel<F>, dim3(B), dim3(256), 0, s, temb, map_emb, E, E_ld, cond, G, out, B, Kpad, plane, sat)
  DISPATCH_FMT(fmt, CALL)
#undef CALL
}

struct ActNormArg { double mu[8], sg[8]; };
template <int PREC, int D>
__global__ void __launch_bounds__(256) final_proj_flow_kernel(const void* __restrict__ Y, int C, int Lp, long long plane,
                                                              const float* __restrict__ W ,
                                                              const float* __restrict__ bias,
                                                              float* __restrict__ x , FlowStep fs,
                                                              ActNormArg nm, double* __restrict__ actions, int B, int P) {
  const long long pos = blockIdx.x * 4LL + (threadIdx.x >> 6);
  const int lane = threadIdx.x & 63;
  if (pos >= (long long)B * P) return;
  const int b = (int)(pos / P), l = (int)(pos - (long long)b * P);
  const long long row = (long long)b * Lp + l + 1;
  float s[D];
#pragma unroll
  for (int d = 0; d < D; ++d) s[d] = 0.f;
  for (int c = lane * 8; c < C; c += 512) {
    float y[8];
    if constexpr ((PREC & 3) == ST_F32) {
      const f32x4_t y0 = *(const f32x4_t*)((const float*)Y + row * C + c), y1 = *(const f32x4_t*)((const float*)Y + row * C + c + 4);
#pragma unroll
      for (int j = 0; j < 4; ++j) { y[j] = y0[j]; y[4 + j] = y1[j]; }
    } else {
      constexpr int ET = (PREC & 3) == ST_F16 ? 1 : 0;
      const short8_t yv = *(const short8_t*)((const unsigned short*)Y + row * C + c);
#pragma unroll
      for (int j = 0; j < 8; ++j) y[j] = e2f<ET>((unsigned short)yv[j]);
      if constexpr ((PREC & 4) != 0) {
        const short8_t yl = *(const short8_t*)((const unsigned short*)((const char*)Y + plane) + row * C + c);
#pragma unroll
        for (int j = 0; j < 8; ++j) y[j] += e2f<ET>((unsigned short)yl[j]);
      }
    }
#pragma unroll
    for (int d = 0; d < D; ++d) {
      const f32x4_t w0 = *(const f32x4_t*)(W + (long long)d * C + c), w1 = *(const f32x4_t*)(W + (long long)d * C + c + 4);
#pragma unroll
      for (int j = 0; j < 4; ++j) { s[d] = fmaf(y[j], w0[j], s[d]); }
#pragma unroll
      for (int j = 0; j < 4; ++j) { s[d] = fmaf(y[4 + j], w1[j], s[d]); }
    }
  }
#pragma unroll
  for (int d = 0; d < D; ++d) {
#pragma unroll
    for (int m = 32; m >= 1; m >>= 1) s[d] += __shfl_xor(s[d], m);
  }
  if (lane < D) {
    float sv = s[0];
    double sg = nm.sg[0], mu = nm.mu[0];
#pragma unroll
    for (int d = 1; d < D; ++d) if (lane == d) { sv = s[d]; sg = nm.sg[d]; mu = nm.mu[d]; }
    const float v = sv + bias[lane];
    const long long xi = pos * D + lane;
    float xn;
    if (fs.mode == 0) {
      xn = x[xi] + v * fs.dt;
    } else if (fs.mode == 1) {
      xn = v;
    } else {
      const float xc = x[xi];
      float x0 = (xc - fs.sb * v) / fs.sa;
      x0 = fminf(fmaxf(x0, -1.0f), 1.0f);
      xn = fs.c0 * x0 + fs.c1 * xc;
      if (fs.sigma != 0.0f) {
        const long long zr = fs.z_idx ? (long long)fs.z_idx[b] : (long long)fs.z_row0 + b;
        xn += fs.sigma * fs.z[zr * fs.z_row + (long long)l * D + lane];
      }
    }
    x[xi] = xn;
    if (actions != nullptr) actions[xi] = (double)xn * sg + mu;
  }
}
void launch_final_proj_flow(const void* Y, int C, int Lp, long long plane, const float* W, const float* bias, int D, float* x,
                            FlowStep fs, const double* act_norm, double* actions, int B, int P, int fmt, hipStream_t s) {
  long long pos = (long long)B * P;
  dim3 grid((unsigned)((pos + 3) / 4)), block(256);
  ActNormArg nm{};
  for (int d = 0; d < D && d < 8; ++d) { nm.mu[d] = act_norm[d]; nm.sg[d] = act_norm[D + d]; }
#define CALLD(F, DD) DN_LAUNCH((final_proj_flow_kernel<F, DD>), grid, block, 0, s, Y, C, Lp, plane, W, bias, x, fs, nm, actions, B, P)
#define CALL(F) do { if (D == 2) CALLD(F, 2); else if (D == 8) CALLD(F, 8); else throw std::runtime_error("final projection: action_dim must be 2 or 8"); } while (0)
  DISPATCH_FMT(fmt, CALL)
#undef CALL
#undef CALLD
}

template <int PREC, bool SRC_F32>
__global__ void im2col2d_kernel(const void* __restrict__ in, void* __restrict__ out, int B, int H, int W, int C,
                                TapList taps, int stride, int pad, int OH, int OW, int Kpad) {
  const long long row = blockIdx.x;
  const int ow = (int)(row % OW), oh = (int)((row / OW) % OH), b = (int)(row / ((long long)OW * OH));
  const int K = taps.n * C;
  for (int k = threadIdx.x; k < Kpad; k += blockDim.x) {
    float v = 0.f;
    if (k < K) {
      const int c = k % C, kk = k / C;
      const int ih = oh * stride + taps.kh[kk] - pad, iw = ow * stride + taps.kw[kk] - pad;
      if (ih >= 0 && ih < H && iw >= 0 && iw < W) {
        const long long idx = (((long long)b * H + ih) * W + iw) * C + c;
        v = SRC_F32 ? ((const float*)in)[idx] : load_elem<PREC>(in, idx);
      }
    }
    store_elem<PREC>(out, row * Kpad + k, v);
  }
}
void launch_im2col2d(const void* in, bool src_f32, void* out, int B, int H, int W, int C, const TapList& taps, int stride,
                     int pad, int OH, int OW, int Kpad, int fmt, hipStream_t s) {
  dim3 grid((unsigned)((long long)B * OH * OW)), block(Kpad >= 256 ? 256 : 64);
#define CALL(F) do { if (src_f32) DN_LAUNCH((im2col2d_kernel<F, true>), grid, block, 0, s, in, out, B, H, W, C, taps, stride, pad, OH, OW, Kpad); \
                     else DN_LAUNCH((im2col2d_kernel<F, false>), grid, block, 0, s, in, out, B, H, W, C, taps, stride, pad, OH, OW, Kpad); } while (0)
  DISPATCH_ST(fmt, CALL)
#undef CALL
}

#define GN2D_MAXP 7
template <int PREC>
__global__ void __launch_bounds__(256) gn2d_kernel(const float* __restrict__ in, int nslab, long long slab_stride,
                                                   const float* __restrict__ gamma, const float* __restrict__ beta,
                                                   const void* __restrict__ res, int relu, void* __restrict__ out, int HW,
                                                   int C, float eps, long long res_plane, long long out_plane, int* __restrict__ sat) {
  float satm = 0.0f;
  __shared__ float red[2][64];
  const int b = blockIdx.x, tid = threadIdx.x;
  const int T = C >> 2, PP = 256 / T, G = C >> 4;
  const int tpos = tid / T, tc = tid - tpos * T, grp = tc >> 2;
  const long long base = (long long)b * HW * C + 4 * tc;
  f32x4_t v[GN2D_MAXP];
  float s = 0.f;
#pragma unroll
  for (int k = 0; k < GN2D_MAXP; ++k) {
    const int pos = k * PP + tpos;
    f32x4_t x = {0.f, 0.f, 0.f, 0.f};
    if (pos < HW) {
      const float* src = in + base + (long long)pos * C;
      for (int sl = 0; sl < nslab; ++sl) {
        const f32x4_t t = *(const f32x4_t*)(src + sl * slab_stride);
        x += t;
      }
      s += (x[0] + x[1]) + (x[2] + x[3]);
    }
    v[k] = x;
  }
  s += __shfl_xor(s, 1);
  s += __shfl_xor(s, 2);
  if ((tc & 3) == 0) red[0][tpos * G + grp] = s;
  __syncthreads();
  float tot = 0.f;
  for (int q = 0; q < PP; ++q) tot += red[0][q * G + grp];
  const float inv_n = 1.0f / (float)(HW * 16);
  const float mean = tot * inv_n;
  float q2 = 0.f;
#pragma unroll
  for (int k = 0; k < GN2D_MAXP; ++k) {
    if (k * PP + tpos < HW) {
#pragma unroll
      for (int j = 0; j < 4; ++j) { const float d = v[k][j] - mean; q2 = fmaf(d, d, q2); }
    }
  }
  q2 += __shfl_xor(q2, 1);
  q2 += __shfl_xor(q2, 2);
  if ((tc & 3) == 0) red[1][tpos * G + grp] = q2;
  __syncthreads();
  float var = 0.f;
  for (int q = 0; q < PP; ++q) var += red[1][q * G + grp];
  const float rstd = rsqrtf(var * inv_n + eps);
  const f32x4_t ga = *(const f32x4_t*)(gamma + 4 * tc), be = *(const f32x4_t*)(beta + 4 * tc);
#pragma unroll
  for (int k = 0; k < GN2D_MAXP; ++k) {
    const int pos = k * PP + tpos;
    if (pos >= HW) continue;
    const long long idx = base + (long long)pos * C;
    float y[4];
#pragma unroll
    for (int j = 0; j < 4; ++j) y[j] = (v[k][j] - mean) * rstd * ga[j] + be[j];
    constexpr int ET = (PREC & 3) == ST_F16 ? 1 : 0;
    if (res != nullptr) {
      if constexpr ((PREC & 3) == ST_F32) {
        const f32x4_t r = *(const f32x4_t*)((const float*)res + idx);
#pragma unroll
        for (int j = 0; j < 4; ++j) y[j] += r[j];
      } else {
        const short4_t r = *(const short4_t*)((const unsigned short*)res + idx);
        if constexpr ((PREC & 4) != 0) {
          const short4_t rl = *(const short4_t*)((const unsigned short*)((const char*)res + res_plane) + idx);
#pragma unroll
          for (int j = 0; j < 4; ++j) y[j] += e2f<ET>((unsigned short)r[j]) + e2f<ET>((unsigned short)rl[j]);
        } else {
#pragma unroll
          for (int j = 0; j < 4; ++j) y[j] += e2f<ET>((unsigned short)r[j]);
        }
      }
    }
    if (relu) {
#pragma unroll
      for (int j = 0; j < 4; ++j) y[j] = y[j] > 0.f ? y[j] : 0.f;
    }
    if constexpr ((PREC & 3) == ST_F32) {
      const f32x4_t o = {y[0], y[1], y[2], y[3]};
      *(f32x4_t*)((float*)out + idx) = o;
    } else {
      short4_t o;
      if constexpr (ET == 1) { sat_see2(satm, y[0], y[1]); sat_see2(satm, y[2], y[3]); }
#pragma unroll
      for (int j = 0; j < 4; ++j) o[j] = (short)f2e<ET>(y[j]);
      *(short4_t*)((unsigned short*)out + idx) = o;
      if constexpr ((PREC & 4) != 0) {
        short4_t o2;
#pragma unroll
        for (int j = 0; j < 4; ++j) o2[j] = (short)f2e<ET>(y[j] - e2f<ET>((unsigned short)o[j]));
        *(short4_t*)((unsigned short*)((char*)out + out_plane) + idx) = o2;
      }
    }
  }
  if constexpr ((PREC & 3) == ST_F16) sat_flush(sat, satm);
}
void launch_gn2d(const float* in, int nslab, long long slab_stride, const float* gamma, const float* beta, const void* res,
                 int relu, void* out, int B, int HW, int C, float eps, int fmt, long long res_plane, long long out_plane,
                 hipStream_t s, int* sat) {
  if (C < 64 || C > 1024 || (C & (C - 1)) != 0 || (HW + 256 / (C >> 2) - 1) / (256 / (C >> 2)) > GN2D_MAXP)
    throw std::runtime_error("encoder GroupNorm: unsupported map shape");
  dim3 grid((unsigned)B), block(256);
#define CALL(F) DN_LAUNCH(gn2d_kernel<F>, grid, block, 0, s, in, nslab, slab_stride, gamma, beta, res, relu, out, HW, C, eps, \
                                   res_plane, out_plane, sat)
  DISPATCH_FMT(fmt, CALL)
#undef CALL
// ... 66 lines not shown
```

Measured before the change: 18790 candidate expansions/s.

## Fuse first residual conv and final projection into halo conv GEMM epilogues

Adds two fused epilogue modes to the halo conv3 kernels. In the first mode, the 1x1 residual conv of the first down block (input dim 2) is computed in the epilogue straight from x_cur, which removes a separate GEMM launch and its residual buffer. In the second mode, the final conv's GroupNorm+Mish output is projected onto the action dims inside the epilogue and written as per-tile partial sums, so final.h is never materialised. A small kernel then reduces those partials and applies the flow step. This is on by default for D=2 with non-f32 formats. It adds kernel variants and shared-memory use, and it drops the debug buffers for the fused layers.

```diff
diff --git a/ditreeonlineplanner_amd/csrc/denoise.h b/ditreeonlineplanner_amd/csrc/denoise.h
--- a/ditreeonlineplanner_amd/csrc/denoise.h
+++ b/ditreeonlineplanner_amd/csrc/denoise.h
@@ -2,7 +2,8 @@
 #include <hip/hip_runtime.h>
 #include <stdint.h>
 
-enum { MODE_BIAS = 0, MODE_GN_MISH = 1, MODE_GN_MISH_FILM = 2, MODE_GN_MISH_RES = 3 };
+enum { MODE_BIAS = 0, MODE_GN_MISH = 1, MODE_GN_MISH_FILM = 2, MODE_GN_MISH_RES = 3,
+       MODE_GN_MISH_RES_IN = 4, MODE_GN_MISH_PROJ = 5 };
 
 enum { ST_BF16 = 0, ST_F32 = 1, ST_F16 = 2 };
 static inline int fmt_make(int st, bool split) { return st | (split ? 4 : 0); }
@@ -46,6 +47,11 @@
   float* sk_ws;
   int* sk_cnt;
   int* sat;
+  const float* res_x;
+  const float* res_w;
+  const float* res_b;
+  const float* proj_w;
+  float* proj_ws;
 };
 
 void denoise_set_dry_run(bool on);
@@ -68,6 +74,8 @@
   const int* z_idx;
   int z_row0;
 };
+void launch_final_partial_flow(const float* parts, int nparts, const float* bias, int D, float* x, FlowStep fs,
+                               const double* act_norm, double* actions, int B, int P, hipStream_t s);
 void launch_final_proj_flow(const void* Y, int C, int Lp, long long plane, const float* W, const float* bias, int D, float* x,
                             FlowStep fs, const double* act_norm , double* actions, int B, int P, int fmt,
                             hipStream_t s);
diff --git a/ditreeonlineplanner_amd/csrc/denoise_host.hip b/ditreeonlineplanner_amd/csrc/denoise_host.hip
--- a/ditreeonlineplanner_amd/csrc/denoise_host.hip
+++ b/ditreeonlineplanner_amd/csrc/denoise_host.hip
@@ -91,6 +91,9 @@
   long long cond_plane = 0;
   int condK = 0, film_cols = 0;
   Act final_h;
+  bool fused_ends = false;
+  float* proj_ws = nullptr;
+  int proj_parts = 0;
   const float* lm_ptr = nullptr;
   void* zero_row = nullptr;
   static constexpr int SAT_SLOTS = 256;
@@ -130,6 +133,7 @@
   int pick_splitk(const ConvGemmParams& p, int fmt) {
     const char* e = getenv("DITREE_DENOISE_SPLITK");
     if (!e || atoi(e) == 0 || !fmt_split(fmt) || p.L == 4 || conv_gemm_kind(p, fmt) != 0) return 1;
+    if (p.mode == MODE_GN_MISH_RES_IN || p.mode == MODE_GN_MISH_PROJ) return 1;
     const int tiles = (p.M >> 8) * (p.N >> 8), nvc = p.Cin >> 5;
     int sk = 1;
     static const int cap = [] { const char* c = getenv("DITREE_DENOISE_SPLITK_WGS"); return c ? atoi(c) : 64; }();
@@ -236,6 +240,9 @@
     film_op = nullptr;
     sat_flags = sat_cond = sat_sample = nullptr;
     sat_names.clear();
+    fused_ends = false;
+    proj_ws = nullptr;
+    proj_parts = 0;
     prec = -1;
     Bmax = 0;
     Buser = 0;
@@ -338,7 +345,8 @@
   const char* aptr(const Act& a) const { return (const char*)a.p + (size_t)a.coff * es(); }
 
   void add_conv3(std::vector<std::function<void(int, int, hipStream_t)>>& ops, const std::string& wname, const Act& in,
-                 const Act& out, int mode, const std::string& gn, int film_off, const Act* res) {
+                 const Act& out, int mode, const std::string& gn, int film_off, const Act* res, const float* end_w = nullptr,
+                 const float* end_b = nullptr) {
     const HostParam& w = P_(wname + ".weight");
     const int Cout = (int)w.dims[0], Cin = (int)w.dims[1];
     const float* wd = w.data;
@@ -356,6 +364,8 @@
     if (mode == MODE_GN_MISH_RES) {
       p.Res = aptr(*res); p.ldres = res->ld; p.res_Lp = res->Lp(); p.res_off = res->padded ? 1 : 0; p.res_plane = res->plane;
     }
+    if (mode == MODE_GN_MISH_RES_IN) { p.res_x = x_cur; p.res_w = end_w; p.res_b = end_b; }
+    if (mode == MODE_GN_MISH_PROJ) { p.Out = nullptr; p.sat = nullptr; p.proj_w = end_w; p.proj_ws = proj_ws; }
     emit_block(ops, p, out, in.L);
   }
   void emit_block(std::vector<std::function<void(int, int, hipStream_t)>>& ops, const ConvGemmParams& p, const Act& out, int L) {
@@ -366,6 +376,8 @@
     const bool fused = mode < MODE_GN_MISH ||
                        ((Cout & 255) == 0 && (gch == 64 || gch == 128 || gch == 256) && ((L & 15) == 0 || short_fusable));
     const bool fused_needs_tiles = fused && mode >= MODE_GN_MISH && (L & 15) != 0;
+    if ((mode == MODE_GN_MISH_RES_IN || mode == MODE_GN_MISH_PROJ) && (!fused || fused_needs_tiles))
+      throw std::runtime_error("a fused end of the network needs the fused GroupNorm epilogue at 16 | L");
     ConvGemmParams qf = p, q = p;
     q.mode = MODE_BIAS;
     const float* film_p = p.film;
@@ -463,6 +475,14 @@
     add_conv3(unet_ops, pre + ".blocks.1.block.0", h, out, MODE_GN_MISH_RES, pre + ".blocks.1.block.1", 0, &res);
   }
 
+  void final_step(const FlowStep& fs, const double* act_norm, double* actions, int B, hipStream_t s) {
+    if (fused_ends)
+      launch_final_partial_flow(proj_ws, proj_parts, dev_f["unet.final_conv.1.bias"], D, x_cur, fs, act_norm, actions, B, P, s);
+    else
+      launch_final_proj_flow(final_h.p, final_h.C, final_h.Lp(), final_h.plane, dev_f["unet.final_conv.1.weight"],
+                             dev_f["unet.final_conv.1.bias"], D, x_cur, fs, act_norm, actions, B, P, ufmt, s);
+  }
+
   void build(int prec_, int Bmax_);
 };
 
@@ -497,6 +517,16 @@
   if (fmt_split(ufmt) && ((C0 | C1 | C2) & 255) != 0)
     throw std::runtime_error("the split precisions need down_dims that are multiples of 256 (halo / gemm16 tiles)");
   x_cur = (float*)dalloc((size_t)Bmax * P * D * 4);
+  {
+    const char* e = getenv("DITREE_FUSE_ENDS");
+    const int gch = C0 / 8;
+    fused_ends = !(e && atoi(e) == 0) && D == 2 && fmt_st(ufmt) != ST_F32 && (C0 & 255) == 0 && (gch == 64 || gch == 128 || gch == 256) &&
+                 has("unet.down_modules.0.0.residual_conv.weight");
+    if (fused_ends) {
+      proj_parts = C0 / 128;
+      proj_ws = (float*)dalloc((size_t)Bmax * P * proj_parts * D * 4);
+    }
+  }
   temb = (float*)dalloc(256 * 4);
   condK = (cond_dim + 63) / 64 * 64;
   const int Brows = (Bmax + 255) / 256 * 256;
@@ -574,6 +604,11 @@
     p.film = film; p.film_ld = film_cols; p.film_off = film_offs[0];
     const int L = L0;
     emit_block(unet_ops, p, h, L0);
+    if (fused_ends) {
+      Act o = make_act("d0b1.out", L0, C0);
+      add_conv3(unet_ops, pre + ".blocks.1.block.0", h, o, MODE_GN_MISH_RES_IN, pre + ".blocks.1.block.1", 0, nullptr,
+                vec(pre + ".residual_conv.weight"), vec(pre + ".residual_conv.bias"));
+    } else {
     const HostParam& wr = P_(pre + ".residual_conv.weight");
     const float* wrd = wr.data;
     const Packed wrp = pack(pre + ".residual_conv", ufmt, C0, 1, 64, [=](int n, int, int ci) {
@@ -590,6 +625,7 @@
     unet_ops.push_back([this, q, L, uf](int, int Bp, hipStream_t s) mutable { q.M = Bp * L; run_gemm(q, uf, s); });
     Act o = make_act("d0b1.out", L0, C0);
     add_conv3(unet_ops, pre + ".blocks.1.block.0", h, o, MODE_GN_MISH_RES, pre + ".blocks.1.block.1", 0, &res);
+    }
     fc = film_offs[1];
   }
   Act cat1 = make_act("cat1", L1, 2 * C1);
@@ -629,8 +665,15 @@
   add_crb("unet.up_modules.1.1", u1a, u1b, fc, "u1b2");
   Act fin = make_act("final.in", L0, C0);
   add_up(unet_ops, "unet.up_modules.1.2.conv", u1b, fin);
-  final_h = make_act("final.h", L0, C0);
-  add_conv3(unet_ops, "unet.final_conv.0.block.0", fin, final_h, MODE_GN_MISH, "unet.final_conv.0.block.1", 0, nullptr);
+  if (fused_ends) {
+    final_h = fin;
+    final_h.p = nullptr;
+    add_conv3(unet_ops, "unet.final_conv.0.block.0", fin, final_h, MODE_GN_MISH_PROJ, "unet.final_conv.0.block.1", 0, nullptr,
+              vec("unet.final_conv.1.weight"));
+  } else {
+    final_h = make_act("final.h", L0, C0);
+    add_conv3(unet_ops, "unet.final_conv.0.block.0", fin, final_h, MODE_GN_MISH, "unet.final_conv.0.block.1", 0, nullptr);
+  }
   vec("unet.final_conv.1.weight");
   vec("unet.final_conv.1.bias");
   vec("unet.diffusion_step_encoder.1.weight");
@@ -943,6 +986,8 @@
       for (auto& op : enc_ops) op(0, bgran, 0, nullptr);
       film_op(bgran, bgran, nullptr);
       for (auto& op : unet_ops) op(bgran, bgran, nullptr);
+      const double unit_norm[16] = {0, 0, 0, 0, 0, 0, 0, 0, 1, 1, 1, 1, 1, 1, 1, 1};
+      final_step(FlowStep{}, unit_norm, nullptr, bgran, nullptr);
     } catch (...) {
       denoise_set_dry_run(false);
       lm_ptr = nullptr;
@@ -1151,9 +1196,7 @@
       fs.z_row = st->ddpm_z_row; fs.z_idx = noise_idx; fs.z_row0 = st->ddpm_row0;
       if (fs.sigma != 0.0f && !fs.z) return set_err(ctx, DITREE_E_ARG, "denoise: a DDPM step with sigma > 0 needs step noise");
     }
-    launch_final_proj_flow(st->final_h.p, st->final_h.C, st->final_h.Lp(), st->final_h.plane, st->dev_f["unet.final_conv.1.weight"],
-                           st->dev_f["unet.final_conv.1.bias"], st->D, st->x_cur, fs, act_norm,
-                           (last && actions) ? actions : nullptr, B, st->P, uf, s);
+    st->final_step(fs, act_norm, (last && actions) ? actions : nullptr, B, s);
   }
   } catch (const std::exception& e) {
     return set_err(ctx, DITREE_E_ARG, std::string("denoise: ") + e.what());
@@ -1364,6 +1407,8 @@
     dims3[0] = B; dims3[1] = 1; dims3[2] = cols;
     return DITREE_OK;
   }
+  if (st->fused_ends && (nm == "final.h" || nm == "d0b1.res"))
+    return set_err(ctx, DITREE_E_STATE, "debug_read: " + nm + " does not exist in a fused plan (bind with DITREE_FUSE_ENDS=0 to keep it)");
   auto it = st->named.find(nm);
   if (it == st->named.end()) return set_err(ctx, DITREE_E_ARG, "debug_read: unknown buffer " + nm);
   const Act& a = it->second;
diff --git a/ditreeonlineplanner_amd/csrc/denoise_kernels.hip b/ditreeonlineplanner_amd/csrc/denoise_kernels.hip
--- a/ditreeonlineplanner_amd/csrc/denoise_kernels.hip
+++ b/ditreeonlineplanner_amd/csrc/denoise_kernels.hip
@@ -557,9 +557,10 @@
   gemm_epilogue<PREC>(p, acc, smem, tm, tn, tid, lane, r5, h, wm, wn, out_extra);
 }
 
-template <int ET, bool SPLIT, bool SHORT = false>
+template <int ET, bool SPLIT, bool SHORT = false, int EPI = 0>
 __device__ __forceinline__ void gemm_epilogue16(const ConvGemmParams& p, f32x4_t (&acc)[4][8], char* smem, int tm, int tn,
                                                 int tid, int lane, int r4, int h4, int wm, int wn) {
+  static_assert(EPI == 0 || !SHORT, "the fused ends exist for 16 | L only");
   const int c_l = wn * 128 + 8 * r4;
   const int n0 = tn * 256 + c_l;
   {
@@ -619,7 +620,7 @@
     const long long orow = (long long)(blk_b[mb] + lane_b) * p.out_Lp + (long long)(blk_l[mb] + 4 * h4 + lane_l) * p.out_stride + p.out_off;
     return (char*)p.Out + (orow * p.ldc + p.out_coff + n0) * esize;
   };
-  if (p.mode < MODE_GN_MISH) {
+  if (EPI == 0 && p.mode < MODE_GN_MISH) {
     const int esize = p.out_f32 ? 4 : 2;
     const long long ostep = (long long)p.out_stride * p.ldc * esize;
 #pragma unroll
@@ -640,7 +641,7 @@
     }
     return;
   }
-  const bool has_film = p.mode == MODE_GN_MISH_FILM, has_res = p.mode == MODE_GN_MISH_RES;
+  const bool has_film = EPI == 0 && p.mode == MODE_GN_MISH_FILM, has_res = EPI == 0 && p.mode == MODE_GN_MISH_RES;
   const int spt = 256 / p.L;
   const int ns = spt > 16 ? spt * 4 : 64;
   float* s_sum = (float*)smem;
@@ -651,6 +652,15 @@
   const int b_last = p.M / p.L - 1;
   for (int i = tid; i < 2 * ns; i += 512) s_sum[i] = 0.0f;
   s_gb[tid] = tid < 256 ? p.gamma[tn * 256 + tid] : p.beta[tn * 256 + tid - 256];
+  float* s_rw = s_film;
+  float* s_rb = s_film + 512;
+  float* s_x = s_film + 768;
+  if constexpr (EPI == 1) {
+    s_rw[tid] = p.res_w[tn * 512 + tid];
+    if (tid < 256) s_rb[tid] = p.res_b[tn * 256 + tid];
+    else if (tid < 384) *(f32x4_t*)(s_x + (tid - 256) * 4) = *(const f32x4_t*)(p.res_x + (long long)tm * 512 + (tid - 256) * 4);
+  }
+  if constexpr (EPI == 2) s_rw[tid] = p.proj_w[(long long)(tid >> 8) * p.N + tn * 256 + (tid & 255)];
   if (has_film && !film_direct) {
     for (int idx = tid; idx < spt * 128; idx += 512) {
       const int sm = idx >> 7, c4 = idx & 127;
@@ -795,12 +805,23 @@
 #pragma unroll
       for (int j = 0; j < 4; ++j) { fs[j] = f0[j]; fs[4 + j] = f1[j]; fb[j] = f2[j]; fb[4 + j] = f3[j]; }
     }
-    char* ob = out_ptr(mb, 2);
+    char* ob = EPI == 2 ? nullptr : out_ptr(mb, 2);
 #pragma unroll
     for (int ip = 0; ip < 2; ++ip, ob += 2 * ostep) {
       const int r = mb * 4 + 2 * ip;
+      const int trow = wm * 64 + mb * 16 + 4 * h4 + 2 * ip;
       f32x2_t v[8];
-      if (has_res) {
+      if constexpr (EPI == 1) {
+        const f32x4_t xa = *(const f32x4_t*)(s_x + trow * 2);
+        const f32x2_t x0 = {xa[0], xa[2]}, x1 = {xa[1], xa[3]};
+#pragma unroll
+        for (int jj = 0; jj < 4; ++jj) {
+          const f32x4_t w4 = *(const f32x4_t*)(s_rw + (c_l + 2 * jj) * 2);
+          const f32x2_t b2 = *(const f32x2_t*)(s_rb + c_l + 2 * jj);
+          v[2 * jj] = b2[0] + __builtin_elementwise_fma(x1, f32x2_t{w4[1], w4[1]}, x0 * w4[0]);
+          v[2 * jj + 1] = b2[1] + __builtin_elementwise_fma(x1, f32x2_t{w4[3], w4[3]}, x0 * w4[2]);
+        }
+      } else if (has_res) {
         const short8_t h0 = __builtin_bit_cast(short8_t, rh[0]), h1 = __builtin_bit_cast(short8_t, rh[1]);
 #pragma unroll
         for (int j = 0; j < 8; ++j) v[j] = f32x2_t{e2f<ET>((unsigned short)h0[j]), e2f<ET>((unsigned short)h1[j])};
@@ -826,6 +847,34 @@
 #pragma unroll
         for (int j = 0; j < 8; ++j) v[j] = v[j] * fs[j] + fb[j];
       }
+      if constexpr (EPI == 2) {
+        f32x2_t pd[2];
+#pragma unroll
+        for (int d = 0; d < 2; ++d) {
+          const f32x4_t w0 = *(const f32x4_t*)(s_rw + d * 256 + c_l), w1 = *(const f32x4_t*)(s_rw + d * 256 + c_l + 4);
+          f32x2_t a = v[0] * w0[0];
+#pragma unroll
+          for (int j = 1; j < 4; ++j) a = __builtin_elementwise_fma(v[j], f32x2_t{w0[j], w0[j]}, a);
+#pragma unroll
+          for (int j = 0; j < 4; ++j) a = __builtin_elementwise_fma(v[4 + j], f32x2_t{w1[j], w1[j]}, a);
+          pd[d] = a;
+        }
+        float q[4] = {pd[0][0], pd[1][0], pd[0][1], pd[1][1]};
+#pragma unroll
+        for (int k = 0; k < 4; ++k) q[k] = dpp_add<0xB1>(q[k]);
+#pragma unroll
+        for (int k = 0; k < 4; ++k) q[k] = dpp_add<0x4E>(q[k]);
+#pragma unroll
+        for (int k = 0; k < 4; ++k) q[k] = dpp_add<0x141>(q[k]);
+#pragma unroll
+        for (int k = 0; k < 4; ++k) q[k] = dpp_add<0x140>(q[k]);
+        if (r4 == 0) {
+          const int nparts = p.N >> 7;
+          float* wp = p.proj_ws + (((long long)tm * 256 + trow) * nparts + tn * 2 + wn) * 2;
+          *(f32x2_t*)wp = f32x2_t{q[0], q[1]};
+          *(f32x2_t*)(wp + nparts * 2) = f32x2_t{q[2], q[3]};
+        }
+      } else {
       float row[8];
 #pragma unroll
       for (int j = 0; j < 8; ++j) row[j] = v[j][0];
@@ -833,6 +882,7 @@
 #pragma unroll
       for (int j = 0; j < 8; ++j) row[j] = v[j][1];
       store_row(ob + ostep, row);
+      }
       __builtin_amdgcn_sched_barrier(0);
     }
   }
@@ -857,8 +907,10 @@
   return rc;
 }
 #endif
-template <int ET, bool SPLIT>
+constexpr int ENDS_RES_IN = 1 << 4, ENDS_PROJ = 2 << 4;
+template <int ETE, bool SPLIT>
 __global__ void __launch_bounds__(512, 2) conv3_halo16_kernel(ConvGemmParams p) {
+  constexpr int ET = ETE & 1, EPI = ETE >> 4;
   extern __shared__ __attribute__((aligned(16))) char smem[];
   constexpr int A_BUF = 40960, W_BUF = 32768, W_BASE = 2 * A_BUF;
   const int tid = threadIdx.x, lane = tid & 63;
@@ -1077,11 +1129,13 @@
   }
   __builtin_amdgcn_s_setprio(0);
   __syncthreads();
-  gemm_epilogue16<ET, SPLIT>(p, acc, smem, tm, tn, tid, lane, r4, h4, wm, wn);
-}
-
-template <int ET, bool SHORT = false, bool SPLITK = false, int NP = 5>
+  gemm_epilogue16<ET, SPLIT, false, EPI>(p, acc, smem, tm, tn, tid, lane, r4, h4, wm, wn);
+}
+
+template <int ETE, bool SHORT = false, bool SPLITK = false, int NP = 5>
 __global__ void __launch_bounds__(512, 2) conv3_halo16x3_kernel(ConvGemmParams p) {
+  constexpr int ET = ETE & 1, EPI = ETE >> 4;
+  static_assert(EPI == 0 || (!SHORT && !SPLITK && NP == 5), "the fused ends: 16 | L, one pass, five activation pieces");
   extern __shared__ __attribute__((aligned(16))) char smem[];
   static_assert(NP == 5 || NP == 6, "five or six activation pieces");
   constexpr int A_BUF = NP * 8192, W_BUF = 32768, W_BASE = 2 * A_BUF;
@@ -1356,7 +1410,7 @@
     }
     if (tid == 0) p.sk_cnt[tile] = 0;
   }
-  gemm_epilogue16<ET, true, SHORT>(p, acc, smem, tm, tn, tid, lane, r4, h4, wm, wn);
+  gemm_epilogue16<ET, true, SHORT, EPI>(p, acc, smem, tm, tn, tid, lane, r4, h4, wm, wn);
 #ifdef HALO16_STAMP
   __syncthreads();
   if (tid == 0) {
@@ -1756,6 +1810,14 @@
   hipFuncSetAttribute((const void*)conv3_halo16x3_kernel<1, true, true>, at, 147456);
   hipFuncSetAttribute((const void*)conv3_halo16x3_kernel<0, true, false, 6>, at, 163840);
   hipFuncSetAttribute((const void*)conv3_halo16x3_kernel<1, true, false, 6>, at, 163840);
+  hipFuncSetAttribute((const void*)conv3_halo16_kernel<ENDS_RES_IN | 0, false>, at, 147456);
+  hipFuncSetAttribute((const void*)conv3_halo16_kernel<ENDS_RES_IN | 1, false>, at, 147456);
+  hipFuncSetAttribute((const void*)conv3_halo16_kernel<ENDS_PROJ | 0, false>, at, 147456);
+  hipFuncSetAttribute((const void*)conv3_halo16_kernel<ENDS_PROJ | 1, false>, at, 147456);
+  hipFuncSetAttribute((const void*)conv3_halo16x3_kernel<ENDS_RES_IN | 0>, at, 147456);
+  hipFuncSetAttribute((const void*)conv3_halo16x3_kernel<ENDS_RES_IN | 1>, at, 147456);
+  hipFuncSetAttribute((const void*)conv3_halo16x3_kernel<ENDS_PROJ | 0>, at, 147456);
+  hipFuncSetAttribute((const void*)conv3_halo16x3_kernel<ENDS_PROJ | 1>, at, 147456);
   hipFuncSetAttribute((const void*)gemm16_kernel<0, false>, at, 131072);
   hipFuncSetAttribute((const void*)gemm16_kernel<1, false>, at, 131072);
   hipFuncSetAttribute((const void*)gemm16_kernel<0, true>, at, 131072);
@@ -1772,6 +1834,21 @@
   const bool split = fmt_split(fmt), f16 = st == ST_F16;
   const int ntn = (p.N + 255) >> 8, ntm = (p.M + 255) >> 8;
   const dim3 grid(ntm * ntn), block(512);
+  if (p.mode == MODE_GN_MISH_RES_IN || p.mode == MODE_GN_MISH_PROJ) {
+    const int gch = p.group_ch;
+    const bool ok = halo_eligible(p, fmt) && (p.L & 15) == 0 && p.splitk <= 1 && gch * 8 == p.N && (gch == 64 || gch == 128 || gch == 256) &&
+                    (p.mode == MODE_GN_MISH_RES_IN ? (p.res_x && p.res_w && p.res_b && p.Out) : (p.proj_w && p.proj_ws));
+    if (!ok) throw std::runtime_error("conv_gemm: the fused first residual / final projection need the halo tile at 16 | L");
+#define ENDS(E) do {                                                                                       \
+      if (split) { if (f16) DN_LAUNCH((conv3_halo16x3_kernel<E | 1>), grid, block, 147456, s, p);            \
+                   else DN_LAUNCH((conv3_halo16x3_kernel<E | 0>), grid, block, 147456, s, p); }              \
+      else { if (f16) DN_LAUNCH((conv3_halo16_kernel<E | 1, false>), grid, block, 147456, s, p);             \
+             else DN_LAUNCH((conv3_halo16_kernel<E | 0, false>), grid, block, 147456, s, p); }               \
+    } while (0)
+    if (p.mode == MODE_GN_MISH_RES_IN) ENDS(ENDS_RES_IN); else ENDS(ENDS_PROJ);
+#undef ENDS
+    return;
+  }
   if (halo_eligible(p, fmt)) {
     if (split && p.splitk > 1) {
       if (p.sk_ws == nullptr || p.sk_cnt == nullptr || ((p.Cin >> 5) % p.splitk) != 0 || (p.Cin >> 5) / p.splitk < 2)
@@ -2242,6 +2319,28 @@
 }
 
 struct ActNormArg { double mu[8], sg[8]; };
+template <int D>
+__device__ __forceinline__ void flow_step_apply(float v, float* __restrict__ x, const FlowStep& fs, double sg, double mu,
+                                                double* __restrict__ actions, long long pos, int b, int l, int d) {
+  const long long xi = pos * D + d;
+  float xn;
+  if (fs.mode == 0) {
+    xn = x[xi] + v * fs.dt;
+  } else if (fs.mode == 1) {
+    xn = v;
+  } else {
+    const float xc = x[xi];
+    float x0 = (xc - fs.sb * v) / fs.sa;
+    x0 = fminf(fmaxf(x0, -1.0f), 1.0f);
+    xn = fs.c0 * x0 + fs.c1 * xc;
+    if (fs.sigma != 0.0f) {
+      const long long zr = fs.z_idx ? (long long)fs.z_idx[b] : (long long)fs.z_row0 + b;
+      xn += fs.sigma * fs.z[zr * fs.z_row + (long long)l * D + d];
+    }
+  }
+  x[xi] = xn;
+  if (actions != nullptr) actions[xi] = (double)xn * sg + mu;
+}
 template <int PREC, int D>
 __global__ void __launch_bounds__(256) final_proj_flow_kernel(const void* __restrict__ Y, int C, int Lp, long long plane,
                                                               const float* __restrict__ W ,
@@ -2292,26 +2391,33 @@
     double sg = nm.sg[0], mu = nm.mu[0];
 #pragma unroll
     for (int d = 1; d < D; ++d) if (lane == d) { sv = s[d]; sg = nm.sg[d]; mu = nm.mu[d]; }
-    const float v = sv + bias[lane];
-    const long long xi = pos * D + lane;
-    float xn;
-    if (fs.mode == 0) {
-      xn = x[xi] + v * fs.dt;
-    } else if (fs.mode == 1) {
-      xn = v;
-    } else {
-      const float xc = x[xi];
-      float x0 = (xc - fs.sb * v) / fs.sa;
-      x0 = fminf(fmaxf(x0, -1.0f), 1.0f);
-      xn = fs.c0 * x0 + fs.c1 * xc;
-      if (fs.sigma != 0.0f) {
-        const long long zr = fs.z_idx ? (long long)fs.z_idx[b] : (long long)fs.z_row0 + b;
-        xn += fs.sigma * fs.z[zr * fs.z_row + (long long)l * D + lane];
-      }
-    }
-    x[xi] = xn;
-    if (actions != nullptr) actions[xi] = (double)xn * sg + mu;
-  }
+    flow_step_apply<D>(sv + bias[lane], x, fs, sg, mu, actions, pos, b, l, lane);
+  }
+}
+template <int D>
+__global__ void __launch_bounds__(256) final_partial_flow_kernel(const float* __restrict__ parts, int nparts,
+                                                                 const float* __restrict__ bias, float* __restrict__ x, FlowStep fs,
+                                                                 ActNormArg nm, double* __restrict__ actions, int B, int P) {
+  const long long i = blockIdx.x * 256LL + threadIdx.x;
+  if (i >= (long long)B * P * D) return;
+  const long long pos = i / D;
+  const int d = (int)(i - pos * D);
+  const int b = (int)(pos / P), l = (int)(pos - (long long)b * P);
+  const float* pp = parts + pos * nparts * D + d;
+  float sv = pp[0];
+  for (int k = 1; k < nparts; ++k) sv += pp[k * D];
+  double sg = nm.sg[0], mu = nm.mu[0];
+#pragma unroll
+  for (int dd = 1; dd < D; ++dd) if (d == dd) { sg = nm.sg[dd]; mu = nm.mu[dd]; }
+  flow_step_apply<D>(sv + bias[d], x, fs, sg, mu, actions, pos, b, l, d);
+}
+void launch_final_partial_flow(const float* parts, int nparts, const float* bias, int D, float* x, FlowStep fs,
+                               const double* act_norm, double* actions, int B, int P, hipStream_t s) {
+  if (D != 2 || nparts < 1) throw std::runtime_error("final projection from partial sums: action_dim must be 2");
+  const long long n = (long long)B * P * D;
+  ActNormArg nm{};
+  for (int d = 0; d < D; ++d) { nm.mu[d] = act_norm[d]; nm.sg[d] = act_norm[D + d]; }
+  DN_LAUNCH((final_partial_flow_kernel<2>), dim3((unsigned)((n + 255) / 256)), dim3(256), 0, s, parts, nparts, bias, x, fs, nm, actions, B, P);
 }
 void launch_final_proj_flow(const void* Y, int C, int Lp, long long plane, const float* W, const float* bias, int D, float* x,
                             FlowStep fs, const double* act_norm, double* actions, int B, int P, int fmt, hipStream_t s) {
```

Result: no change. 18930 candidate expansions/s (median of 6 runs) (+0.7%).
